# neka-nat/probreg

Measured on NVIDIA H100. Metric: cpd_em_iterations_per_sec, higher is better.
Workload: dtype f32

## Files before the change

probreg_b200/csrc/cpd_b200.cu:

```cuda
#include "cpd_b200.h"
#include "kernels.cuh"
#include "lowrank.cuh"
#include "gram_i8.cuh"
#include "bcpd.cuh"
#include "gmmtree.cuh"

#include <cub/device/device_radix_sort.cuh>
#ifdef CPD_HOST_EMU
#include "emu_nccl.h"
#include "emu_solver.h"
#endif

#include <dlfcn.h>
#include <math.h>
#include <stdarg.h>
#include <stdio.h>
#include <stdlib.h>
#include <string.h>

#include <algorithm>
#include <vector>

using namespace cpd;

static thread_local char g_err[512] = "";
static int fail(int code, const char* fmt, ...) {
    va_list ap;
    va_start(ap, fmt);
    vsnprintf(g_err, sizeof(g_err), fmt, ap);
    va_end(ap);
    return code;
}
#define CU(call)                                                                                   \
    do {                                                                                           \
        cudaError_t e_ = (call);                                                                   \
        if (e_ != cudaSuccess)                                                                     \
            return fail(CPD_ERR_CUDA, "%s failed at %s:%d: %s", #call, __FILE__, __LINE__, cudaGetErrorString(e_)); \
    } while (0)
#define KCHECK() CU(cudaGetLastError())

extern "C" const char* cpd_last_error(void) { return g_err; }
extern "C" int cpd_version(void) { return 100; }
extern "C" int cpd_device_count(void) {
    int n = 0;
    if (cudaGetDeviceCount(&n) != cudaSuccess) { cudaGetLastError(); return 0; }
    return n;
}

namespace {
typedef struct { char internal[128]; } nccl_uid;
typedef void* nccl_comm;
struct NcclApi {
    void* lib = nullptr;
    int (*GetUniqueId)(nccl_uid*) = nullptr;
    int (*CommInitRank)(nccl_comm*, int, nccl_uid, int) = nullptr;
    int (*AllReduce)(const void*, void*, size_t, int, int, nccl_comm, cudaStream_t) = nullptr;
    int (*CommDestroy)(nccl_comm) = nullptr;
    const char* (*GetErrorString)(int) = nullptr;
};
NcclApi g_nccl;
int load_nccl() {
    if (g_nccl.lib) return CPD_OK;
#ifdef CPD_HOST_EMU
    static_assert(sizeof(nccl_uid) == sizeof(emu::nccl_uid_t), "unique id layout");
    g_nccl.GetUniqueId = reinterpret_cast<int (*)(nccl_uid*)>(emu::ncclGetUniqueId);
    g_nccl.CommInitRank = reinterpret_cast<int (*)(nccl_comm*, int, nccl_uid, int)>(emu::ncclCommInitRank);
    g_nccl.AllReduce = emu::ncclAllReduce;
    g_nccl.CommDestroy = emu::ncclCommDestroy;
    g_nccl.GetErrorString = emu::ncclGetErrorString;
    g_nccl.lib = (void*)&g_nccl;
    return CPD_OK;
#endif
    const char* names[] = {"libnccl.so.2", "libnccl.so"};
    void* lib = nullptr;
    for (const char* nm : names) { lib = dlopen(nm, RTLD_NOW | RTLD_GLOBAL); if (lib) break; }
    if (!lib) return fail(CPD_ERR_NCCL, "cannot dlopen libnccl.so.2: %s", dlerror());
    g_nccl.GetUniqueId = (int (*)(nccl_uid*))dlsym(lib, "ncclGetUniqueId");
    g_nccl.CommInitRank = (int (*)(nccl_comm*, int, nccl_uid, int))dlsym(lib, "ncclCommInitRank");
    g_nccl.AllReduce = (int (*)(const void*, void*, size_t, int, int, nccl_comm, cudaStream_t))dlsym(lib, "ncclAllReduce");
    g_nccl.CommDestroy = (int (*)(nccl_comm))dlsym(lib, "ncclCommDestroy");
    g_nccl.GetErrorString = (const char* (*)(int))dlsym(lib, "ncclGetErrorString");
    if (!g_nccl.GetUniqueId || !g_nccl.CommInitRank || !g_nccl.AllReduce || !g_nccl.CommDestroy)
        return fail(CPD_ERR_NCCL, "libnccl lacks an expected symbol");
    g_nccl.lib = lib;
    return CPD_OK;
}
constexpr int NCCL_DOUBLE = 8, NCCL_SUM = 0;

struct SolverApi {
    void* lib = nullptr;
    int (*Create)(void**) = nullptr;
    int (*Destroy)(void*) = nullptr;
    int (*SetStream)(void*, cudaStream_t) = nullptr;
    int (*CreateParams)(void**) = nullptr;
    int (*DestroyParams)(void*) = nullptr;
    int (*XgetrfBuf)(void*, void*, int64_t, int64_t, int, const void*, int64_t, int, size_t*, size_t*) = nullptr;
    int (*Xgetrf)(void*, void*, int64_t, int64_t, int, void*, int64_t, int64_t*, int, void*, size_t, void*, size_t, int*) = nullptr;
    int (*Xgetrs)(void*, void*, int, int64_t, int64_t, int, const void*, int64_t, const int64_t*, int, void*, int64_t, int*) = nullptr;
};
SolverApi g_sol;
int load_cusolver() {
    if (g_sol.lib) return CPD_OK;
#ifdef CPD_HOST_EMU
    g_sol.Create = emu::solverCreate; g_sol.Destroy = emu::solverDestroy; g_sol.SetStream = emu::solverSetStream;
    g_sol.CreateParams = emu::solverCreateParams; g_sol.DestroyParams = emu::solverDestroyParams;
    g_sol.XgetrfBuf = emu::solverXgetrfBuf; g_sol.Xgetrf = emu::solverXgetrf; g_sol.Xgetrs = emu::solverXgetrs;
    g_sol.lib = (void*)&g_sol;
    return CPD_OK;
#endif
    const char* names[] = {"libcusolver.so.11", "/usr/local/cuda/lib64/libcusolver.so.11", "libcusolver.so"};
    void* lib = nullptr;
    for (const char* nm : names) { lib = dlopen(nm, RTLD_NOW | RTLD_GLOBAL); if (lib) break; }
    if (!lib) return fail(CPD_ERR_CUDA, "cannot dlopen libcusolver.so.11: %s", dlerror());
#define SOLSYM(field, name) g_sol.field = (decltype(g_sol.field))dlsym(lib, name)
    SOLSYM(Create, "cusolverDnCreate");
    SOLSYM(Destroy, "cusolverDnDestroy");
    SOLSYM(SetStream, "cusolverDnSetStream");
    SOLSYM(CreateParams, "cusolverDnCreateParams");
    SOLSYM(DestroyParams, "cusolverDnDestroyParams");
    SOLSYM(XgetrfBuf, "cusolverDnXgetrf_bufferSize");
    SOLSYM(Xgetrf, "cusolverDnXgetrf");
    SOLSYM(Xgetrs, "cusolverDnXgetrs");
#undef SOLSYM
    if (!g_sol.Create || !g_sol.SetStream || !g_sol.CreateParams || !g_sol.XgetrfBuf || !g_sol.Xgetrf || !g_sol.Xgetrs)
        return fail(CPD_ERR_CUDA, "libcusolver lacks an expected symbol");
    g_sol.lib = lib;
    return CPD_OK;
}
constexpr int CUDA_R_64F_ = 1, CUBLAS_OP_T_ = 1;
}
#define SOLV(call)                                                                          \
    do {                                                                                    \
        int r_ = (call);                                                                    \
        if (r_ != 0) return fail(CPD_ERR_CUDA, "%s failed with cusolverStatus %d", #call, r_); \
    } while (0)
#define NC(call)                                                                                                   \
    do {                                                                                                           \
        int r_ = (call);                                                                                           \
        if (r_ != 0)                                                                                               \
            return fail(CPD_ERR_NCCL, "%s failed: %s", #call, g_nccl.GetErrorString ? g_nccl.GetErrorString(r_) : "?"); \
    } while (0)

struct cpd_ctx {
    int device = 0, dim = 3, sm_count = 132, slots1 = 264, slots2 = 264;
    cudaStream_t stream = nullptr;
    bool own_stream = false;
    long long m = 0, mpad = 0, n = 0, npad = 0, n_global = 0;
    double *d_yc = nullptr, *d_ts = nullptr, *d_xc = nullptr, *d_raw = nullptr;
    size_t raw_cap = 0;
    float4 *d_srcP = nullptr, *d_srcJ = nullptr, *d_tgtP = nullptr, *d_tgtQ = nullptr;
    P1Part* d_part1 = nullptr;
    double* d_part2 = nullptr;
    size_t part1_cap = 0, part2_cap = 0;
    double *d_pt1 = nullptr, *d_p1 = nullptr, *d_pxc = nullptr, *d_px = nullptr;
    double *d_mom_src = nullptr, *d_mom_tgt = nullptr, *d_mom = nullptr, *d_sums = nullptr;
    size_t mom_src_cap = 0, mom_tgt_cap = 0, sums_cap = 0;
    DevState* d_state = nullptr;
    DevState h_state;
    double* h_pin = nullptr;
    double* d_frame = nullptr;
    double* h_stats = nullptr;
    cudaEvent_t stats_ev = nullptr, copy_ev = nullptr;
    int stats_pending = 0;
    long long stats_count[2] = {0, 0};
    bool origin_given = false;
    int it1 = 0, it2 = 0, j1 = 1, j2 = 1, g1 = 1, g2 = 1;
    float4 *d_sbox = nullptr, *d_tbox = nullptr, *d_ssub = nullptr, *d_tsub = nullptr;
    float *d_omax = nullptr, *d_omax_sub = nullptr;
    bool cull_on = true, cull_active = false;
    double extent = 0.0;
    int4 *d_work1 = nullptr, *d_work2 = nullptr;
    int *d_slots1 = nullptr, *d_slots2 = nullptr;
    bool have_source = false, have_target = false, have_state = false, prepared = false;
    nccl_comm comm = nullptr;
    int world = 1, rank = 0;
    int *d_perm_src = nullptr, *d_perm_tgt = nullptr, *d_idx_tmp = nullptr;
    unsigned *d_codes = nullptr, *d_codes_out = nullptr;
    size_t sort_cap = 0, sort_tmp_cap = 0;
    void* d_sort_tmp = nullptr;
    double *d_outN = nullptr, *d_outM = nullptr;
    float* d_G = nullptr;
    double *d_W = nullptr, *d_A = nullptr, *d_B = nullptr, *d_ts2 = nullptr, *d_nrpart = nullptr;
    int64_t* d_ipiv = nullptr;
    int* d_info = nullptr;
    void *d_work = nullptr, *h_work = nullptr, *sol = nullptr, *sol_params = nullptr;
    size_t work_dev = 0, work_host = 0;
    long long nr_m = 0;
    double nr_lmd = 0.0;
    bool nr_ready = false;
    bool nr_lost_to_bcpd = false;
    float* d_la = nullptr;
    double *d_la64 = nullptr, *d_la_part = nullptr, *d_bc_es = nullptr;
    size_t la_cap = 0;
    double* d_log2c = nullptr;
    bool wgt_on = false;
    BcpdState* d_bc = nullptr;
    float* d_bc_ginv = nullptr;
    double *d_bc_A = nullptr, *d_bc_S = nullptr, *d_bc_v = nullptr, *d_bc_r = nullptr, *d_bc_alpha = nullptr, *d_bc_sdiag = nullptr,
           *d_bc_part = nullptr, *d_bc_sums = nullptr;
    int64_t* d_bc_ipiv = nullptr;
    int* d_bc_info = nullptr;
    long long bc_m = 0;
    size_t bc_part_cap = 0;
    double bc_sigma2 = 0.0;
    bool bc_ready = false;
    bool bc_stopped = false;
    cudaEvent_t bc_ev[6] = {nullptr, nullptr, nullptr, nullptr, nullptr, nullptr};
    float bc_ms[5] = {0.f, 0.f, 0.f, 0.f, 0.f};
    long long bc_vec_m = 0, bc_dense_m = 0;
    bool bc_lowrank = false;
    double *d_bc_sys = nullptr, *d_bc_C = nullptr, *d_bc_CQ = nullptr, *d_bc_rt = nullptr, *d_bc_w = nullptr;
    int64_t* d_bc_lr_ipiv = nullptr;
    long long bc_lr_m = 0;
    int bc_lr_k = 0;
    int gt_levels = 0;
    long long gt_total = 0, gt_cap = 0, gt_m = 0;
    size_t gt_part_cap = 0, gt_sort_cap = 0;
    double *d_gt_nodes = nullptr, *d_gt_prep = nullptr, *d_gt_pts = nullptr, *d_gt_spts = nullptr, *d_gt_g = nullptr,
           *d_gt_part = nullptr, *d_gt_mom = nullptr, *d_gt_scr = nullptr;
    unsigned *d_gt_keys = nullptr, *d_gt_keys2 = nullptr;
    int *d_gt_idx = nullptr, *d_gt_idx2 = nullptr, *d_gt_cur = nullptr, *d_gt_start = nullptr, *d_gt_end = nullptr, *d_gt_asg = nullptr;
    long long* d_gt_seeds = nullptr;
    void* d_gt_sort = nullptr;
    cudaEvent_t gt_ev[7] = {nullptr, nullptr, nullptr, nullptr, nullptr, nullptr, nullptr};
    float gt_ms[6] = {0.f, 0.f, 0.f, 0.f, 0.f, 0.f};
    double *d_wgt = nullptr, *d_p1t = nullptr, *d_pxt = nullptr;
    long long prior_m = 0;
    double prior_alpha = 1.0;
    bool prior_on = false;
    int lr_rank = 0;
    int lr_owner = 0;
    double lr_gscale = 1.0;
    bool lr_w_stale = false;
    float lr_setup_ms[3] = {0.f, 0.f, 0.f};
    long long lr_m = 0;
    int lr_cap = 0;
    float4* d_lr_pts = nullptr;
    double *d_lr_Q = nullptr, *d_lr_X = nullptr, *d_lr_coef = nullptr, *d_lr_part = nullptr, *d_lr_Bc = nullptr, *d_lr_S = nullptr,
           *d_lr_R = nullptr, *d_lr_sys = nullptr, *d_lr_rhs = nullptr, *d_lr_c = nullptr, *d_lr_out = nullptr, *d_lr_panel = nullptr, *d_lr_Lt = nullptr;
    bool lr_spd = true;
    size_t lr_part_cap = 0;
    unsigned char* d_gi_planes = nullptr;
    double *d_gi_part = nullptr, *d_gi_colmax = nullptr;
    size_t gi_planes_cap = 0, gi_part_cap = 0, gi_colmax_cap = 0;
    size_t lr_out_cap = 0;
    P2PMailbox* d_box = nullptr;
    P2PInfo* d_p2p = nullptr;
    void* peer_ptr[P2P_MAX] = {nullptr};
    cudaEvent_t ev0 = nullptr, ev1 = nullptr, sev[7] = {nullptr, nullptr, nullptr, nullptr, nullptr, nullptr, nullptr};
    bool profiling = false;
    int64_t launches = 0;
    DevState* h_state_ring = nullptr;
    cudaEvent_t state_ev[8] = {nullptr, nullptr, nullptr, nullptr, nullptr, nullptr, nullptr, nullptr};
    int state_slot = 0;
    bool graph_on = true;
    cudaGraphExec_t em_graph = nullptr;
    int em_graph_key = -1, em_graph_launches = 0, prepare_gen = 0;
    void* d_flush = nullptr;
    size_t flush_cap = 0;
    std::vector<cudaEvent_t> pool;
};

namespace {
constexpr int STATE_RING = 8;
template <typename T>
int dev_alloc(T** p, size_t count) {
    if (*p) { cudaFree(*p); *p = nullptr; }
    cudaError_t e = cudaMalloc((void**)p, std::max<size_t>(count, 1) * sizeof(T));
    if (e != cudaSuccess) return fail(CPD_ERR_CUDA, "cudaMalloc(%zu bytes) failed: %s", count * sizeof(T), cudaGetErrorString(e));
    return CPD_OK;
}
#define TRY(x) do { int r__ = (x); if (r__ != CPD_OK) return r__; } while (0)
template <typename T>
struct DevBuf {
    T* p = nullptr;
    ~DevBuf() { if (p) cudaFree(p); }
    int alloc(size_t count) { return dev_alloc(&p, count); }
};

inline unsigned blocks_for(long long n) { return (unsigned)((n + THREADS - 1) / THREADS); }

struct WorkList {
    std::vector<int4> items;
    std::vector<int> tile_slots;
    int max_slots = 1;
};
WorkList build_work(int ntiles, int nunits, int slots, double last_cost, double overhead) {
    const double OVERHEAD = overhead;
    WorkList w;
    nunits = std::max(1, nunits);
    auto cost_of = [&](int t) { return t == ntiles - 1 ? last_cost : 1.0; };
    auto span_of = [&](int t, int j) { return cost_of(t) * (double)((nunits + j - 1) / j) + OVERHEAD; };
    int best_j = 1;
    double best = 1e300;
    for (int j = 1; j <= nunits; ++j) {
        const long long items = (long long)ntiles * j;
        const double waves = ceil((double)items / slots);
        const double span = waves * ((double)((nunits + j - 1) / j) + OVERHEAD);
        if (span < best - 1e-9) { best = span; best_j = j; }
        if (items > 8LL * slots) break;
    }
    w.tile_slots.assign(ntiles, best_j);
    if (ntiles <= slots) {
        std::vector<int> cuts(ntiles, 1);
        int used = ntiles;
        while (used < slots) {
            int worst = -1;
            double wv = -1.0;
            for (int t = 0; t < ntiles; ++t) {
                const double v = span_of(t, cuts[t]);
                if (cuts[t] < nunits && v > wv) { wv = v; worst = t; }
            }
            if (worst < 0) break;
            ++cuts[worst];
            ++used;
        }
        double span = 0.0;
        for (int t = 0; t < ntiles; ++t) span = std::max(span, span_of(t, cuts[t]));
        if (span <= best + 1e-9) w.tile_slots = cuts;
    }
    for (int t = 0; t < ntiles; ++t) {
        const int j = w.tile_slots[t];
        for (int s = 0; s < j; ++s) {
            const int a = (int)((long long)nunits * s / j), b = (int)((long long)nunits * (s + 1) / j);
            w.items.push_back(make_int4(t, a, b, s));
        }
        w.max_slots = std::max(w.max_slots, j);
    }
    std::stable_sort(w.items.begin(), w.items.end(), [&](const int4& a, const int4& b) {
        return cost_of(a.x) * (a.z - a.y) > cost_of(b.x) * (b.z - b.y);
    });
    return w;
}

int ensure_stats(cpd_ctx* h);
int upload_state(cpd_ctx* h) {
    TRY(ensure_stats(h));
    if (!h->h_state_ring) {
        CU(cudaMallocHost((void**)&h->h_state_ring, STATE_RING * sizeof(DevState)));
        for (int k = 0; k < STATE_RING; ++k) CU(cudaEventCreateWithFlags(&h->state_ev[k], cudaEventDisableTiming));
    }
    const int k = h->state_slot;
    h->state_slot = (k + 1) % STATE_RING;
    CU(cudaEventSynchronize(h->state_ev[k]));
    h->h_state_ring[k] = h->h_state;
    CU(cudaMemcpyAsync(h->d_state, &h->h_state_ring[k], sizeof(DevState), cudaMemcpyHostToDevice, h->stream));
    CU(cudaEventRecord(h->state_ev[k], h->stream));
    return CPD_OK;
}

int upload_cloud(cpd_ctx* h, const double* src, long long count, double* dst3) {
    if (h->dim == 3) {
        CU(cudaMemcpyAsync(dst3, src, (size_t)count * 3 * sizeof(double), cudaMemcpyHostToDevice, h->stream));
    } else {
        CU(cudaMemsetAsync(dst3, 0, (size_t)count * 3 * sizeof(double), h->stream));
        CU(cudaMemcpy2DAsync(dst3, 3 * sizeof(double), src, 2 * sizeof(double), 2 * sizeof(double), (size_t)count,
                             cudaMemcpyHostToDevice, h->stream));
    }
    return CPD_OK;
}
int download_cloud(cpd_ctx* h, const double* src3, long long count, double* dst) {
    if (h->dim == 3) {
        CU(cudaMemcpyAsync(dst, src3, (size_t)count * 3 * sizeof(double), cudaMemcpyDeviceToHost, h->stream));
    } else {
        CU(cudaMemcpy2DAsync(dst, 2 * sizeof(double), src3, 3 * sizeof(double), 2 * sizeof(double), (size_t)count,
                             cudaMemcpyDeviceToHost, h->stream));
    }
    return CPD_OK;
}

int cloud_sums_dev(cpd_ctx* h, const double* d_pts, long long count, double* part, double* d_out) {
    const unsigned nb = blocks_for(count);
    cloud_sums_kernel<<<nb, THREADS, 0, h->stream>>>(d_pts, count, part);
    reduce_cols_kernel<<<1, 4 * 32, 0, h->stream>>>(part, (int)nb, 4, d_out);
    KCHECK();
    h->launches += 2;
    return CPD_OK;
}

int ingest_cloud(cpd_ctx* h, const double* host_pts, long long count, int is_target, long long n_global, const double* origin,
                 int* d_perm, double* d_out) {
    if (h->raw_cap < (size_t)count * 3) { TRY(dev_alloc(&h->d_raw, (size_t)count * 3)); h->raw_cap = (size_t)count * 3; }
    const unsigned nb = blocks_for(count);
    if (h->sums_cap < (size_t)nb * 9 + 16) {
        TRY(dev_alloc(&h->d_sums, (size_t)nb * 9 + 16));
        h->sums_cap = (size_t)nb * 9 + 16;
    }
    if (h->sort_cap < (size_t)count) {
        TRY(dev_alloc(&h->d_codes, (size_t)count));
        TRY(dev_alloc(&h->d_codes_out, (size_t)count));
        TRY(dev_alloc(&h->d_idx_tmp, (size_t)count));
        h->sort_cap = (size_t)count;
    }
    size_t need = 0;
    CU(cub::DeviceRadixSort::SortPairs(nullptr, need, h->d_codes, h->d_codes_out, h->d_idx_tmp, d_perm, (int)count, 0, 30, h->stream));
    if (need > h->sort_tmp_cap) {
        if (h->d_sort_tmp) cudaFree(h->d_sort_tmp);
        h->d_sort_tmp = nullptr;
        CU(cudaMalloc(&h->d_sort_tmp, need));
        h->sort_tmp_cap = need;
    }
    TRY(upload_cloud(h, host_pts, count, h->d_raw));
    CU(cudaEventRecord(h->copy_ev, h->stream));
    double* frame = h->d_frame + 8 * is_target;
    stats_kernel<<<nb, THREADS, 0, h->stream>>>(h->d_raw, count, h->d_sums + 16);
    stats_fold_kernel<<<1, 288, 0, h->stream>>>(h->d_sums + 16, (int)nb, h->d_sums);
    cloud_frame_kernel<<<1, 32, 0, h->stream>>>(h->d_sums, count, is_target, n_global, origin != nullptr, origin ? origin[0] : 0.0,
                                                origin ? origin[1] : 0.0, origin ? origin[2] : 0.0, h->d_state, frame);
    CU(cudaMemcpyAsync(h->h_stats + 9 * is_target, h->d_sums, 9 * sizeof(double), cudaMemcpyDeviceToHost, h->stream));
    CU(cudaEventRecord(h->stats_ev, h->stream));
    h->stats_pending |= 1 << is_target;
    h->stats_count[is_target] = count;
    morton_frame_kernel<<<nb, THREADS, 0, h->stream>>>(h->d_raw, count, frame, h->d_codes, h->d_idx_tmp);
    CU(cub::DeviceRadixSort::SortPairs(h->d_sort_tmp, need, h->d_codes, h->d_codes_out, h->d_idx_tmp, d_perm, (int)count, 0, 30,
                                       h->stream));
    gather3_frame_kernel<<<nb, THREADS, 0, h->stream>>>(h->d_raw, d_perm, count, frame, d_out);
    KCHECK();
    h->launches += 6;
    CU(cudaEventSynchronize(h->copy_ev));
    return CPD_OK;
}

int ensure_stats(cpd_ctx* h) {
    if (!h->stats_pending) return CPD_OK;
    CU(cudaEventSynchronize(h->stats_ev));
    if (h->stats_pending & 1)
        for (int a = 0; a < 3; ++a) h->h_state.cy[a] = h->h_stats[a] / (double)h->stats_count[0];
    if (h->stats_pending & 2) {
        const double* t = h->h_stats + 9;
        if (!h->origin_given) for (int a = 0; a < 3; ++a) h->h_state.cx[a] = t[a] / (double)h->stats_count[1];
        h->extent = std::max(t[6] - t[3], std::max(t[7] - t[4], t[8] - t[5]));
    }
    h->stats_pending = 0;
    return CPD_OK;
}

int prepare(cpd_ctx* h) {
    TRY(ensure_stats(h));
    if (h->prepared) return CPD_OK;
    if (!h->have_source || !h->have_target) return fail(CPD_ERR_STATE, "source and target must both be set");
    h->it1 = (int)((h->n + ITILE1 - 1) / ITILE1);
    h->it2 = (int)((h->m + ITILE2 - 1) / ITILE2);
    const long long in_last = h->n - (long long)(h->it1 - 1) * ITILE1;
    const int live = (int)((in_last + 32 * RI1 - 1) / (32 * RI1));
    double last_cost = live < THREADS / 32 ? std::max(0.6, live / (double)(THREADS / 32)) : 1.0;
    if (const char* e = getenv("CPD_B200_PLAN_LAST_COST")) { const double v = atof(e); if (v > 0.0 && v <= 1.0) last_cost = v; }
    WorkList w1;
    if (const char* e = getenv("CPD_B200_PLAN_UNIT"); e && !strcmp(e, "stage")) {
        w1 = build_work(h->it1, (int)(h->mpad / P1_STAGE), h->slots1, last_cost, 0.5);
        for (int4& it : w1.items) { it.y *= P1_STAGE / SUB; it.z *= P1_STAGE / SUB; }
    } else {
        w1 = build_work(h->it1, (int)(h->mpad / SUB), h->slots1, last_cost, 0.5 * (P1_STAGE / SUB));
    }
    const WorkList w2 = build_work(h->it2, (int)(h->npad / P2_STAGE), h->slots2, 1.0, 0.5);
    h->j1 = w1.max_slots; h->g1 = (int)w1.items.size();
    h->j2 = w2.max_slots; h->g2 = (int)w2.items.size();
    TRY(dev_alloc(&h->d_work1, w1.items.size()));
    TRY(dev_alloc(&h->d_work2, w2.items.size()));
    TRY(dev_alloc(&h->d_slots1, w1.tile_slots.size()));
    TRY(dev_alloc(&h->d_slots2, w2.tile_slots.size()));
    CU(cudaMemcpyAsync(h->d_work1, w1.items.data(), w1.items.size() * sizeof(int4), cudaMemcpyHostToDevice, h->stream));
    CU(cudaMemcpyAsync(h->d_work2, w2.items.data(), w2.items.size() * sizeof(int4), cudaMemcpyHostToDevice, h->stream));
    CU(cudaMemcpyAsync(h->d_slots1, w1.tile_slots.data(), w1.tile_slots.size() * sizeof(int), cudaMemcpyHostToDevice, h->stream));
    CU(cudaMemcpyAsync(h->d_slots2, w2.tile_slots.data(), w2.tile_slots.size() * sizeof(int), cudaMemcpyHostToDevice, h->stream));
    CU(cudaStreamSynchronize(h->stream));
    TRY(dev_alloc(&h->d_sbox, (size_t)(h->mpad / P1_STAGE) * 2));
    TRY(dev_alloc(&h->d_tbox, (size_t)(h->npad / P2_STAGE) * 2));
    TRY(dev_alloc(&h->d_omax, (size_t)(h->npad / P2_STAGE)));
    TRY(dev_alloc(&h->d_ssub, (size_t)(h->mpad / SUB) * 2));
    TRY(dev_alloc(&h->d_tsub, (size_t)(h->npad / SUB) * 2));
    TRY(dev_alloc(&h->d_omax_sub, (size_t)(h->npad / SUB)));
    const size_t need1 = (size_t)h->j1 * h->n, need2 = (size_t)h->j2 * h->m * 4;
    if (need1 > h->part1_cap) { TRY(dev_alloc(&h->d_part1, need1)); h->part1_cap = need1; }
    if (need2 > h->part2_cap) { TRY(dev_alloc(&h->d_part2, need2)); h->part2_cap = need2; }
    const size_t ms = (size_t)blocks_for(h->m) * MOM_SRC, mt = (size_t)blocks_for(h->npad) * MOM_TGT;
    if (ms > h->mom_src_cap) { TRY(dev_alloc(&h->d_mom_src, ms)); h->mom_src_cap = ms; }
    if (mt > h->mom_tgt_cap) { TRY(dev_alloc(&h->d_mom_tgt, mt)); h->mom_tgt_cap = mt; }
    h->prepared = true;
    h->prepare_gen += 1;
    return CPD_OK;
}

int allreduce(cpd_ctx* h, double* buf, size_t count) {
    if (!h->comm) return CPD_OK;
    NC(g_nccl.AllReduce(buf, buf, count, NCCL_DOUBLE, NCCL_SUM, h->comm, h->stream));
    return CPD_OK;
}

inline void mark(cpd_ctx* h, int k) {
    if (h->profiling) cudaEventRecord(h->sev[k], h->stream);
}

int launch_estep(cpd_ctx* h, const double* d_sigma2, const double* d_w, const double* d_ts) {
    TRY(prepare(h));
    const long long cover = std::max(h->mpad, h->n);
    mark(h, 0);
    pack_kernel<<<blocks_for(cover), THREADS, 0, h->stream>>>(h->d_state, d_sigma2, h->d_yc, d_ts, h->d_xc, h->m, h->mpad,
                                                              h->n, h->d_srcP, h->d_srcJ, h->d_tgtP);
    mark(h, 1);
    const bool cull = h->cull_on && h->cull_active;
    const int nst1 = (int)(h->mpad / P1_STAGE);
    stage_bbox_kernel<<<(unsigned)nst1, THREADS, 0, h->stream>>>(h->d_srcP, (int)h->m, P1_STAGE, h->d_sbox);
    h->launches += 1;
    const int nsub1 = (int)(h->mpad / SUB), nsub2 = (int)(h->npad / SUB);
    if (cull) {
        stage_bbox_kernel<<<(unsigned)(h->npad / P2_STAGE), THREADS, 0, h->stream>>>(h->d_tgtP, (int)h->n, P2_STAGE, h->d_tbox);
        sub_bbox_kernel<<<(unsigned)((nsub1 + 7) / 8), THREADS, 0, h->stream>>>(h->d_srcP, (int)h->m, nsub1, h->d_ssub);
        sub_bbox_kernel<<<(unsigned)((nsub2 + 7) / 8), THREADS, 0, h->stream>>>(h->d_tgtP, (int)h->n, nsub2, h->d_tsub);
        h->launches += 3;
    }
    const bool wgt = h->wgt_on;
    if (wgt) {
        weight_patch_kernel<<<blocks_for(h->m), THREADS, 0, h->stream>>>(h->d_la, h->m, h->d_srcP, h->d_srcJ);
        h->launches += 1;
    }
#define CPD_PASS1(C, W) pass1_kernel<C, W><<<h->g1, THREADS, PASS1_SMEM, h->stream>>>(h->d_tgtP, (int)h->n, h->d_srcJ, h->d_work1, h->d_part1, h->d_sbox, nst1, (C) ? h->d_ssub : nullptr)
    if (cull) { if (wgt) CPD_PASS1(true, true); else CPD_PASS1(true, false); }
    else { if (wgt) CPD_PASS1(false, true); else CPD_PASS1(false, false); }
#undef CPD_PASS1
    mark(h, 2);
    finalize1_kernel<<<blocks_for(h->npad), THREADS, 0, h->stream>>>(h->d_state, d_sigma2, d_w, h->d_part1, h->d_slots1, (int)h->n,
                                                                     h->d_tgtP, h->d_tgtQ, h->npad, h->d_pt1, h->d_mom_tgt,
                                                                     wgt ? h->d_log2c : nullptr);
    mark(h, 3);
    if (cull) {
        stage_omax_kernel<<<(unsigned)(h->npad / P2_STAGE), THREADS, 0, h->stream>>>(h->d_tgtQ, h->d_omax);
        sub_omax_kernel<<<(unsigned)((nsub2 + 7) / 8), THREADS, 0, h->stream>>>(h->d_tgtQ, nsub2, h->d_omax_sub);
        h->launches += 2;
    }
#define CPD_PASS2(C, W) pass2_kernel<C, W><<<h->g2, THREADS, PASS2_SMEM, h->stream>>>(h->d_srcP, (int)h->m, h->d_tgtQ, h->d_work2, h->d_part2, (C) ? h->d_tbox : nullptr, (C) ? h->d_omax : nullptr, (C) ? h->d_tsub : nullptr, (C) ? h->d_omax_sub : nullptr)
    if (cull) { if (wgt) CPD_PASS2(true, true); else CPD_PASS2(true, false); }
    else { if (wgt) CPD_PASS2(false, true); else CPD_PASS2(false, false); }
#undef CPD_PASS2
    mark(h, 4);
    finalize2_kernel<<<blocks_for(h->m), THREADS, 0, h->stream>>>(h->d_state, d_sigma2, h->d_part2, h->d_slots2, (int)h->m, h->d_yc,
                                                                  d_ts, h->d_p1, h->d_pxc, h->d_mom_src);
    mark(h, 5);
    mark(h, 6);
    KCHECK();
    h->launches += 5;
    return CPD_OK;
}

int read_params(cpd_ctx* h, cpd_params* out) {
    static_assert(sizeof(DevState) <= 48 * sizeof(double), "DevState outgrew the pinned staging buffer");
    CU(cudaMemcpyAsync(h->h_pin, h->d_state, sizeof(DevState), cudaMemcpyDeviceToHost, h->stream));
    CU(cudaStreamSynchronize(h->stream));
    if (reinterpret_cast<const DevState*>(h->h_pin)->err)
        return fail(CPD_ERR_STATE, "a peer rank did not deliver its moments within the P2P exchange timeout");
    const int d = h->dim;
    for (int i = 0; i < 9; ++i) out->lin[i] = 0.0;
    for (int i = 0; i < d; ++i)
        for (int j = 0; j < d; ++j) out->lin[i * d + j] = h->h_pin[3 * i + j];
    for (int i = 0; i < 3; ++i) out->t[i] = (i < d) ? h->h_pin[9 + i] : 0.0;
    out->scale = h->h_pin[12];
    out->sigma2 = h->h_pin[13];
    TRY(ensure_stats(h));
    h->cull_active = h->extent > 0.0 && 13.3 * sqrt(out->sigma2) < 0.25 * h->extent;
    out->q = h->h_pin[14];
    out->n_p = h->h_pin[15];
    return CPD_OK;
}
}

extern "C" int cpd_plan_work(int ntiles, int nunits, int slots, double last_tile_cost, int* items ,
                             int capacity, int* n_items, int* max_slots) {
    if (ntiles < 1 || nunits < 1 || slots < 1 || !(last_tile_cost > 0.0 && last_tile_cost <= 1.0) || !n_items || !max_slots)
        return fail(CPD_ERR_ARG, "bad argument");
    const WorkList w = build_work(ntiles, nunits, slots, last_tile_cost, 0.5 * (P1_STAGE / SUB));
    *n_items = (int)w.items.size();
    *max_slots = w.max_slots;
    if (items) {
        if (capacity < (int)w.items.size()) return fail(CPD_ERR_ARG, "capacity %d < %d work items", capacity, (int)w.items.size());
        for (size_t i = 0; i < w.items.size(); ++i) {
            items[4 * i] = w.items[i].x; items[4 * i + 1] = w.items[i].y; items[4 * i + 2] = w.items[i].z; items[4 * i + 3] = w.items[i].w;
        }
    }
    return CPD_OK;
}

extern "C" int cpd_create(cpd_ctx** out, int device, int dim, void* stream) {
    if (!out) return fail(CPD_ERR_ARG, "out is NULL");
    if (dim != 2 && dim != 3) return fail(CPD_ERR_ARG, "dim must be 2 or 3, got %d", dim);
    int ndev = 0;
    if (cudaGetDeviceCount(&ndev) != cudaSuccess || ndev == 0) {
        cudaGetLastError();
        return fail(CPD_ERR_CUDA, "no CUDA device: this library has no CPU path");
    }
    if (device < 0 || device >= ndev) return fail(CPD_ERR_ARG, "device %d out of range (%d visible)", device, ndev);
    CU(cudaSetDevice(device));
    cudaDeviceProp prop;
    CU(cudaGetDeviceProperties(&prop, device));
    if (prop.major != 9 || prop.minor != 0)
        return fail(CPD_ERR_CUDA, "device %d is sm_%d%d; this library is built for sm_90a (Hopper) only", device, prop.major, prop.minor);
    cpd_ctx* h = new cpd_ctx();
    h->device = device;
    h->dim = dim;
    h->sm_count = prop.multiProcessorCount;
    if (stream) { h->stream = (cudaStream_t)stream; h->own_stream = false; }
    else { CU(cudaStreamCreateWithFlags(&h->stream, cudaStreamNonBlocking)); h->own_stream = true; }
    CU(cudaFuncSetAttribute(pass1_kernel<false, false>, cudaFuncAttributeMaxDynamicSharedMemorySize, PASS1_SMEM));
    CU(cudaFuncSetAttribute(pass2_kernel<false, false>, cudaFuncAttributeMaxDynamicSharedMemorySize, PASS2_SMEM));
    CU(cudaFuncSetAttribute(pass1_kernel<true, false>, cudaFuncAttributeMaxDynamicSharedMemorySize, PASS1_SMEM));
    CU(cudaFuncSetAttribute(pass2_kernel<true, false>, cudaFuncAttributeMaxDynamicSharedMemorySize, PASS2_SMEM));
    CU(cudaFuncSetAttribute(pass1_kernel<false, true>, cudaFuncAttributeMaxDynamicSharedMemorySize, PASS1_SMEM));
    CU(cudaFuncSetAttribute(pass2_kernel<false, true>, cudaFuncAttributeMaxDynamicSharedMemorySize, PASS2_SMEM));
    CU(cudaFuncSetAttribute(pass1_kernel<true, true>, cudaFuncAttributeMaxDynamicSharedMemorySize, PASS1_SMEM));
    CU(cudaFuncSetAttribute(pass2_kernel<true, true>, cudaFuncAttributeMaxDynamicSharedMemorySize, PASS2_SMEM));
    int occ1 = 0, occ2 = 0;
    CU(cudaOccupancyMaxActiveBlocksPerMultiprocessor(&occ1, pass1_kernel<false, false>, THREADS, PASS1_SMEM));
    CU(cudaOccupancyMaxActiveBlocksPerMultiprocessor(&occ2, pass2_kernel<false, false>, THREADS, PASS2_SMEM));
    h->slots1 = h->sm_count * std::max(1, occ1);
    h->slots2 = h->sm_count * std::max(1, occ2);
    TRY(dev_alloc(&h->d_state, 1));
    TRY(dev_alloc(&h->d_mom, (size_t)MOM_PAD));
    CU(cudaMallocHost((void**)&h->h_pin, 64 * sizeof(double)));
    TRY(dev_alloc(&h->d_frame, 16));
    CU(cudaMallocHost((void**)&h->h_stats, 18 * sizeof(double)));
    CU(cudaEventCreateWithFlags(&h->stats_ev, cudaEventDisableTiming));
    CU(cudaEventCreateWithFlags(&h->copy_ev, cudaEventDisableTiming));
    CU(cudaEventCreate(&h->ev0));
    CU(cudaEventCreate(&h->ev1));
    for (int k = 0; k < 7; ++k) CU(cudaEventCreate(&h->sev[k]));
    { const char* e = getenv("CPD_B200_NO_CULL"); h->cull_on = !(e && e[0] == '1'); }
    { const char* e = getenv("CPD_B200_NO_GRAPH"); h->graph_on = !(e && e[0] == '1'); }
    memset(&h->h_state, 0, sizeof(DevState));
    h->h_state.dim = dim;
    h->h_state.scale = 1.0;
    h->h_state.lin[0] = h->h_state.lin[4] = h->h_state.lin[8] = 1.0;
    h->h_state.update_scale = 1;
    *out = h;
    return upload_state(h);
}

extern "C" void cpd_destroy(cpd_ctx* h) {
    if (!h) return;
    cudaSetDevice(h->device);
    cudaStreamSynchronize(h->stream);
    void* wl[] = {h->d_work1, h->d_work2, h->d_slots1, h->d_slots2, h->d_sbox, h->d_tbox, h->d_omax, h->d_ssub, h->d_tsub, h->d_omax_sub};
    for (void* p : wl) if (p) cudaFree(p);
    void* srt[] = {h->d_perm_src, h->d_perm_tgt, h->d_idx_tmp, h->d_codes, h->d_codes_out, h->d_sort_tmp, h->d_outN, h->d_outM};
    for (void* p : srt) if (p) cudaFree(p);
    void* nrp[] = {h->d_G, h->d_W, h->d_A, h->d_B, h->d_ts2, h->d_nrpart, h->d_ipiv, h->d_info, h->d_work};
    for (void* p : nrp) if (p) cudaFree(p);
    void* lrp[] = {h->d_lr_pts, h->d_lr_Q, h->d_lr_X, h->d_lr_coef, h->d_lr_part, h->d_lr_Bc, h->d_lr_S, h->d_lr_R, h->d_lr_sys, h->d_lr_rhs,
                   h->d_lr_c, h->d_lr_out, h->d_lr_panel, h->d_lr_Lt, h->d_gi_planes, h->d_gi_part, h->d_gi_colmax, h->d_wgt, h->d_p1t, h->d_pxt, h->d_la, h->d_log2c,
                   h->d_la64, h->d_la_part, h->d_bc_es};
    for (void* p : lrp) if (p) cudaFree(p);
    void* bcp[] = {h->d_bc, h->d_bc_ginv, h->d_bc_A, h->d_bc_S, h->d_bc_v, h->d_bc_r, h->d_bc_alpha, h->d_bc_sdiag, h->d_bc_part, h->d_bc_sums,
                   h->d_bc_ipiv, h->d_bc_info, h->d_bc_sys, h->d_bc_C, h->d_bc_CQ, h->d_bc_rt, h->d_bc_w, h->d_bc_lr_ipiv};
    for (void* p : bcp) if (p) cudaFree(p);
    for (cudaEvent_t e : h->bc_ev) if (e) cudaEventDestroy(e);
    void* gtp[] = {h->d_gt_nodes, h->d_gt_prep, h->d_gt_pts, h->d_gt_spts, h->d_gt_g, h->d_gt_part, h->d_gt_mom, h->d_gt_scr, h->d_gt_keys,
                   h->d_gt_keys2, h->d_gt_idx, h->d_gt_idx2, h->d_gt_cur, h->d_gt_start, h->d_gt_end, h->d_gt_asg, h->d_gt_seeds, h->d_gt_sort};
    for (void* p : gtp) if (p) cudaFree(p);
    for (cudaEvent_t e : h->gt_ev) if (e) cudaEventDestroy(e);
    if (h->h_work) free(h->h_work);
    if (h->sol_params && g_sol.DestroyParams) g_sol.DestroyParams(h->sol_params);
    if (h->sol && g_sol.Destroy) g_sol.Destroy(h->sol);
    for (int r = 0; r < P2P_MAX; ++r) if (h->peer_ptr[r]) cudaIpcCloseMemHandle(h->peer_ptr[r]);
    if (h->d_box) cudaFree(h->d_box);
    if (h->d_p2p) cudaFree(h->d_p2p);
    void* ptrs[] = {h->d_yc, h->d_ts, h->d_xc, h->d_raw, h->d_srcP, h->d_srcJ, h->d_tgtP, h->d_tgtQ, h->d_part1, h->d_part2, h->d_pt1, h->d_p1,
                    h->d_pxc, h->d_px, h->d_mom_src, h->d_mom_tgt, h->d_mom, h->d_sums, h->d_state, h->d_flush};
    for (void* p : ptrs) if (p) cudaFree(p);
    if (h->h_pin) cudaFreeHost(h->h_pin);
    if (h->h_stats) cudaFreeHost(h->h_stats);
    if (h->d_frame) cudaFree(h->d_frame);
    if (h->stats_ev) cudaEventDestroy(h->stats_ev);
    if (h->copy_ev) cudaEventDestroy(h->copy_ev);
#ifndef CPD_HOST_EMU
    if (h->em_graph) cudaGraphExecDestroy(h->em_graph);
#endif
    if (h->h_state_ring) cudaFreeHost(h->h_state_ring);
    for (int k = 0; k < 8; ++k) if (h->state_ev[k]) cudaEventDestroy(h->state_ev[k]);
    if (h->ev0) cudaEventDestroy(h->ev0);
    if (h->ev1) cudaEventDestroy(h->ev1);
    for (int k = 0; k < 7; ++k) if (h->sev[k]) cudaEventDestroy(h->sev[k]);
    for (cudaEvent_t e : h->pool) if (e) cudaEventDestroy(e);
    if (h->own_stream) cudaStreamDestroy(h->stream);
    delete h;
}

extern "C" int cpd_set_source(cpd_ctx* h, const double* source, int64_t m) {
    if (!h || !source) return fail(CPD_ERR_ARG, "null argument");
    if (m < 1 || m > 0x7fffffffLL - 65536) return fail(CPD_ERR_ARG, "source count %lld out of range", (long long)m);
    CU(cudaSetDevice(h->device));
    if (m != h->m || !h->d_yc) {
        h->m = m;
        h->mpad = (m + P1_STAGE - 1) / P1_STAGE * P1_STAGE;
        TRY(dev_alloc(&h->d_yc, (size_t)m * 3));
        TRY(dev_alloc(&h->d_ts, (size_t)m * 3));
        TRY(dev_alloc(&h->d_srcP, (size_t)h->mpad));
        TRY(dev_alloc(&h->d_srcJ, (size_t)h->mpad * 2));
        TRY(dev_alloc(&h->d_p1, (size_t)m));
        TRY(dev_alloc(&h->d_pxc, (size_t)m * 3));
        TRY(dev_alloc(&h->d_px, (size_t)m * 3));
        TRY(dev_alloc(&h->d_perm_src, (size_t)m));
        TRY(dev_alloc(&h->d_outM, (size_t)m * 3));
        h->prepared = false;
        h->nr_ready = false;
    }
    TRY(ingest_cloud(h, source, m, 0, 0, nullptr, h->d_perm_src, h->d_yc));
    h->bc_ready = false;
    h->bc_stopped = false;
    h->h_state.m = m;
    h->have_source = true;
    return CPD_OK;
}

extern "C" int cpd_set_target(cpd_ctx* h, const double* target, int64_t n_local, int64_t n_global, const double* frame_origin) {
    if (!h || !target) return fail(CPD_ERR_ARG, "null argument");
    if (n_local < 1 || n_local > 0x7fffffffLL - 65536) return fail(CPD_ERR_ARG, "target count %lld out of range", (long long)n_local);
    if (n_global < n_local) return fail(CPD_ERR_ARG, "n_global (%lld) < n_local (%lld)", (long long)n_global, (long long)n_local);
    if (!frame_origin && n_global != n_local) return fail(CPD_ERR_ARG, "a sharded target needs an explicit frame_origin");
    CU(cudaSetDevice(h->device));
    if (n_local != h->n || !h->d_xc) {
        h->n = n_local;
        h->npad = (n_local + P2_STAGE - 1) / P2_STAGE * P2_STAGE;
        TRY(dev_alloc(&h->d_xc, (size_t)n_local * 3));
        TRY(dev_alloc(&h->d_tgtP, (size_t)n_local));
        TRY(dev_alloc(&h->d_tgtQ, (size_t)h->npad * 3));
        TRY(dev_alloc(&h->d_pt1, (size_t)n_local));
        TRY(dev_alloc(&h->d_perm_tgt, (size_t)n_local));
        TRY(dev_alloc(&h->d_outN, (size_t)n_local));
        h->prepared = false;
    }
    h->n_global = n_global;
    double origin[3] = {0.0, 0.0, 0.0};
    if (frame_origin) for (int a = 0; a < h->dim; ++a) origin[a] = frame_origin[a];
    h->origin_given = frame_origin != nullptr;
    if (h->origin_given) for (int a = 0; a < 3; ++a) h->h_state.cx[a] = origin[a];
    TRY(ingest_cloud(h, target, n_local, 1, n_global, frame_origin ? origin : nullptr, h->d_perm_tgt, h->d_xc));
    h->h_state.n_global = n_global;
    h->have_target = true;
    return CPD_OK;
}

extern "C" int cpd_sigma2_init(cpd_ctx* h, double* sigma2) {
    if (!h || !sigma2) return fail(CPD_ERR_ARG, "null argument");
    if (!h->have_source || !h->have_target) return fail(CPD_ERR_STATE, "source and target must both be set");
    CU(cudaSetDevice(h->device));
    double sx[4], sy[4];
    const size_t pn = (size_t)blocks_for(h->n) * 4, pm = (size_t)blocks_for(h->m) * 4;
    if (h->sums_cap < 16 + pn + pm) { TRY(dev_alloc(&h->d_sums, 16 + pn + pm)); h->sums_cap = 16 + pn + pm; }
    TRY(cloud_sums_dev(h, h->d_xc, h->n, h->d_sums + 16, h->d_sums));
    if (h->comm) TRY(allreduce(h, h->d_sums, 4));
    TRY(cloud_sums_dev(h, h->d_yc, h->m, h->d_sums + 16 + pn, h->d_sums + 4));
    CU(cudaMemcpyAsync(h->h_pin, h->d_sums, 8 * sizeof(double), cudaMemcpyDeviceToHost, h->stream));
    CU(cudaStreamSynchronize(h->stream));
    TRY(ensure_stats(h));
    for (int k = 0; k < 4; ++k) { sx[k] = h->h_pin[k]; sy[k] = h->h_pin[4 + k]; }
    double dlt[3], d2 = 0.0, dsy = 0.0;
    for (int a = 0; a < 3; ++a) { dlt[a] = h->h_state.cy[a] - h->h_state.cx[a]; d2 += dlt[a] * dlt[a]; dsy += dlt[a] * sy[1 + a]; }
    const double M = (double)h->m, N = (double)h->n_global;
    const double syy = sy[0] + 2.0 * dsy + M * d2;
    double cross = 0.0;
    for (int a = 0; a < 3; ++a) cross += sx[1 + a] * (sy[1 + a] + M * dlt[a]);
    *sigma2 = (M * sx[0] + N * syy - 2.0 * cross) / (M * N * h->dim);
    return CPD_OK;
}

extern "C" int cpd_set_state(cpd_ctx* h, int tf_kind, int update_scale, double w, const cpd_params* init) {
    if (!h || !init) return fail(CPD_ERR_ARG, "null argument");
    if (tf_kind != CPD_TF_RIGID && tf_kind != CPD_TF_AFFINE) return fail(CPD_ERR_ARG, "tf_kind %d not supported by the fused EM loop", tf_kind);
    if (!(w >= 0.0 && w < 1.0)) return fail(CPD_ERR_ARG, "w must be in [0, 1), got %g", w);
    if (!(init->sigma2 > 0.0)) return fail(CPD_ERR_ARG, "sigma2 must be positive, got %g", init->sigma2);
    CU(cudaSetDevice(h->device));
    DevState& s = h->h_state;
    const int d = h->dim;
    for (int i = 0; i < 3; ++i)
        for (int j = 0; j < 3; ++j) s.lin[3 * i + j] = (i < d && j < d) ? init->lin[i * d + j] : (i == j ? 1.0 : 0.0);
    for (int i = 0; i < 3; ++i) s.t[i] = (i < d) ? init->t[i] : 0.0;
    s.scale = (tf_kind == CPD_TF_RIGID) ? init->scale : 1.0;
    s.sigma2 = init->sigma2;
    s.q = init->q;
    s.n_p = 0.0;
    s.w = w;
    s.tf_kind = tf_kind;
    s.update_scale = update_scale ? 1 : 0;
    s.dim = d;
    TRY(ensure_stats(h));
    h->cull_active = h->extent > 0.0 && 13.3 * sqrt(init->sigma2) < 0.25 * h->extent;
    h->have_state = true;
    return upload_state(h);
}

namespace {
int em_step_launches(cpd_ctx* h) {
    TRY(launch_estep(h, &h->d_state->sigma2, &h->d_state->w, nullptr));
    const int nbs = (int)blocks_for(h->m), nbt = (int)blocks_for(h->npad);
    if (h->d_p2p) {
        moments_p2p_kernel<<<1, 256, 0, h->stream>>>(h->d_state, h->d_mom_src, nbs, RM_SRC, h->d_mom_tgt, nbt, RM_TGT, h->d_mom,
                                                     h->d_p2p);
        h->launches += 1;
    } else if (h->comm) {
        moments_kernel<0><<<1, 256, 0, h->stream>>>(h->d_state, h->d_mom_src, nbs, RM_SRC, h->d_mom_tgt, nbt, RM_TGT, h->d_mom);
        TRY(allreduce(h, h->d_mom, MOM_PAD));
        mstep_residual_kernel<<<1, 32, 0, h->stream>>>(h->d_state, h->d_mom);
        h->launches += 2;
    } else {
        moments_kernel<1><<<1, 256, 0, h->stream>>>(h->d_state, h->d_mom_src, nbs, RM_SRC, h->d_mom_tgt, nbt, RM_TGT, h->d_mom);
        h->launches += 1;
    }
    mark(h, 6);
    KCHECK();
    return CPD_OK;
}
}

extern "C" int cpd_em_step(cpd_ctx* h, cpd_params* out) {
    if (!h) return fail(CPD_ERR_ARG, "null handle");
    if (!h->have_state) return fail(CPD_ERR_STATE, "cpd_set_state has not been called");
    CU(cudaSetDevice(h->device));
#ifndef CPD_HOST_EMU
    const bool use_graph = h->graph_on && !h->profiling && !(h->comm && !h->d_p2p) && !h->wgt_on;
#else
    const bool use_graph = false;
#endif
    if (!use_graph) {
        TRY(em_step_launches(h));
    }
#ifndef CPD_HOST_EMU
    else {
        TRY(prepare(h));
        const int key = h->prepare_gen * 2 + ((h->cull_on && h->cull_active) ? 1 : 0);
        if (!h->em_graph || h->em_graph_key != key) {
            if (h->em_graph) { cudaGraphExecDestroy(h->em_graph); h->em_graph = nullptr; }
            const int64_t before = h->launches;
            cudaGraph_t g = nullptr;
            CU(cudaStreamBeginCapture(h->stream, cudaStreamCaptureModeThreadLocal));
            const int rc = em_step_launches(h);
            const cudaError_t ce = cudaStreamEndCapture(h->stream, &g);
            h->em_graph_launches = (int)(h->launches - before);
            h->launches = before;
            if (rc != CPD_OK) { if (g) cudaGraphDestroy(g); return rc; }
            if (ce != cudaSuccess) return fail(CPD_ERR_CUDA, "cudaStreamEndCapture failed: %s", cudaGetErrorString(ce));
            const cudaError_t ie = cudaGraphInstantiate(&h->em_graph, g, 0);
            cudaGraphDestroy(g);
            if (ie != cudaSuccess) { h->em_graph = nullptr; return fail(CPD_ERR_CUDA, "cudaGraphInstantiate failed: %s", cudaGetErrorString(ie)); }
            h->em_graph_key = key;
        }
        CU(cudaGraphLaunch(h->em_graph, h->stream));
        h->launches += h->em_graph_launches;
    }
#endif
    if (out) return read_params(h, out);
    return CPD_OK;
}

extern "C" int cpd_em_run(cpd_ctx* h, int maxiter, double tol, cpd_params* out, int* iters_run, double* trace) {
    if (!h || !out) return fail(CPD_ERR_ARG, "null argument");
    if (!h->have_state) return fail(CPD_ERR_STATE, "cpd_set_state has not been called");
    double q = h->h_state.q;
    int it = 0;
    cpd_params cur;
    memset(&cur, 0, sizeof(cur));
    for (it = 0; it < maxiter; ++it) {
        TRY(cpd_em_step(h, &cur));
        if (trace) { trace[2 * it] = cur.sigma2; trace[2 * it + 1] = cur.q; }
        if (fabs(cur.q - q) < tol) { ++it; break; }
        q = cur.q;
    }
    if (maxiter <= 0) TRY(read_params(h, &cur));
    *out = cur;
    if (iters_run) *iters_run = it;
    return CPD_OK;
}

extern "C" int cpd_estep(cpd_ctx* h, const double* t_source, double sigma2, double w, double* pt1, double* p1, double* px, double* n_p) {
    if (!h || !t_source) return fail(CPD_ERR_ARG, "null argument");
    if (!(sigma2 > 0.0)) return fail(CPD_ERR_ARG, "sigma2 must be positive, got %g", sigma2);
    if (!(w >= 0.0 && w < 1.0)) return fail(CPD_ERR_ARG, "w must be in [0, 1), got %g", w);
    if (!h->have_source || !h->have_target) return fail(CPD_ERR_STATE, "source and target must both be set");
    CU(cudaSetDevice(h->device));
    if (h->raw_cap < (size_t)h->m * 3) { TRY(dev_alloc(&h->d_raw, (size_t)h->m * 3)); h->raw_cap = (size_t)h->m * 3; }
    TRY(upload_cloud(h, t_source, h->m, h->d_raw));
    gather3_kernel<<<blocks_for(h->m), THREADS, 0, h->stream>>>(h->d_raw, h->d_perm_src, h->m, 0.0, 0.0, 0.0, h->d_ts);
    h->launches += 1;
    TRY(ensure_stats(h));
    h->cull_active = h->extent > 0.0 && 13.3 * sqrt(sigma2) < 0.25 * h->extent;
    h->h_pin[32] = sigma2;
    h->h_pin[33] = w;
    CU(cudaMemcpyAsync(&h->d_state->es_sigma2, h->h_pin + 32, 2 * sizeof(double), cudaMemcpyHostToDevice, h->stream));
    TRY(launch_estep(h, &h->d_state->es_sigma2, &h->d_state->es_w, h->d_ts));
    if (h->comm) {
        TRY(allreduce(h, h->d_p1, (size_t)h->m));
        TRY(allreduce(h, h->d_pxc, (size_t)h->m * 3));
    }
    return cpd_last_estep(h, pt1, p1, px, n_p);
}

namespace {
int bcpd_weights(cpd_ctx* h, const double* alpha, const double* sdiag, const int* perm, const double* ssw) {
    const long long m = h->m;
    const unsigned nb = blocks_for(m);
    bcpd_la_kernel<<<nb, THREADS, 0, h->stream>>>(alpha, sdiag, m, ssw, h->dim, h->d_la64, h->d_la_part);
    bcpd_la_finish_kernel<<<1, 32, 0, h->stream>>>(h->d_la_part, (int)nb, ssw, h->dim, h->n_global, h->d_log2c);
    bcpd_la_apply_kernel<<<nb, THREADS, 0, h->stream>>>(h->d_la64, perm, m, h->d_log2c, h->d_la);
    KCHECK();
    h->launches += 3;
    return CPD_OK;
}
int ensure_weight_buffers(cpd_ctx* h) {
    const long long m = h->m;
    if (h->la_cap < (size_t)m) {
        TRY(dev_alloc(&h->d_la, (size_t)m));
        TRY(dev_alloc(&h->d_la64, (size_t)m));
        TRY(dev_alloc(&h->d_la_part, (size_t)blocks_for(m)));
        h->la_cap = (size_t)m;
    }
    if (!h->d_log2c) TRY(dev_alloc(&h->d_log2c, 3));
    if (!h->d_bc_es) TRY(dev_alloc(&h->d_bc_es, 3));
    return CPD_OK;
}
}

extern "C" int cpd_bcpd_estep(cpd_ctx* h, const double* t_source, double scale, const double* alpha, const double* sigma_diag,
                              double sigma2, double w, double* nu_d, double* nu, double* px, double* n_p) {
    if (!h || !t_source || !alpha || !sigma_diag) return fail(CPD_ERR_ARG, "null argument");
    if (!(sigma2 > 0.0)) return fail(CPD_ERR_ARG, "sigma2 must be positive, got %g", sigma2);
    if (!(w >= 0.0 && w < 1.0)) return fail(CPD_ERR_ARG, "w must be in [0, 1), got %g", w);
    if (!h->have_source || !h->have_target) return fail(CPD_ERR_STATE, "source and target must both be set");
    CU(cudaSetDevice(h->device));
    const long long m = h->m;
    bool any_weight = false;
    for (long long i = 0; i < m; ++i) {
        if (!(alpha[i] >= 0.0) || !(sigma_diag[i] >= 0.0)) return fail(CPD_ERR_ARG, "alpha and diag(sigma_mat) must be non-negative");
        any_weight = any_weight || (alpha[i] > 0.0 && sigma_diag[i] < INFINITY);
    }
    if (!any_weight) return fail(CPD_ERR_ARG, "every source has zero weight");
    TRY(ensure_weight_buffers(h));
    h->h_pin[44] = scale;
    h->h_pin[45] = sigma2;
    h->h_pin[46] = w;
    CU(cudaMemcpyAsync(h->d_bc_es, h->h_pin + 44, 3 * sizeof(double), cudaMemcpyHostToDevice, h->stream));
    CU(cudaMemcpyAsync(h->d_outM, alpha, (size_t)m * sizeof(double), cudaMemcpyHostToDevice, h->stream));
    CU(cudaMemcpyAsync(h->d_outM + m, sigma_diag, (size_t)m * sizeof(double), cudaMemcpyHostToDevice, h->stream));
    TRY(bcpd_weights(h, h->d_outM, h->d_outM + m, h->d_perm_src, h->d_bc_es));
    if (h->raw_cap < (size_t)m * 3) { TRY(dev_alloc(&h->d_raw, (size_t)m * 3)); h->raw_cap = (size_t)m * 3; }
    TRY(upload_cloud(h, t_source, m, h->d_raw));
    gather3_kernel<<<blocks_for(m), THREADS, 0, h->stream>>>(h->d_raw, h->d_perm_src, m, 0.0, 0.0, 0.0, h->d_ts);
    h->launches += 1;
    TRY(ensure_stats(h));
    h->cull_active = h->extent > 0.0 && 13.3 * sqrt(sigma2) < 0.25 * h->extent;
    h->h_pin[32] = sigma2;
    h->h_pin[33] = w;
    CU(cudaMemcpyAsync(&h->d_state->es_sigma2, h->h_pin + 32, 2 * sizeof(double), cudaMemcpyHostToDevice, h->stream));
    h->wgt_on = true;
    const int r = launch_estep(h, &h->d_state->es_sigma2, &h->d_state->es_w, h->d_ts);
    h->wgt_on = false;
    TRY(r);
    if (h->comm) {
        TRY(allreduce(h, h->d_p1, (size_t)m));
        TRY(allreduce(h, h->d_pxc, (size_t)m * 3));
    }
    return cpd_last_estep(h, nu_d, nu, px, n_p);
}

extern "C" int cpd_last_estep(cpd_ctx* h, double* pt1, double* p1, double* px, double* n_p) {
    if (!h) return fail(CPD_ERR_ARG, "null handle");
    if (!h->prepared) return fail(CPD_ERR_STATE, "no E-step has run on this handle");
    CU(cudaSetDevice(h->device));
    if (pt1) {
        scatter_kernel<<<blocks_for(h->n), THREADS, 0, h->stream>>>(h->d_pt1, h->d_perm_tgt, h->n, 1, h->d_outN);
        CU(cudaMemcpyAsync(pt1, h->d_outN, (size_t)h->n * sizeof(double), cudaMemcpyDeviceToHost, h->stream));
        h->launches += 1;
    }
    if (p1) {
        scatter_kernel<<<blocks_for(h->m), THREADS, 0, h->stream>>>(h->d_p1, h->d_perm_src, h->m, 1, h->d_outM);
        CU(cudaMemcpyAsync(p1, h->d_outM, (size_t)h->m * sizeof(double), cudaMemcpyDeviceToHost, h->stream));
        CU(cudaStreamSynchronize(h->stream));
        h->launches += 1;
    }
    if (px) {
        uncentre_px_kernel<<<blocks_for(h->m), THREADS, 0, h->stream>>>(h->d_state, h->d_p1, h->d_pxc, (int)h->m, h->d_px);
        scatter_kernel<<<blocks_for(h->m), THREADS, 0, h->stream>>>(h->d_px, h->d_perm_src, h->m, 3, h->d_outM);
        KCHECK();
        h->launches += 2;
        TRY(download_cloud(h, h->d_outM, h->m, px));
    }
    if (n_p) {
        const unsigned nb = blocks_for(h->m);
        if (h->sums_cap < (size_t)nb * 4 + 4) { TRY(dev_alloc(&h->d_sums, (size_t)nb * 4 + 4)); h->sums_cap = (size_t)nb * 4 + 4; }
        src_moments_api_kernel<<<nb, THREADS, 0, h->stream>>>((int)h->m, h->d_yc, h->d_p1, h->d_pxc, h->d_mom_src);
        reduce_cols_kernel<<<1, MOM_SRC * 32, 0, h->stream>>>(h->d_mom_src, (int)nb, MOM_SRC, h->d_mom);
        KCHECK();
        h->launches += 2;
        CU(cudaMemcpyAsync(h->h_pin + 40, h->d_mom, sizeof(double), cudaMemcpyDeviceToHost, h->stream));
    }
    CU(cudaStreamSynchronize(h->stream));
    if (n_p) *n_p = h->h_pin[40];
    return CPD_OK;
}

extern "C" int cpd_mstep(cpd_ctx* h, int tf_kind, int update_scale, const double* pt1, const double* p1, const double* px, double n_p,
                         cpd_params* out) {
    (void)n_p;
    if (!h || !pt1 || !p1 || !px || !out) return fail(CPD_ERR_ARG, "null argument");
    if (tf_kind != CPD_TF_RIGID && tf_kind != CPD_TF_AFFINE) return fail(CPD_ERR_ARG, "tf_kind %d not supported", tf_kind);
    if (!h->have_source || !h->have_target) return fail(CPD_ERR_STATE, "source and target must both be set");
    CU(cudaSetDevice(h->device));
    TRY(prepare(h));
    h->h_state.tf_kind = tf_kind;
    h->h_state.update_scale = update_scale ? 1 : 0;
    CU(cudaMemcpyAsync(&h->d_state->tf_kind, &h->h_state.tf_kind, 2 * sizeof(int), cudaMemcpyHostToDevice, h->stream));
    CU(cudaMemcpyAsync(h->d_outN, pt1, (size_t)h->n * sizeof(double), cudaMemcpyHostToDevice, h->stream));
    gather1_kernel<<<blocks_for(h->n), THREADS, 0, h->stream>>>(h->d_outN, h->d_perm_tgt, h->n, h->d_pt1);
    CU(cudaMemcpyAsync(h->d_outM, p1, (size_t)h->m * sizeof(double), cudaMemcpyHostToDevice, h->stream));
    gather1_kernel<<<blocks_for(h->m), THREADS, 0, h->stream>>>(h->d_outM, h->d_perm_src, h->m, h->d_p1);
    if (h->raw_cap < (size_t)h->m * 3) { TRY(dev_alloc(&h->d_raw, (size_t)h->m * 3)); h->raw_cap = (size_t)h->m * 3; }
    TRY(upload_cloud(h, px, h->m, h->d_raw));
    gather3_kernel<<<blocks_for(h->m), THREADS, 0, h->stream>>>(h->d_raw, h->d_perm_src, h->m, 0.0, 0.0, 0.0, h->d_px);
    h->launches += 3;
    const int nbs = (int)blocks_for(h->m), nbt = (int)blocks_for(h->n);
    centre_px_kernel<<<nbs, THREADS, 0, h->stream>>>(h->d_state, h->d_p1, h->d_px, (int)h->m, h->d_pxc);
    src_moments_api_kernel<<<nbs, THREADS, 0, h->stream>>>((int)h->m, h->d_yc, h->d_p1, h->d_pxc, h->d_mom_src);
    tgt_moments_api_kernel<<<nbt, THREADS, 0, h->stream>>>(h->d_pt1, h->d_xc, (int)h->n, h->d_mom_tgt);
    moments_kernel<0><<<1, 256, 0, h->stream>>>(h->d_state, h->d_mom_src, nbs, MOM_SRC, h->d_mom_tgt, nbt, MOM_TGT, h->d_mom);
    KCHECK();
    if (h->comm) TRY(allreduce(h, h->d_mom + MOM_SRC, MOM_TGT));
    mstep_api_kernel<<<1, 32, 0, h->stream>>>(h->d_state, h->d_mom);
    KCHECK();
    h->launches += 5;
    return read_params(h, out);
}

#include "host_nonrigid.inl"
#include "host_bcpd.inl"
#include "host_gmmtree.inl"
#include "host_stateless.inl"
#include "host_multi.inl"
#include "host_measure.inl"
```

probreg_b200/csrc/kernels.cuh:

```cuda
#pragma once
#include <cuda_runtime.h>
#include <stdint.h>

namespace cpd {

#ifndef CPD_RI1
#define CPD_RI1 4
#endif
#ifndef CPD_RI2
#define CPD_RI2 4
#endif
#ifndef CPD_MINB1
#define CPD_MINB1 2
#endif
#ifndef CPD_MINB2
#define CPD_MINB2 2
#endif
#ifndef CPD_UNROLL1
#define CPD_UNROLL1 4
#endif
#ifndef CPD_UNROLL2
#define CPD_UNROLL2 4
#endif
#ifndef CPD_SUB
#define CPD_SUB 64
#endif
#ifndef CPD_GRP
#define CPD_GRP 8
#endif
constexpr int UNROLL1 = CPD_UNROLL1, UNROLL2 = CPD_UNROLL2;
constexpr int THREADS = 256;
constexpr int RI1 = CPD_RI1, RI2 = CPD_RI2;
constexpr int ITILE1 = THREADS * RI1, ITILE2 = THREADS * RI2;
constexpr int NPAIR1 = RI1 / 2, NPAIR2 = RI2 / 2;
#ifndef CPD_P1_STAGE
#define CPD_P1_STAGE 512
#endif
#ifndef CPD_P2_STAGE
#define CPD_P2_STAGE 512
#endif
constexpr int P1_STAGE = CPD_P1_STAGE;
constexpr int P2_STAGE = CPD_P2_STAGE;
static_assert(P1_STAGE % 256 == 0 && P2_STAGE % 256 == 0 && P1_STAGE >= 256 && P2_STAGE >= 256, "stage sizes are multiples of 256");
constexpr int P1_REC = 32, P2_REC = 48;
#ifndef CPD_NSTAGE
#define CPD_NSTAGE 3
#endif
constexpr int NSTAGE = CPD_NSTAGE;
constexpr int P1_STAGE_BYTES = P1_STAGE * P1_REC, P2_STAGE_BYTES = P2_STAGE * P2_REC;
constexpr int SUB = CPD_SUB;
constexpr int GRP = CPD_GRP;
constexpr int PASS1_SMEM = NSTAGE * P1_STAGE_BYTES + 64, PASS2_SMEM = NSTAGE * P2_STAGE_BYTES + 64;

#ifdef CPD_HOST_EMU
#define CPD_DYN_SMEM(name) unsigned char* const name = emu::g_dyn_smem
#else
#define CPD_DYN_SMEM(name) extern __shared__ __align__(128) unsigned char name[]
#endif

constexpr float O_INIT = 1048576.0f;
constexpr float TWO100 = 1.2676506002282294e30f;
constexpr float FAR_COORD = 1.0e18f;

constexpr double LOG2E = 1.4426950408889634074;
constexpr double DEAD_LOG2 = -1075.0;
constexpr double EPS32 = 1.1920928955078125e-07;

enum { RM_NP = 0, RM_SY = 1, RM_C = 4, RM_V1 = 10, RM_VY = 13, RM_SRC = 22, RM_SRR = 22, RM_NPT = 23, RM_TGT = 2,
       RM_COUNT = 24, MOM_PAD = 32 };
enum { MOM_NP = 0, MOM_SX = 1, MOM_SY = 4, MOM_B = 7, MOM_C = 16, MOM_NPT = 22, MOM_SXT = 23, MOM_TXX = 26,
       MOM_COUNT = 27, MOM_SRC = 22, MOM_TGT = 5 };

struct P1Part {
    double S;
    double SU;
    float o;
    float pad;
};

struct DevState {
    double lin[9];
    double t[3];
    double scale;
    double sigma2;
    double q;
    double n_p;
    double cx[3];
    double cy[3];
    double w;
    double es_sigma2;
    double es_w;
    long long m;
    long long n_global;
    int tf_kind;
    int update_scale;
    int dim;
    int err;
};

constexpr int P2P_MAX = 16;
struct P2PMailbox {
    double slots[2][P2P_MAX][MOM_PAD];
    unsigned long long flags[2][P2P_MAX];
};
struct P2PInfo {
    P2PMailbox* box[P2P_MAX];
    int world, rank;
    unsigned long long seq;
    unsigned long long timeout_ns;
};

#ifdef CPD_HOST_EMU
}
#include "emu_device.h"
namespace cpd {
#else
__device__ __forceinline__ float ex2(float x) {
    float y;
    asm("ex2.approx.ftz.f32 %0, %1;" : "=f"(y) : "f"(x));
    return y;
}
typedef unsigned long long u64;
__device__ __forceinline__ u64 pack2(float lo, float hi) { u64 r; asm("mov.b64 %0, {%1, %2};" : "=l"(r) : "f"(lo), "f"(hi)); return r; }
__device__ __forceinline__ float2 unpack2(u64 v) { float2 r; asm("mov.b64 {%0, %1}, %2;" : "=f"(r.x), "=f"(r.y) : "l"(v)); return r; }
__device__ __forceinline__ u64 fsub2(u64 a, u64 b) {
    const float2 x = unpack2(a), y = unpack2(b);
    return pack2(__fsub_rn(x.x, y.x), __fsub_rn(x.y, y.y));
}
__device__ __forceinline__ u64 fadd2(u64 a, u64 b) {
    const float2 x = unpack2(a), y = unpack2(b);
    return pack2(__fadd_rn(x.x, y.x), __fadd_rn(x.y, y.y));
}
__device__ __forceinline__ u64 fmul2(u64 a, u64 b) {
    const float2 x = unpack2(a), y = unpack2(b);
    return pack2(__fmul_rn(x.x, y.x), __fmul_rn(x.y, y.y));
}
__device__ __forceinline__ u64 ffma2(u64 a, u64 b, u64 c) {
    const float2 x = unpack2(a), y = unpack2(b), z = unpack2(c);
    return pack2(__fmaf_rn(x.x, y.x, z.x), __fmaf_rn(x.y, y.y, z.y));
}
__device__ __forceinline__ unsigned long long globaltimer_ns() {
    unsigned long long t;
    asm volatile("mov.u64 %0, %%globaltimer;" : "=l"(t));
    return t;
}
__device__ __forceinline__ uint32_t smem_u32(const void* p) { return (uint32_t)__cvta_generic_to_shared(p); }
__device__ __forceinline__ void mbar_init(uint64_t* bar, uint32_t count) {
    asm volatile("mbarrier.init.shared::cta.b64 [%0], %1;" ::"r"(smem_u32(bar)), "r"(count));
}
__device__ __forceinline__ void mbar_fence_init() { asm volatile("fence.mbarrier_init.release.cluster;" ::: "memory"); }
__device__ __forceinline__ void mbar_expect_tx(uint64_t* bar, uint32_t bytes) {
    asm volatile("mbarrier.arrive.expect_tx.shared::cta.b64 _, [%0], %1;" ::"r"(smem_u32(bar)), "r"(bytes) : "memory");
}
__device__ __forceinline__ void tma_load_1d(void* dst, const void* src, uint32_t bytes, uint64_t* bar) {
    asm volatile("cp.async.bulk.shared::cluster.global.mbarrier::complete_tx::bytes [%0], [%1], %2, [%3];" ::"r"(
                     smem_u32(dst)),
                 "l"(src), "r"(bytes), "r"(smem_u32(bar))
                 : "memory");
}
__device__ __forceinline__ void mbar_wait(uint64_t* bar, uint32_t parity) {
    asm volatile(
        "{\n"
        ".reg .pred P1;\n"
        "LAB_WAIT:\n"
        "mbarrier.try_wait.parity.shared::cta.b64 P1, [%0], %1;\n"
        "@P1 bra DONE;\n"
        "bra LAB_WAIT;\n"
        "DONE:\n"
        "}" ::"r"(smem_u32(bar)),
        "r"(parity)
        : "memory");
}
#endif
__device__ __forceinline__ double warp_sum(double v) {
#pragma unroll
    for (int o = 16; o > 0; o >>= 1) v += __shfl_xor_sync(0xffffffffu, v, o);
    return v;
}
template <int K>
__device__ __forceinline__ void block_reduce_store(double (&v)[K], double* out) {
    __shared__ double sh[K][THREADS / 32];
    const int lane = threadIdx.x & 31, wid = threadIdx.x >> 5;
#pragma unroll
    for (int k = 0; k < K; ++k) {
        double s = warp_sum(v[k]);
        if (lane == 0) sh[k][wid] = s;
    }
    __syncthreads();
    if (threadIdx.x < K) {
        double s = 0.0;
#pragma unroll
        for (int w = 0; w < THREADS / 32; ++w) s += sh[threadIdx.x][w];
        out[threadIdx.x] = s;
    }
}

__global__ void __launch_bounds__(THREADS)
pack_kernel(const DevState* __restrict__ st, const double* __restrict__ sigma2_ptr,
            const double* __restrict__ yc , const double* __restrict__ ts ,
            const double* __restrict__ xc , long long m, long long mpad, long long n,
            float4* __restrict__ srcP , float4* __restrict__ srcJ ,
            float4* __restrict__ tgtP ) {
    const long long i = (long long)blockIdx.x * THREADS + threadIdx.x;
    const double sk = sqrt(LOG2E / (2.0 * *sigma2_ptr));
    if (i < mpad) {
        float4 o;
        if (i < m) {
            double px, py, pz;
            if (ts != nullptr) {
                px = ts[3 * i + 0] - st->cx[0];
                py = ts[3 * i + 1] - st->cx[1];
                pz = ts[3 * i + 2] - st->cx[2];
            } else {
                const double s = (st->tf_kind == 0) ? st->scale : 1.0;
                double l[9], tp[3];
#pragma unroll
                for (int k = 0; k < 9; ++k) l[k] = s * st->lin[k];
#pragma unroll
                for (int a = 0; a < 3; ++a)
                    tp[a] = l[3 * a] * st->cy[0] + l[3 * a + 1] * st->cy[1] + l[3 * a + 2] * st->cy[2] + st->t[a] - st->cx[a];
                const double y0 = yc[3 * i], y1 = yc[3 * i + 1], y2 = yc[3 * i + 2];
                px = l[0] * y0 + l[1] * y1 + l[2] * y2 + tp[0];
                py = l[3] * y0 + l[4] * y1 + l[5] * y2 + tp[1];
                pz = l[6] * y0 + l[7] * y1 + l[8] * y2 + tp[2];
            }
            o = make_float4((float)(sk * px), (float)(sk * py), (float)(sk * pz), 0.0f);
        } else {
            o = make_float4(FAR_COORD, FAR_COORD, FAR_COORD, 0.0f);
        }
        srcP[i] = o;
        srcJ[2 * i] = make_float4(o.x, o.x, o.y, o.y);
        srcJ[2 * i + 1] = make_float4(o.z, o.z, 0.0f, 0.0f);
    }
    if (i < n) {
        tgtP[i] = make_float4((float)(sk * xc[3 * i]), (float)(sk * xc[3 * i + 1]), (float)(sk * xc[3 * i + 2]), 0.0f);
    }
}

__global__ void __launch_bounds__(THREADS)
weight_patch_kernel(const float* __restrict__ la, long long m, float4* __restrict__ srcP, float4* __restrict__ srcJ) {
    const long long i = (long long)blockIdx.x * THREADS + threadIdx.x;
    if (i < m) {
        const float v = la[i];
        srcP[i].w = v;
        float4 r = srcJ[2 * i + 1];
        r.z = v; r.w = v;
        srcJ[2 * i + 1] = r;
    }
}

constexpr float CULL_GAP = 130.0f;
__global__ void __launch_bounds__(THREADS)
stage_bbox_kernel(const float4* __restrict__ pts, int n, int blk, float4* __restrict__ box) {
    __shared__ float sh[6][THREADS / 32];
    const int b = blockIdx.x;
    float lo[3] = {3.0e38f, 3.0e38f, 3.0e38f}, hi[3] = {-3.0e38f, -3.0e38f, -3.0e38f};
    for (int i = b * blk + threadIdx.x; i < min(n, (b + 1) * blk); i += THREADS) {
        const float4 p = pts[i];
        lo[0] = fminf(lo[0], p.x); lo[1] = fminf(lo[1], p.y); lo[2] = fminf(lo[2], p.z);
        hi[0] = fmaxf(hi[0], p.x); hi[1] = fmaxf(hi[1], p.y); hi[2] = fmaxf(hi[2], p.z);
    }
    const int lane = threadIdx.x & 31, wid = threadIdx.x >> 5;
#pragma unroll
    for (int a = 0; a < 3; ++a) {
#pragma unroll
        for (int o = 16; o > 0; o >>= 1) {
            lo[a] = fminf(lo[a], __shfl_xor_sync(0xffffffffu, lo[a], o));
            hi[a] = fmaxf(hi[a], __shfl_xor_sync(0xffffffffu, hi[a], o));
        }
        if (lane == 0) { sh[a][wid] = lo[a]; sh[3 + a][wid] = hi[a]; }
    }
    __syncthreads();
    if (threadIdx.x == 0) {
        float l[3], h[3];
        for (int a = 0; a < 3; ++a) {
            l[a] = sh[a][0]; h[a] = sh[3 + a][0];
            for (int w = 1; w < THREADS / 32; ++w) { l[a] = fminf(l[a], sh[a][w]); h[a] = fmaxf(h[a], sh[3 + a][w]); }
        }
        box[2 * b] = make_float4(l[0], l[1], l[2], 0.f);
        box[2 * b + 1] = make_float4(h[0], h[1], h[2], 0.f);
    }
}
__global__ void __launch_bounds__(THREADS)
stage_omax_kernel(const float4* __restrict__ tgtQ, float* __restrict__ omax) {
    __shared__ float sh[THREADS / 32];
    const int b = blockIdx.x;
    float m = 3.0e38f;
    for (int i = threadIdx.x; i < P2_STAGE; i += THREADS) m = fminf(m, tgtQ[3 * ((size_t)b * P2_STAGE + i) + 1].z);
#pragma unroll
    for (int o = 16; o > 0; o >>= 1) m = fminf(m, __shfl_xor_sync(0xffffffffu, m, o));
    if ((threadIdx.x & 31) == 0) sh[threadIdx.x >> 5] = m;
    __syncthreads();
    if (threadIdx.x == 0) {
        for (int w = 1; w < THREADS / 32; ++w) m = fminf(m, sh[w]);
        omax[b] = -m;
    }
}
__global__ void __launch_bounds__(THREADS)
sub_bbox_kernel(const float4* __restrict__ pts, int n, int nsub, float4* __restrict__ box) {
    const int b = blockIdx.x * (THREADS / 32) + (threadIdx.x >> 5), lane = threadIdx.x & 31;
    if (b >= nsub) return;
    float lo[3] = {3.0e38f, 3.0e38f, 3.0e38f}, hi[3] = {-3.0e38f, -3.0e38f, -3.0e38f};
    for (int i = b * SUB + lane; i < min(n, (b + 1) * SUB); i += 32) {
        const float4 p = pts[i];
        lo[0] = fminf(lo[0], p.x); lo[1] = fminf(lo[1], p.y); lo[2] = fminf(lo[2], p.z);
        hi[0] = fmaxf(hi[0], p.x); hi[1] = fmaxf(hi[1], p.y); hi[2] = fmaxf(hi[2], p.z);
    }
#pragma unroll
    for (int a = 0; a < 3; ++a) {
#pragma unroll
        for (int o = 16; o > 0; o >>= 1) {
            lo[a] = fminf(lo[a], __shfl_xor_sync(0xffffffffu, lo[a], o));
            hi[a] = fmaxf(hi[a], __shfl_xor_sync(0xffffffffu, hi[a], o));
        }
    }
    if (lane == 0) {
        box[2 * b] = make_float4(lo[0], lo[1], lo[2], 0.f);
        box[2 * b + 1] = make_float4(hi[0], hi[1], hi[2], 0.f);
    }
}
__global__ void __launch_bounds__(THREADS)
sub_omax_kernel(const float4* __restrict__ tgtQ, int nsub, float* __restrict__ omax) {
    const int b = blockIdx.x * (THREADS / 32) + (threadIdx.x >> 5), lane = threadIdx.x & 31;
    if (b >= nsub) return;
    float m = 3.0e38f;
    for (int i = lane; i < SUB; i += 32) m = fminf(m, tgtQ[3 * ((size_t)b * SUB + i) + 1].z);
#pragma unroll
    for (int o = 16; o > 0; o >>= 1) m = fminf(m, __shfl_xor_sync(0xffffffffu, m, o));
    if (lane == 0) omax[b] = -m;
}
template <int NP>
__device__ __forceinline__ void warp_bbox(const u64 (&ax)[NP], const u64 (&ay)[NP], const u64 (&az)[NP], float* __restrict__ wbox) {
    float lo[3] = {3.0e38f, 3.0e38f, 3.0e38f}, hi[3] = {-3.0e38f, -3.0e38f, -3.0e38f};
#pragma unroll
    for (int p = 0; p < NP; ++p) {
        const float2 x = unpack2(ax[p]), y = unpack2(ay[p]), z = unpack2(az[p]);
        lo[0] = fminf(lo[0], fminf(x.x, x.y)); hi[0] = fmaxf(hi[0], fmaxf(x.x, x.y));
        lo[1] = fminf(lo[1], fminf(y.x, y.y)); hi[1] = fmaxf(hi[1], fmaxf(y.x, y.y));
        lo[2] = fminf(lo[2], fminf(z.x, z.y)); hi[2] = fmaxf(hi[2], fmaxf(z.x, z.y));
    }
#pragma unroll
    for (int a = 0; a < 3; ++a) {
#pragma unroll
        for (int o = 16; o > 0; o >>= 1) {
            lo[a] = fminf(lo[a], __shfl_xor_sync(0xffffffffu, lo[a], o));
            hi[a] = fmaxf(hi[a], __shfl_xor_sync(0xffffffffu, hi[a], o));
        }
    }
    if ((threadIdx.x & 31) == 0) {
#pragma unroll
        for (int a = 0; a < 3; ++a) { wbox[a] = lo[a]; wbox[3 + a] = hi[a]; }
    }
    __syncwarp();
}
__device__ __forceinline__ float box_gap2(const float* __restrict__ wbox, const float4 blo, const float4 bhi) {
    const float gx = fmaxf(0.f, fmaxf(blo.x - wbox[3], wbox[0] - bhi.x));
    const float gy = fmaxf(0.f, fmaxf(blo.y - wbox[4], wbox[1] - bhi.y));
    const float gz = fmaxf(0.f, fmaxf(blo.z - wbox[5], wbox[2] - bhi.z));
    return fmaf(gz, gz, fmaf(gy, gy, gx * gx)) * 0.9999f;
}

template <bool WGT>
__device__ __forceinline__ void pass1_sum(const ulonglong2* __restrict__ q, const u64 (&ax)[NPAIR1], const u64 (&ay)[NPAIR1],
                                          const u64 (&az)[NPAIR1], const u64 (&no)[NPAIR1], u64 (&Sc)[NPAIR1], u64 (&Uc)[NPAIR1]) {
    if (GRP > 0) {
#pragma unroll 1
        for (int g0 = 0; g0 < SUB; g0 += (GRP > 0 ? GRP : SUB)) {
            u64 gs[NPAIR1], gu[NPAIR1];
#pragma unroll
            for (int jj = 0; jj < (GRP > 0 ? GRP : 1); ++jj) {
                const ulonglong2 bxy = q[2 * (g0 + jj)];
                const u64 bz = q[2 * (g0 + jj) + 1].x;
                u64 la = 0ull;
                if (WGT) la = q[2 * (g0 + jj) + 1].y;
#pragma unroll
                for (int p = 0; p < NPAIR1; ++p) {
                    const u64 dx = fsub2(ax[p], bxy.x), dy = fsub2(ay[p], bxy.y), dz = fsub2(az[p], bz);
                    u64 t = ffma2(dx, dx, no[p]);
                    t = ffma2(dy, dy, t);
                    t = ffma2(dz, dz, t);
                    if (WGT) t = fadd2(t, la);
                    const float2 tt = unpack2(t);
                    const u64 e = pack2(ex2(-tt.x), ex2(-tt.y));
                    gs[p] = jj == 0 ? e : fadd2(gs[p], e);
                    gu[p] = jj == 0 ? fmul2(e, t) : ffma2(e, t, gu[p]);
                }
            }
#pragma unroll
            for (int p = 0; p < NPAIR1; ++p) { Sc[p] = fadd2(Sc[p], gs[p]); Uc[p] = fadd2(Uc[p], gu[p]); }
        }
    } else {
#pragma unroll UNROLL1
        for (int jj = 0; jj < SUB; ++jj) {
            const ulonglong2 bxy = q[2 * jj];
            const u64 bz = q[2 * jj + 1].x;
            u64 la = 0ull;
            if (WGT) la = q[2 * jj + 1].y;
#pragma unroll
            for (int p = 0; p < NPAIR1; ++p) {
                const u64 dx = fsub2(ax[p], bxy.x), dy = fsub2(ay[p], bxy.y), dz = fsub2(az[p], bz);
                u64 t = ffma2(dx, dx, no[p]);
                t = ffma2(dy, dy, t);
                t = ffma2(dz, dz, t);
                if (WGT) t = fadd2(t, la);
                const float2 tt = unpack2(t);
                const u64 e = pack2(ex2(-tt.x), ex2(-tt.y));
                Sc[p] = fadd2(Sc[p], e);
                Uc[p] = ffma2(e, t, Uc[p]);
            }
        }
    }
}

template <bool CULL, bool WGT>
__global__ void __launch_bounds__(THREADS, CPD_MINB1)
pass1_kernel(const float4* __restrict__ ipts, int ni, const float4* __restrict__ jrec, const int4* __restrict__ work,
             P1Part* __restrict__ part, const float4* __restrict__ sbox ,
             int nstages_total, const float4* __restrict__ ssub ) {
    __shared__ float wbox[THREADS / 32][8];
    CPD_DYN_SMEM(smraw);
    uint64_t* full = reinterpret_cast<uint64_t*>(smraw + NSTAGE * P1_STAGE_BYTES);
    const int tid = threadIdx.x;
    const int4 wk = work[blockIdx.x];
    constexpr int SPS = P1_STAGE / SUB;
    const int itile = wk.x, split = wk.w;
    const int st0 = wk.y / SPS, nst = (wk.z + SPS - 1) / SPS - st0;
    const int sc_first = wk.y - st0 * SPS, sc_last = wk.z - (st0 + nst - 1) * SPS;
    const unsigned char* jbytes = reinterpret_cast<const unsigned char*>(jrec);
    if (tid == 0) {
        for (int s = 0; s < NSTAGE; ++s) mbar_init(&full[s], 1);
        mbar_fence_init();
    }
    __syncthreads();
    if (tid == 0) {
        for (int s = 0; s < NSTAGE && s < nst; ++s) {
            mbar_expect_tx(&full[s], P1_STAGE_BYTES);
            tma_load_1d(smraw + s * P1_STAGE_BYTES, jbytes + (size_t)(st0 + s) * P1_STAGE_BYTES, P1_STAGE_BYTES, &full[s]);
        }
    }
    if (itile * ITILE1 + (tid >> 5) * (32 * RI1) >= ni) return;
    u64 ax[NPAIR1], ay[NPAIR1], az[NPAIR1], no[NPAIR1];
    double S[RI1], SU[RI1];
#pragma unroll
    for (int p = 0; p < NPAIR1; ++p) {
        int n0 = itile * ITILE1 + (tid >> 5) * (32 * RI1) + (2 * p) * 32 + (tid & 31), n1 = n0 + 32;
        n0 = n0 < ni ? n0 : ni - 1;
        n1 = n1 < ni ? n1 : ni - 1;
        const float4 p0 = ipts[n0], p1 = ipts[n1];
        ax[p] = pack2(p0.x, p1.x); ay[p] = pack2(p0.y, p1.y); az[p] = pack2(p0.z, p1.z);
        no[p] = pack2(-O_INIT, -O_INIT);
    }
    float* const mybox = wbox[tid >> 5];
    warp_bbox<NPAIR1>(ax, ay, az, mybox);
    {
        const int lane = tid & 31;
        float best = 3.0e38f;
        int bi = 0;
        for (int sidx = lane; sidx < nstages_total; sidx += 32) {
            const float g2 = box_gap2(mybox, sbox[2 * sidx], sbox[2 * sidx + 1]);
            if (g2 < best) { best = g2; bi = sidx; }
        }
#pragma unroll
        for (int o = 16; o > 0; o >>= 1) {
            const float ob = __shfl_xor_sync(0xffffffffu, best, o);
            const int oi = __shfl_xor_sync(0xffffffffu, bi, o);
            if (ob < best || (ob == best && oi < bi)) { best = ob; bi = oi; }
        }
        const ulonglong2* near = reinterpret_cast<const ulonglong2*>(jbytes + (size_t)bi * P1_STAGE_BYTES);
        float cm[RI1];
#pragma unroll
        for (int r = 0; r < RI1; ++r) cm[r] = 3.0e38f;
#pragma unroll 4
        for (int jj = 0; jj < 128; ++jj) {
            const ulonglong2 bxy = near[2 * jj];
            const u64 bz = near[2 * jj + 1].x;
            u64 la = 0ull;
            if (WGT) la = near[2 * jj + 1].y;
#pragma unroll
            for (int p = 0; p < NPAIR1; ++p) {
                const u64 dx = fsub2(ax[p], bxy.x), dy = fsub2(ay[p], bxy.y), dz = fsub2(az[p], bz);
                u64 uu = ffma2(dz, dz, ffma2(dy, dy, fmul2(dx, dx)));
                if (WGT) uu = fadd2(uu, la);
                const float2 u = unpack2(uu);
                cm[2 * p] = fminf(cm[2 * p], u.x);
                cm[2 * p + 1] = fminf(cm[2 * p + 1], u.y);
            }
        }
#pragma unroll
        for (int p = 0; p < NPAIR1; ++p)
            no[p] = pack2(-fminf(O_INIT, floorf(cm[2 * p])), -fminf(O_INIT, floorf(cm[2 * p + 1])));
    }
    float omax_w = O_INIT;
    if (CULL) {
        float om = -3.0e38f;
#pragma unroll
        for (int p = 0; p < NPAIR1; ++p) { const float2 nv = unpack2(no[p]); om = fmaxf(om, fmaxf(-nv.x, -nv.y)); }
#pragma unroll
        for (int o = 16; o > 0; o >>= 1) om = fmaxf(om, __shfl_xor_sync(0xffffffffu, om, o));
        omax_w = om;
    }
#pragma unroll
    for (int r = 0; r < RI1; ++r) { S[r] = 0.0; SU[r] = 0.0; }
    for (int it = 0; it < nst; ++it) {
        const int s = it % NSTAGE;
        mbar_wait(&full[s], (uint32_t)((it / NSTAGE) & 1));
        const ulonglong2* sp = reinterpret_cast<const ulonglong2*>(smraw + s * P1_STAGE_BYTES);
        bool skip = false;
        if (CULL) {
            const float4 blo = sbox[2 * (st0 + it)], bhi = sbox[2 * (st0 + it) + 1];
            skip = box_gap2(mybox, blo, bhi) - omax_w >= CULL_GAP;
        }
#pragma unroll 1
        for (int sc = (it == 0 ? sc_first : 0); sc < (skip ? 0 : (it == nst - 1 ? sc_last : SPS)); ++sc) {
            if (CULL) {
                const int sb = (st0 + it) * (P1_STAGE / SUB) + sc;
                if (box_gap2(mybox, ssub[2 * sb], ssub[2 * sb + 1]) - omax_w >= CULL_GAP) continue;
            }
            const ulonglong2* q = sp + sc * (2 * SUB);
            u64 Sc[NPAIR1], Uc[NPAIR1];
#pragma unroll
            for (int p = 0; p < NPAIR1; ++p) { Sc[p] = 0ull; Uc[p] = 0ull; }
            pass1_sum<WGT>(q, ax, ay, az, no, Sc, Uc);
            bool bad = false;
#pragma unroll
            for (int p = 0; p < NPAIR1; ++p) {
                const float2 v = unpack2(Sc[p]);
                bad |= !(v.x < TWO100) | !(v.y < TWO100);
            }
            if (__any_sync(0xffffffffu, bad)) {
                float cm[RI1];
#pragma unroll
                for (int r = 0; r < RI1; ++r) cm[r] = 3.0e38f;
#pragma unroll UNROLL1
                for (int jj = 0; jj < SUB; ++jj) {
                    const ulonglong2 bxy = q[2 * jj];
                    const u64 bz = q[2 * jj + 1].x;
                    u64 la = 0ull;
                    if (WGT) la = q[2 * jj + 1].y;
#pragma unroll
                    for (int p = 0; p < NPAIR1; ++p) {
                        const u64 dx = fsub2(ax[p], bxy.x), dy = fsub2(ay[p], bxy.y), dz = fsub2(az[p], bz);
                        u64 uu = ffma2(dz, dz, ffma2(dy, dy, fmul2(dx, dx)));
                        if (WGT) uu = fadd2(uu, la);
                        const float2 u = unpack2(uu);
                        cm[2 * p] = fminf(cm[2 * p], u.x);
                        cm[2 * p + 1] = fminf(cm[2 * p + 1], u.y);
                    }
                }
#pragma unroll
                for (int p = 0; p < NPAIR1; ++p) {
                    const float2 nv = unpack2(no[p]);
                    const float o0 = -nv.x, o1 = -nv.y;
                    const float on0 = fminf(o0, floorf(cm[2 * p])), on1 = fminf(o1, floorf(cm[2 * p + 1]));
                    const int sh0 = (int)fmaxf(on0 - o0, -4000.0f), sh1 = (int)fmaxf(on1 - o1, -4000.0f);
                    S[2 * p] = ldexp(S[2 * p], sh0); SU[2 * p] = ldexp(SU[2 * p], sh0);
                    S[2 * p + 1] = ldexp(S[2 * p + 1], sh1); SU[2 * p + 1] = ldexp(SU[2 * p + 1], sh1);
                    no[p] = pack2(-on0, -on1);
                    Sc[p] = 0ull; Uc[p] = 0ull;
                }
                if (CULL) {
                    float om = -3.0e38f;
#pragma unroll
                    for (int p = 0; p < NPAIR1; ++p) { const float2 nv = unpack2(no[p]); om = fmaxf(om, fmaxf(-nv.x, -nv.y)); }
#pragma unroll
                    for (int o = 16; o > 0; o >>= 1) om = fmaxf(om, __shfl_xor_sync(0xffffffffu, om, o));
                    omax_w = om;
                }
                pass1_sum<WGT>(q, ax, ay, az, no, Sc, Uc);
            }
#pragma unroll
            for (int p = 0; p < NPAIR1; ++p) {
                const float2 sv = unpack2(Sc[p]), uv = unpack2(Uc[p]), nv = unpack2(no[p]);
                S[2 * p] += (double)sv.x;
                S[2 * p + 1] += (double)sv.y;
                SU[2 * p] += (double)uv.x - (double)nv.x * (double)sv.x;
                SU[2 * p + 1] += (double)uv.y - (double)nv.y * (double)sv.y;
            }
        }
        __syncthreads();
        if (tid == 0 && it + NSTAGE < nst) {
            mbar_expect_tx(&full[s], P1_STAGE_BYTES);
            tma_load_1d(smraw + s * P1_STAGE_BYTES, jbytes + (size_t)(st0 + it + NSTAGE) * P1_STAGE_BYTES, P1_STAGE_BYTES, &full[s]);
        }
    }
#pragma unroll
    for (int p = 0; p < NPAIR1; ++p) {
        const float2 nv = unpack2(no[p]);
#pragma unroll
        for (int h = 0; h < 2; ++h) {
            const int n = itile * ITILE1 + (tid >> 5) * (32 * RI1) + (2 * p + h) * 32 + (tid & 31);
            if (n < ni) {
                P1Part out;
                out.S = S[2 * p + h]; out.SU = SU[2 * p + h]; out.o = h ? -nv.y : -nv.x; out.pad = 0.0f;
                part[(size_t)split * ni + n] = out;
            }
        }
    }
}

__global__ void __launch_bounds__(THREADS)
finalize1_kernel(const DevState* __restrict__ st, const double* __restrict__ sigma2_ptr, const double* __restrict__ w_ptr,
                 const P1Part* __restrict__ part, const int* __restrict__ tile_slots, int n, const float4* __restrict__ tgtP,
                 float4* __restrict__ tgtQ, long long npad, double* __restrict__ pt1, double* __restrict__ mom_part,
                 const double* __restrict__ log2c_ptr ) {
    const int i = blockIdx.x * THREADS + threadIdx.x;
    double v[RM_TGT] = {0.0, 0.0};
    if (i < n) {
        const int nsplit = tile_slots[i / ITILE1];
        float omin = 3.0e38f;
        for (int s = 0; s < nsplit; ++s) {
            const P1Part p = part[(size_t)s * n + i];
            if (p.S > 0.0) omin = fminf(omin, p.o);
        }
        double log2S = -INFINITY, SU = 0.0;
        if (omin < 3.0e38f) {
            double S = 0.0;
            for (int s = 0; s < nsplit; ++s) {
                const P1Part p = part[(size_t)s * n + i];
                if (p.S > 0.0) {
                    const int sh = (int)fmaxf(omin - p.o, -4000.0f);
                    S += ldexp(p.S, sh);
                    SU += ldexp(p.SU, sh);
                }
            }
            log2S = log2(S) - (double)omin;
        }
        const double sigma2 = *sigma2_ptr, w = *w_ptr;
        double c = 0.0;
        if (w > 0.0) {
            const double tps = 2.0 * 3.14159265358979323846 * sigma2;
            c = (st->dim == 3 ? tps * sqrt(tps) : tps) * (w / (1.0 - w) * (double)st->m / (double)st->n_global);
        }
        double lc = c > 0.0 ? log2(c) : -INFINITY, dead_shift = 0.0;
        if (log2c_ptr != nullptr) { lc = log2c_ptr[0]; dead_shift = log2c_ptr[1]; c = (lc > -INFINITY) ? 1.0 : 0.0; }
        const bool dead = !(log2S + dead_shift >= DEAD_LOG2);
        double L = 0.0, p1n = 0.0;
        if (!dead) {
            if (c > 0.0) {
                const double hi = fmax(log2S, lc), lo = fmin(log2S, lc);
                L = hi + log2(1.0 + exp2(lo - hi));
                p1n = exp2(log2S - L);
            } else {
                L = log2S; p1n = 1.0;
            }
        }
        pt1[i] = p1n;
        const float4 b = tgtP[i];
        float no = INFINITY, rnf = 0.0f;
        if (!dead) {
            const double rn = exp2(-(L + (double)omin));
            no = -omin;
            rnf = (float)rn;
            v[0] = SU * (double)rnf;
        }
        v[1] = p1n;
        tgtQ[3 * (size_t)i] = make_float4(b.x, b.x, b.y, b.y);
        tgtQ[3 * (size_t)i + 1] = make_float4(b.z, b.z, no, no);
        tgtQ[3 * (size_t)i + 2] = make_float4(rnf, rnf, 0.f, 0.f);
    } else if (i < npad) {
        tgtQ[3 * (size_t)i] = make_float4(0.f, 0.f, 0.f, 0.f);
        tgtQ[3 * (size_t)i + 1] = make_float4(0.f, 0.f, INFINITY, INFINITY);
        tgtQ[3 * (size_t)i + 2] = make_float4(0.f, 0.f, 0.f, 0.f);
    }
    block_reduce_store<RM_TGT>(v, mom_part + (size_t)blockIdx.x * RM_TGT);
}

template <bool CULL, bool WGT>
__global__ void __launch_bounds__(THREADS, CPD_MINB2)
pass2_kernel(const float4* __restrict__ ipts, int ni, const float4* __restrict__ jrec, const int4* __restrict__ work,
             double* __restrict__ part , const float4* __restrict__ tbox ,
             const float* __restrict__ omax_stage, const float4* __restrict__ tsub, const float* __restrict__ omax_sub) {
    __shared__ float wbox[THREADS / 32][8];
    CPD_DYN_SMEM(smraw);
    uint64_t* full = reinterpret_cast<uint64_t*>(smraw + NSTAGE * P2_STAGE_BYTES);
    const int tid = threadIdx.x;
    const int4 wk = work[blockIdx.x];
    const int itile = wk.x, st0 = wk.y, split = wk.w;
    const int nst = wk.z - wk.y;
    const unsigned char* jbytes = reinterpret_cast<const unsigned char*>(jrec);
    if (tid == 0) {
        for (int s = 0; s < NSTAGE; ++s) mbar_init(&full[s], 1);
        mbar_fence_init();
    }
    __syncthreads();
    if (tid == 0) {
        for (int s = 0; s < NSTAGE && s < nst; ++s) {
            mbar_expect_tx(&full[s], P2_STAGE_BYTES);
            tma_load_1d(smraw + s * P2_STAGE_BYTES, jbytes + (size_t)(st0 + s) * P2_STAGE_BYTES, P2_STAGE_BYTES, &full[s]);
        }
    }
    u64 ax[NPAIR2], ay[NPAIR2], az[NPAIR2], al[NPAIR2];
    double A1[RI2], AX[RI2], AY[RI2], AZ[RI2];
#pragma unroll
    for (int p = 0; p < NPAIR2; ++p) {
        int m0 = itile * ITILE2 + (tid >> 5) * (32 * RI2) + (2 * p) * 32 + (tid & 31), m1 = m0 + 32;
        m0 = m0 < ni ? m0 : ni - 1;
        m1 = m1 < ni ? m1 : ni - 1;
        const float4 p0 = ipts[m0], p1 = ipts[m1];
        ax[p] = pack2(p0.x, p1.x); ay[p] = pack2(p0.y, p1.y); az[p] = pack2(p0.z, p1.z);
        if (WGT) al[p] = pack2(p0.w, p1.w);
    }
    float* const mybox = wbox[tid >> 5];
    if (CULL) warp_bbox<NPAIR2>(ax, ay, az, mybox);
#pragma unroll
    for (int r = 0; r < RI2; ++r) { A1[r] = 0.0; AX[r] = 0.0; AY[r] = 0.0; AZ[r] = 0.0; }
    for (int it = 0; it < nst; ++it) {
        const int s = it % NSTAGE;
        mbar_wait(&full[s], (uint32_t)((it / NSTAGE) & 1));
        const ulonglong2* sp = reinterpret_cast<const ulonglong2*>(smraw + s * P2_STAGE_BYTES);
        bool skip = false;
        if (CULL) {
            const float4 blo = tbox[2 * (st0 + it)], bhi = tbox[2 * (st0 + it) + 1];
            skip = box_gap2(mybox, blo, bhi) - omax_stage[st0 + it] >= CULL_GAP;
        }
#pragma unroll 1
        for (int sc = 0; sc < (skip ? 0 : P2_STAGE / SUB); ++sc) {
            if (CULL) {
                const int sb = (st0 + it) * (P2_STAGE / SUB) + sc;
                if (box_gap2(mybox, tsub[2 * sb], tsub[2 * sb + 1]) - omax_sub[sb] >= CULL_GAP) continue;
            }
            const ulonglong2* q = sp + sc * (3 * SUB);
            u64 s1[NPAIR2], sx[NPAIR2], sy[NPAIR2], sz[NPAIR2];
#pragma unroll
            for (int p = 0; p < NPAIR2; ++p) { s1[p] = 0ull; sx[p] = 0ull; sy[p] = 0ull; sz[p] = 0ull; }
            if (GRP > 0) {
#pragma unroll 1
                for (int g0 = 0; g0 < SUB; g0 += (GRP > 0 ? GRP : SUB)) {
                    u64 g1[NPAIR2], gx[NPAIR2], gy[NPAIR2], gz[NPAIR2];
#pragma unroll
                    for (int jj = 0; jj < (GRP > 0 ? GRP : 1); ++jj) {
                        const ulonglong2 bxy = q[3 * (g0 + jj)];
                        const ulonglong2 bzo = q[3 * (g0 + jj) + 1];
                        const u64 rn = q[3 * (g0 + jj) + 2].x;
#pragma unroll
                        for (int p = 0; p < NPAIR2; ++p) {
                            const u64 dx = fsub2(ax[p], bxy.x), dy = fsub2(ay[p], bxy.y), dz = fsub2(az[p], bzo.x);
                            u64 t = ffma2(dx, dx, bzo.y);
                            t = ffma2(dy, dy, t);
                            t = ffma2(dz, dz, t);
                            if (WGT) t = fadd2(t, al[p]);
                            const float2 tt = unpack2(t);
                            const u64 pr = fmul2(pack2(ex2(-tt.x), ex2(-tt.y)), rn);
                            g1[p] = jj == 0 ? pr : fadd2(g1[p], pr);
                            gx[p] = jj == 0 ? fmul2(pr, dx) : ffma2(pr, dx, gx[p]);
                            gy[p] = jj == 0 ? fmul2(pr, dy) : ffma2(pr, dy, gy[p]);
                            gz[p] = jj == 0 ? fmul2(pr, dz) : ffma2(pr, dz, gz[p]);
                        }
                    }
#pragma unroll
                    for (int p = 0; p < NPAIR2; ++p) {
                        s1[p] = fadd2(s1[p], g1[p]); sx[p] = fadd2(sx[p], gx[p]);
                        sy[p] = fadd2(sy[p], gy[p]); sz[p] = fadd2(sz[p], gz[p]);
                    }
                }
            } else {
#pragma unroll UNROLL2
                for (int jj = 0; jj < SUB; ++jj) {
                    const ulonglong2 bxy = q[3 * jj];
                    const ulonglong2 bzo = q[3 * jj + 1];
                    const u64 rn = q[3 * jj + 2].x;
#pragma unroll
                    for (int p = 0; p < NPAIR2; ++p) {
                        const u64 dx = fsub2(ax[p], bxy.x), dy = fsub2(ay[p], bxy.y), dz = fsub2(az[p], bzo.x);
                        u64 t = ffma2(dx, dx, bzo.y);
                        t = ffma2(dy, dy, t);
                        t = ffma2(dz, dz, t);
                        if (WGT) t = fadd2(t, al[p]);
                        const float2 tt = unpack2(t);
                        const u64 pr = fmul2(pack2(ex2(-tt.x), ex2(-tt.y)), rn);
                        s1[p] = fadd2(s1[p], pr);
                        sx[p] = ffma2(pr, dx, sx[p]);
                        sy[p] = ffma2(pr, dy, sy[p]);
                        sz[p] = ffma2(pr, dz, sz[p]);
                    }
                }
            }
#pragma unroll
            for (int p = 0; p < NPAIR2; ++p) {
                const float2 v1 = unpack2(s1[p]), vx = unpack2(sx[p]), vy = unpack2(sy[p]), vz = unpack2(sz[p]);
                A1[2 * p] += (double)v1.x; AX[2 * p] += (double)vx.x; AY[2 * p] += (double)vy.x; AZ[2 * p] += (double)vz.x;
                A1[2 * p + 1] += (double)v1.y; AX[2 * p + 1] += (double)vx.y; AY[2 * p + 1] += (double)vy.y; AZ[2 * p + 1] += (double)vz.y;
            }
        }
        __syncthreads();
        if (tid == 0 && it + NSTAGE < nst) {
            mbar_expect_tx(&full[s], P2_STAGE_BYTES);
            tma_load_1d(smraw + s * P2_STAGE_BYTES, jbytes + (size_t)(st0 + it + NSTAGE) * P2_STAGE_BYTES, P2_STAGE_BYTES, &full[s]);
        }
    }
#pragma unroll
    for (int r = 0; r < RI2; ++r) {
        const int m = itile * ITILE2 + (tid >> 5) * (32 * RI2) + r * 32 + (tid & 31);
        if (m < ni) {
            double2* dst = reinterpret_cast<double2*>(part + ((size_t)split * ni + m) * 4);
            dst[0] = make_double2(A1[r], AX[r]);
            dst[1] = make_double2(AY[r], AZ[r]);
        }
    }
}

__global__ void __launch_bounds__(THREADS)
finalize2_kernel(const DevState* __restrict__ st, const double* __restrict__ sigma2_ptr, const double* __restrict__ part,
                 const int* __restrict__ tile_slots, int m, const double* __restrict__ yc, const double* __restrict__ ts, double* __restrict__ p1,
                 double* __restrict__ pxc, double* __restrict__ mom_part) {
    const int i = blockIdx.x * THREADS + threadIdx.x;
    double v[RM_SRC];
#pragma unroll
    for (int k = 0; k < RM_SRC; ++k) v[k] = 0.0;
    if (i < m) {
        double a1 = 0.0, a[3] = {0.0, 0.0, 0.0};
        const int nsplit = tile_slots[i / ITILE2];
        for (int s = 0; s < nsplit; ++s) {
            const double2* src = reinterpret_cast<const double2*>(part + ((size_t)s * m + i) * 4);
            const double2 u0 = src[0], u1 = src[1];
            a1 += u0.x; a[0] += u0.y; a[1] += u1.x; a[2] += u1.y;
        }
        const double inv_sk = 1.0 / sqrt(LOG2E / (2.0 * *sigma2_ptr));
        const double vv[3] = {-a[0] * inv_sk, -a[1] * inv_sk, -a[2] * inv_sk};
        const double y[3] = {yc[3 * (size_t)i], yc[3 * (size_t)i + 1], yc[3 * (size_t)i + 2]};
        double z[3];
        if (ts != nullptr) {
#pragma unroll
            for (int d = 0; d < 3; ++d) z[d] = ts[3 * (size_t)i + d] - st->cx[d];
        } else {
            const double sc = (st->tf_kind == 0) ? st->scale : 1.0;
#pragma unroll
            for (int d = 0; d < 3; ++d) {
                const double l0 = sc * st->lin[3 * d], l1 = sc * st->lin[3 * d + 1], l2 = sc * st->lin[3 * d + 2];
                const double tp = l0 * st->cy[0] + l1 * st->cy[1] + l2 * st->cy[2] + st->t[d] - st->cx[d];
                z[d] = l0 * y[0] + l1 * y[1] + l2 * y[2] + tp;
            }
        }
        p1[i] = a1;
#pragma unroll
        for (int d = 0; d < 3; ++d) pxc[3 * (size_t)i + d] = a1 * z[d] + vv[d];
        v[RM_NP] = a1;
#pragma unroll
        for (int d = 0; d < 3; ++d) {
            v[RM_SY + d] = a1 * y[d];
            v[RM_V1 + d] = vv[d];
#pragma unroll
            for (int e = 0; e < 3; ++e) v[RM_VY + 3 * d + e] = vv[d] * y[e];
        }
        v[RM_C + 0] = a1 * y[0] * y[0]; v[RM_C + 1] = a1 * y[0] * y[1]; v[RM_C + 2] = a1 * y[0] * y[2];
        v[RM_C + 3] = a1 * y[1] * y[1]; v[RM_C + 4] = a1 * y[1] * y[2]; v[RM_C + 5] = a1 * y[2] * y[2];
    }
    block_reduce_store<RM_SRC>(v, mom_part + (size_t)blockIdx.x * RM_SRC);
}

__global__ void __launch_bounds__(THREADS)
src_moments_api_kernel(int m, const double* __restrict__ yc, const double* __restrict__ p1, const double* __restrict__ pxc,
                       double* __restrict__ mom_part) {
    const int i = blockIdx.x * THREADS + threadIdx.x;
    double v[MOM_SRC];
#pragma unroll
    for (int k = 0; k < MOM_SRC; ++k) v[k] = 0.0;
    if (i < m) {
        const double a1 = p1[i];
        const double a[3] = {pxc[3 * (size_t)i], pxc[3 * (size_t)i + 1], pxc[3 * (size_t)i + 2]};
        const double y[3] = {yc[3 * (size_t)i], yc[3 * (size_t)i + 1], yc[3 * (size_t)i + 2]};
        v[MOM_NP] = a1;
#pragma unroll
        for (int d = 0; d < 3; ++d) {
            v[MOM_SX + d] = a[d];
            v[MOM_SY + d] = a1 * y[d];
#pragma unroll
            for (int e = 0; e < 3; ++e) v[MOM_B + 3 * d + e] = a[d] * y[e];
        }
        v[MOM_C + 0] = a1 * y[0] * y[0]; v[MOM_C + 1] = a1 * y[0] * y[1]; v[MOM_C + 2] = a1 * y[0] * y[2];
        v[MOM_C + 3] = a1 * y[1] * y[1]; v[MOM_C + 4] = a1 * y[1] * y[2]; v[MOM_C + 5] = a1 * y[2] * y[2];
    }
    block_reduce_store<MOM_SRC>(v, mom_part + (size_t)blockIdx.x * MOM_SRC);
}

__global__ void __launch_bounds__(THREADS)
tgt_moments_api_kernel(const double* __restrict__ pt1, const double* __restrict__ xc, int n, double* __restrict__ mom_part) {
    const int i = blockIdx.x * THREADS + threadIdx.x;
    double v[MOM_TGT] = {0.0, 0.0, 0.0, 0.0, 0.0};
    if (i < n) {
        const double p = pt1[i], x0 = xc[3 * (size_t)i], x1 = xc[3 * (size_t)i + 1], x2 = xc[3 * (size_t)i + 2];
        v[0] = p; v[1] = p * x0; v[2] = p * x1; v[3] = p * x2; v[4] = p * (x0 * x0 + x1 * x1 + x2 * x2);
    }
    block_reduce_store<MOM_TGT>(v, mom_part + (size_t)blockIdx.x * MOM_TGT);
}

__device__ inline void jacobi_svd(int n, const double a[3][3], double U[3][3], double s[3], double V[3][3]) {
    double W[3][3];
    for (int i = 0; i < 3; ++i)
        for (int j = 0; j < 3; ++j) { W[i][j] = (i < n && j < n) ? a[i][j] : 0.0; V[i][j] = (i == j) ? 1.0 : 0.0; }
    for (int sweep = 0; sweep < 60; ++sweep) {
        double off = 0.0;
        for (int p = 0; p < n - 1; ++p)
            for (int q = p + 1; q < n; ++q) {
                double al = 0, be = 0, ga = 0;
                for (int i = 0; i < n; ++i) { al += W[i][p] * W[i][p]; be += W[i][q] * W[i][q]; ga += W[i][p] * W[i][q]; }
                if (ga == 0.0) continue;
                const double lim = 1e-32 * al * be;
                if (ga * ga <= lim) continue;
                off = fmax(off, ga * ga / (al * be));
                const double zeta = (be - al) / (2.0 * ga);
                const double t = (zeta >= 0 ? 1.0 : -1.0) / (fabs(zeta) + sqrt(1.0 + zeta * zeta));
                const double c = 1.0 / sqrt(1.0 + t * t), sn = c * t;
                for (int i = 0; i < n; ++i) {
                    const double wp = W[i][p], wq = W[i][q];
                    W[i][p] = c * wp - sn * wq; W[i][q] = sn * wp + c * wq;
                    const double vp = V[i][p], vq = V[i][q];
                    V[i][p] = c * vp - sn * vq; V[i][q] = sn * vp + c * vq;
                }
            }
        if (off == 0.0) break;
    }
    int ord[3] = {0, 1, 2};
    double nrm[3] = {0, 0, 0};
    for (int j = 0; j < n; ++j) { double t = 0; for (int i = 0; i < n; ++i) t += W[i][j] * W[i][j]; nrm[j] = sqrt(t); }
    for (int i = 0; i < n - 1; ++i)
        for (int j = 0; j < n - 1 - i; ++j)
            if (nrm[ord[j]] < nrm[ord[j + 1]]) { int t = ord[j]; ord[j] = ord[j + 1]; ord[j + 1] = t; }
    double Vs[3][3];
    for (int j = 0; j < 3; ++j)
        for (int i = 0; i < 3; ++i) { U[i][j] = (i == j) ? 1.0 : 0.0; Vs[i][j] = (i == j) ? 1.0 : 0.0; }
    const double tiny = nrm[ord[0]] * 1e-300;
    for (int j = 0; j < n; ++j) {
        const int c = ord[j];
        s[j] = nrm[c];
        for (int i = 0; i < n; ++i) { Vs[i][j] = V[i][c]; U[i][j] = (nrm[c] > tiny) ? W[i][c] / nrm[c] : 0.0; }
    }
    for (int j = n; j < 3; ++j) s[j] = 0.0;
    if (n == 3) {
        if (!(s[2] > tiny) && s[1] > tiny) {
            U[0][2] = U[1][0] * U[2][1] - U[2][0] * U[1][1];
            U[1][2] = U[2][0] * U[0][1] - U[0][0] * U[2][1];
            U[2][2] = U[0][0] * U[1][1] - U[1][0] * U[0][1];
        }
    } else if (n == 2) {
        if (!(s[1] > tiny) && s[0] > tiny) { U[0][1] = -U[1][0]; U[1][1] = U[0][0]; }
    }
    for (int i = 0; i < 3; ++i) for (int j = 0; j < 3; ++j) V[i][j] = Vs[i][j];
}

__device__ inline double det_n(int n, const double a[3][3]) {
    if (n == 2) return a[0][0] * a[1][1] - a[0][1] * a[1][0];
    return a[0][0] * (a[1][1] * a[2][2] - a[1][2] * a[2][1]) - a[0][1] * (a[1][0] * a[2][2] - a[1][2] * a[2][0]) +
           a[0][2] * (a[1][0] * a[2][1] - a[1][1] * a[2][0]);
}

__device__ inline void solve_affine(int n, const double Y[3][3], const double A[3][3], double B[3][3]) {
    double Mx[3][6];
    for (int i = 0; i < n; ++i)
        for (int j = 0; j < n; ++j) { Mx[i][j] = Y[j][i]; Mx[i][n + j] = A[j][i]; }
    for (int k = 0; k < n; ++k) {
        int piv = k;
        for (int i = k + 1; i < n; ++i) if (fabs(Mx[i][k]) > fabs(Mx[piv][k])) piv = i;
        if (piv != k) for (int j = 0; j < 2 * n; ++j) { const double t = Mx[k][j]; Mx[k][j] = Mx[piv][j]; Mx[piv][j] = t; }
        for (int i = k + 1; i < n; ++i) {
            const double f = Mx[i][k] / Mx[k][k];
            for (int j = k; j < 2 * n; ++j) Mx[i][j] -= f * Mx[k][j];
        }
    }
    double Z[3][3];
    for (int c = 0; c < n; ++c)
        for (int i = n - 1; i >= 0; --i) {
            double t = Mx[i][n + c];
            for (int j = i + 1; j < n; ++j) t -= Mx[i][j] * Z[j][c];
            Z[i][c] = t / Mx[i][i];
        }
    for (int i = 0; i < 3; ++i) for (int j = 0; j < 3; ++j) B[i][j] = (i < n && j < n) ? Z[j][i] : (i == j ? 1.0 : 0.0);
}

__device__ inline void mstep_solve_api(DevState* st, const double* __restrict__ mom) {
    const int n = st->dim;
    const double Np = mom[MOM_NP];
    double mux[3], muy[3], A[3][3], Y[3][3];
    for (int a = 0; a < 3; ++a) { mux[a] = mom[MOM_SX + a] / Np; muy[a] = mom[MOM_SY + a] / Np; }
    const double Cs[3][3] = {{mom[MOM_C + 0], mom[MOM_C + 1], mom[MOM_C + 2]},
                             {mom[MOM_C + 1], mom[MOM_C + 3], mom[MOM_C + 4]},
                             {mom[MOM_C + 2], mom[MOM_C + 4], mom[MOM_C + 5]}};
    for (int a = 0; a < 3; ++a)
        for (int b = 0; b < 3; ++b) {
            A[a][b] = mom[MOM_B + 3 * a + b] - mom[MOM_SX + a] * mom[MOM_SY + b] / Np;
            Y[a][b] = Cs[a][b] - mom[MOM_SY + a] * mom[MOM_SY + b] / Np;
        }
    double tr_yp1y = 0.0;
    for (int a = 0; a < n; ++a) tr_yp1y += Y[a][a];
    double tr_xp1x = mom[MOM_TXX] + mom[MOM_NPT] * (mux[0] * mux[0] + mux[1] * mux[1] + mux[2] * mux[2]) -
                     2.0 * (mux[0] * mom[MOM_SXT] + mux[1] * mom[MOM_SXT + 1] + mux[2] * mom[MOM_SXT + 2]);
    double lin[3][3], scale = 1.0, sigma2, q;
    if (st->tf_kind == 0) {
        double U[3][3], s[3], V[3][3], UVt[3][3];
        jacobi_svd(n, A, U, s, V);
        for (int i = 0; i < 3; ++i)
            for (int j = 0; j < 3; ++j) { double t = 0; for (int k = 0; k < n; ++k) t += U[i][k] * V[j][k]; UVt[i][j] = t; }
        const double dt = det_n(n, UVt);
        for (int i = 0; i < 3; ++i)
            for (int j = 0; j < 3; ++j) {
                double t = 0;
                for (int k = 0; k < n; ++k) t += U[i][k] * (k == n - 1 ? dt : 1.0) * V[j][k];
                lin[i][j] = (i < n && j < n) ? t : (i == j ? 1.0 : 0.0);
            }
        double tr_atr = 0.0;
        for (int i = 0; i < n; ++i) for (int j = 0; j < n; ++j) tr_atr += A[i][j] * lin[i][j];
        scale = st->update_scale ? tr_atr / tr_yp1y : 1.0;
        if (st->update_scale) sigma2 = (tr_xp1x - scale * tr_atr) / (Np * n);
        else sigma2 = (tr_xp1x + tr_yp1y - scale * tr_atr) / (Np * n);
        sigma2 = fmax(sigma2, EPS32);
        q = (tr_xp1x - 2.0 * scale * tr_atr + scale * scale * tr_yp1y) / (2.0 * sigma2) + n * Np * 0.5 * log(sigma2);
    } else {
        solve_affine(n, Y, A, lin);
        double tr_abt = 0.0;
        for (int i = 0; i < n; ++i) for (int j = 0; j < n; ++j) tr_abt += A[i][j] * lin[i][j];
        sigma2 = fmax((tr_xp1x - tr_abt) / (Np * n), EPS32);
        q = (tr_xp1x - 2.0 * tr_abt + tr_abt) / (2.0 * sigma2) + n * Np * 0.5 * log(sigma2);
    }
    for (int a = 0; a < 3; ++a) {
        double r = 0.0;
        for (int b = 0; b < 3; ++b) r += lin[a][b] * (st->cy[b] + muy[b]);
        st->t[a] = (a < n) ? (st->cx[a] + mux[a]) - scale * r : 0.0;
        for (int b = 0; b < 3; ++b) st->lin[3 * a + b] = lin[a][b];
    }
    st->scale = scale; st->sigma2 = sigma2; st->q = q; st->n_p = Np;
}

__device__ inline void mstep_solve_residual(DevState* st, const double* __restrict__ mom) {
    const int n = st->dim;
    const double Np = mom[RM_NP];
    const double sk2 = LOG2E / (2.0 * st->sigma2);
    const double Srr = mom[RM_SRR] / sk2;
    double muy[3], V1[3], Aold[3][3], Y[3][3], Vc[3][3], Am[3][3], told[3];
    const double sc = (st->tf_kind == 0) ? st->scale : 1.0;
    for (int a = 0; a < 3; ++a) {
        muy[a] = mom[RM_SY + a] / Np;
        V1[a] = mom[RM_V1 + a];
        for (int b = 0; b < 3; ++b) Aold[a][b] = sc * st->lin[3 * a + b];
    }
    for (int a = 0; a < 3; ++a)
        told[a] = Aold[a][0] * st->cy[0] + Aold[a][1] * st->cy[1] + Aold[a][2] * st->cy[2] + st->t[a] - st->cx[a];
    const double Cs[3][3] = {{mom[RM_C + 0], mom[RM_C + 1], mom[RM_C + 2]},
                             {mom[RM_C + 1], mom[RM_C + 3], mom[RM_C + 4]},
                             {mom[RM_C + 2], mom[RM_C + 4], mom[RM_C + 5]}};
    for (int a = 0; a < 3; ++a)
        for (int b = 0; b < 3; ++b) {
            Y[a][b] = Cs[a][b] - mom[RM_SY + a] * mom[RM_SY + b] / Np;
            Vc[a][b] = mom[RM_VY + 3 * a + b] - V1[a] * mom[RM_SY + b] / Np;
        }
    for (int a = 0; a < 3; ++a)
        for (int b = 0; b < 3; ++b) {
            double t = Vc[a][b];
            for (int k = 0; k < 3; ++k) t += Aold[a][k] * Y[k][b];
            Am[a][b] = (a < n && b < n) ? t : 0.0;
        }
    double tr_yp1y = 0.0;
    for (int a = 0; a < n; ++a) tr_yp1y += Y[a][a];
    double lin[3][3], Anew[3][3], scale = 1.0, tr_atr = 0.0;
    if (st->tf_kind == 0) {
        double U[3][3], s[3], V[3][3], UVt[3][3];
        jacobi_svd(n, Am, U, s, V);
        for (int i = 0; i < 3; ++i)
            for (int j = 0; j < 3; ++j) { double t = 0; for (int k = 0; k < n; ++k) t += U[i][k] * V[j][k]; UVt[i][j] = t; }
        const double dt = det_n(n, UVt);
        for (int i = 0; i < 3; ++i)
            for (int j = 0; j < 3; ++j) {
                double t = 0;
                for (int k = 0; k < n; ++k) t += U[i][k] * (k == n - 1 ? dt : 1.0) * V[j][k];
                lin[i][j] = (i < n && j < n) ? t : (i == j ? 1.0 : 0.0);
            }
        for (int i = 0; i < n; ++i) for (int j = 0; j < n; ++j) tr_atr += Am[i][j] * lin[i][j];
        scale = st->update_scale ? tr_atr / tr_yp1y : 1.0;
    } else {
        solve_affine(n, Y, Am, lin);
    }
    for (int i = 0; i < 3; ++i) for (int j = 0; j < 3; ++j) Anew[i][j] = scale * lin[i][j];
    double Q = Srr - (V1[0] * V1[0] + V1[1] * V1[1] + V1[2] * V1[2]) / Np;
    for (int a = 0; a < n; ++a)
        for (int b = 0; b < n; ++b) {
            const double dab = Aold[a][b] - Anew[a][b];
            Q += 2.0 * dab * Vc[a][b];
            double t = 0.0;
            for (int k = 0; k < n; ++k) t += (Aold[a][k] - Anew[a][k]) * Y[k][b];
            Q += t * dab;
        }
    double sigma2;
    if (st->tf_kind == 0 && !st->update_scale) sigma2 = (Q + tr_atr) / (Np * n);
    else sigma2 = Q / (Np * n);
    sigma2 = fmax(sigma2, EPS32);
    const double q = Q / (2.0 * sigma2) + n * Np * 0.5 * log(sigma2);
    for (int a = 0; a < 3; ++a) {
        double mux = st->cx[a] + told[a] + V1[a] / Np, r = 0.0;
        for (int b = 0; b < 3; ++b) { mux += Aold[a][b] * muy[b]; r += Anew[a][b] * (st->cy[b] + muy[b]); }
        st->t[a] = (a < n) ? mux - r : 0.0;
    }
    for (int a = 0; a < 3; ++a) for (int b = 0; b < 3; ++b) st->lin[3 * a + b] = lin[a][b];
    st->scale = scale; st->sigma2 = sigma2; st->q = q; st->n_p = Np;
}

__device__ __forceinline__ void mstep_staged(DevState* st, const double* mom) {
    __shared__ DevState sst;
    __shared__ double smom[MOM_PAD];
    static_assert(sizeof(DevState) % 8 == 0, "DevState is copied as 8-byte words");
    const int nw = (int)(sizeof(DevState) / 8);
    for (int e = threadIdx.x; e < nw; e += blockDim.x) reinterpret_cast<double*>(&sst)[e] = reinterpret_cast<const double*>(st)[e];
    for (int e = threadIdx.x; e < MOM_PAD; e += blockDim.x) smom[e] = mom[e];
    __syncthreads();
    if (threadIdx.x == 0) mstep_solve_residual(&sst, smom);
    __syncthreads();
    if (threadIdx.x < 16) reinterpret_cast<double*>(st)[threadIdx.x] = reinterpret_cast<const double*>(&sst)[threadIdx.x];
}

template <int SOLVE>
__global__ void __launch_bounds__(256)
moments_kernel(DevState* st, const double* __restrict__ part_a, int nb_a, int ka, const double* __restrict__ part_b, int nb_b,
               int kb, double* __restrict__ mom) {
    __shared__ double sh[8][32];
    const int k = threadIdx.x & 31, w = threadIdx.x >> 5;
    double s = 0.0;
    if (k < ka) {
#pragma unroll 8
        for (int b = w; b < nb_a; b += 8) s += part_a[(size_t)b * ka + k];
    } else if (k < ka + kb) {
#pragma unroll 8
        for (int b = w; b < nb_b; b += 8) s += part_b[(size_t)b * kb + (k - ka)];
    }
    sh[w][k] = s;
    __syncthreads();
    if (w == 0) {
        double t = 0.0;
#pragma unroll
        for (int i = 0; i < 8; ++i) t += sh[i][k];
        mom[k] = t;
    }
    if (SOLVE) {
        __syncthreads();
        mstep_staged(st, mom);
    }
}
__global__ void mstep_residual_kernel(DevState* st, const double* __restrict__ mom) {
    mstep_staged(st, mom);
}
__global__ void mstep_api_kernel(DevState* st, const double* __restrict__ mom) {
    if (threadIdx.x == 0) mstep_solve_api(st, mom);
}

#ifndef CPD_HOST_EMU
__device__ __forceinline__ void st_release_sys(unsigned long long* p, unsigned long long v) {
    asm volatile("st.release.sys.global.u64 [%0], %1;" ::"l"(p), "l"(v) : "memory");
}
__device__ __forceinline__ unsigned long long ld_acquire_sys(const unsigned long long* p) {
    unsigned long long v;
    asm volatile("ld.acquire.sys.global.u64 %0, [%1];" : "=l"(v) : "l"(p) : "memory");
    return v;
}
__device__ __forceinline__ double ld_relaxed_sys(const double* p) {
    double v;
    asm volatile("ld.relaxed.sys.global.f64 %0, [%1];" : "=d"(v) : "l"(p) : "memory");
    return v;
}
#endif
__global__ void __launch_bounds__(256)
moments_p2p_kernel(DevState* st, const double* __restrict__ part_a, int nb_a, int ka, const double* __restrict__ part_b,
                   int nb_b, int kb, double* __restrict__ mom, P2PInfo* info) {
    __shared__ double sh[8][32];
    __shared__ double loc[32];
    __shared__ int timeout;
    const int k = threadIdx.x & 31, w = threadIdx.x >> 5;
    double s = 0.0;
    if (k < ka) {
#pragma unroll 8
        for (int b = w; b < nb_a; b += 8) s += part_a[(size_t)b * ka + k];
    } else if (k < ka + kb) {
#pragma unroll 8
        for (int b = w; b < nb_b; b += 8) s += part_b[(size_t)b * kb + (k - ka)];
    }
    sh[w][k] = s;
    if (threadIdx.x == 0) timeout = 0;
    __syncthreads();
    if (w == 0) {
        double t = 0.0;
#pragma unroll
        for (int i = 0; i < 8; ++i) t += sh[i][k];
        loc[k] = t;
    }
    __syncthreads();
    const int world = info->world, rank = info->rank;
    const unsigned long long seq = info->seq + 1;
    const int par = (int)(seq & 1ull);
    for (int r = w; r < world; r += 8) info->box[r]->slots[par][rank][k] = loc[k];
    __threadfence_system();
    __syncthreads();
    if ((int)threadIdx.x < world) {
        st_release_sys(&info->box[threadIdx.x]->flags[par][rank], seq);
        const unsigned long long* f = &info->box[rank]->flags[par][threadIdx.x];
        const unsigned long long t0 = globaltimer_ns(), limit = info->timeout_ns;
        while (ld_acquire_sys(f) < seq) {
            __nanosleep(64);
            if (globaltimer_ns() - t0 > limit) { timeout = 1; break; }
        }
    }
    __syncthreads();
    if (w == 0) {
        double t = 0.0;
        for (int r = 0; r < world; ++r) t += ld_relaxed_sys(&info->box[rank]->slots[par][r][k]);
        mom[k] = t;
        if (k == 0) {
            info->seq = seq;
            if (timeout) st->err = 1;
        }
    }
    __syncthreads();
    if (!timeout && st->err == 0) mstep_staged(st, mom);
}

__device__ __forceinline__ unsigned spread3(unsigned v) {
    v &= 0x3ffu;
    v = (v | (v << 16)) & 0x030000ffu;
    v = (v | (v << 8)) & 0x0300f00fu;
    v = (v | (v << 4)) & 0x030c30c3u;
    v = (v | (v << 2)) & 0x09249249u;
    return v;
}
__global__ void __launch_bounds__(THREADS)
morton_kernel(const double* __restrict__ pts, long long n, double lo0, double lo1, double lo2, double inv_range,
              unsigned* __restrict__ codes, int* __restrict__ idx) {
    const long long i = (long long)blockIdx.x * THREADS + threadIdx.x;
    if (i < n) {
        const double q0 = (pts[3 * i] - lo0) * inv_range, q1 = (pts[3 * i + 1] - lo1) * inv_range, q2 = (pts[3 * i + 2] - lo2) * inv_range;
        const unsigned a = (unsigned)fmin(fmax(q0 * 1023.0, 0.0), 1023.0), b = (unsigned)fmin(fmax(q1 * 1023.0, 0.0), 1023.0),
                       c = (unsigned)fmin(fmax(q2 * 1023.0, 0.0), 1023.0);
        codes[i] = spread3(a) | (spread3(b) << 1) | (spread3(c) << 2);
        idx[i] = (int)i;
    }
}
__global__ void __launch_bounds__(THREADS)
morton_frame_kernel(const double* __restrict__ pts, long long n, const double* __restrict__ frame, unsigned* __restrict__ codes,
                    int* __restrict__ idx) {
    const long long i = (long long)blockIdx.x * THREADS + threadIdx.x;
    if (i < n) {
        const double inv_range = frame[3];
        const double q0 = (pts[3 * i] - frame[0]) * inv_range, q1 = (pts[3 * i + 1] - frame[1]) * inv_range,
                     q2 = (pts[3 * i + 2] - frame[2]) * inv_range;
        const unsigned a = (unsigned)fmin(fmax(q0 * 1023.0, 0.0), 1023.0), b = (unsigned)fmin(fmax(q1 * 1023.0, 0.0), 1023.0),
                       c = (unsigned)fmin(fmax(q2 * 1023.0, 0.0), 1023.0);
        codes[i] = spread3(a) | (spread3(b) << 1) | (spread3(c) << 2);
        idx[i] = (int)i;
    }
}
__global__ void __launch_bounds__(THREADS)
gather3_frame_kernel(const double* __restrict__ in, const int* __restrict__ perm, long long n, const double* __restrict__ frame,
                     double* __restrict__ out) {
    const long long k = (long long)blockIdx.x * THREADS + threadIdx.x;
    if (k < n) {
        const long long j = perm[k];
        out[3 * k] = in[3 * j] - frame[4]; out[3 * k + 1] = in[3 * j + 1] - frame[5]; out[3 * k + 2] = in[3 * j + 2] - frame[6];
    }
}
__global__ void __launch_bounds__(THREADS)
gather3_kernel(const double* __restrict__ in, const int* __restrict__ perm, long long n, double o0, double o1, double o2,
               double* __restrict__ out) {
    const long long k = (long long)blockIdx.x * THREADS + threadIdx.x;
    if (k < n) {
        const long long j = perm[k];
        out[3 * k] = in[3 * j] - o0; out[3 * k + 1] = in[3 * j + 1] - o1; out[3 * k + 2] = in[3 * j + 2] - o2;
    }
}
__global__ void __launch_bounds__(THREADS)
gather1_kernel(const double* __restrict__ in, const int* __restrict__ perm, long long n, double* __restrict__ out) {
    const long long k = (long long)blockIdx.x * THREADS + threadIdx.x;
    if (k < n) out[k] = in[perm[k]];
}
__global__ void __launch_bounds__(THREADS)
gather_f32_kernel(const double* __restrict__ in, const int* __restrict__ perm, long long n, float* __restrict__ out) {
    const long long k = (long long)blockIdx.x * THREADS + threadIdx.x;
    if (k < n) out[k] = (float)in[perm[k]];
}
__global__ void __launch_bounds__(THREADS)
scatter_kernel(const double* __restrict__ in, const int* __restrict__ perm, long long n, int ncomp, double* __restrict__ out) {
    const long long k = (long long)blockIdx.x * THREADS + threadIdx.x;
    if (k < n) {
        const long long j = perm[k];
        for (int c = 0; c < ncomp; ++c) out[ncomp * j + c] = in[ncomp * k + c];
    }
}

__global__ void __launch_bounds__(THREADS)
stats_kernel(const double* __restrict__ pts, long long n, double* __restrict__ part) {
    __shared__ double sh[9][THREADS / 32];
    const long long i = (long long)blockIdx.x * THREADS + threadIdx.x;
    double v[9];
    if (i < n) {
        for (int a = 0; a < 3; ++a) { v[a] = pts[3 * i + a]; v[3 + a] = v[a]; v[6 + a] = v[a]; }
    } else {
        for (int a = 0; a < 3; ++a) { v[a] = 0.0; v[3 + a] = 1.0e300; v[6 + a] = -1.0e300; }
    }
    const int lane = threadIdx.x & 31, wid = threadIdx.x >> 5;
#pragma unroll
    for (int k = 0; k < 9; ++k) {
        double x = v[k];
#pragma unroll
        for (int o = 16; o > 0; o >>= 1) {
            const double y = __shfl_xor_sync(0xffffffffu, x, o);
            x = k < 3 ? x + y : (k < 6 ? fmin(x, y) : fmax(x, y));
        }
        if (lane == 0) sh[k][wid] = x;
    }
    __syncthreads();
    if (threadIdx.x < 9) {
        const int k = threadIdx.x;
        double x = sh[k][0];
        for (int w = 1; w < THREADS / 32; ++w) x = k < 3 ? x + sh[k][w] : (k < 6 ? fmin(x, sh[k][w]) : fmax(x, sh[k][w]));
        part[(size_t)blockIdx.x * 9 + k] = x;
    }
}
__global__ void __launch_bounds__(288)
stats_fold_kernel(const double* __restrict__ part, int nb, double* __restrict__ out) {
    const int k = threadIdx.x >> 5, lane = threadIdx.x & 31;
    double x = k < 3 ? 0.0 : (k < 6 ? 1.0e300 : -1.0e300);
    for (int b = lane; b < nb; b += 32) {
        const double y = part[(size_t)b * 9 + k];
        x = k < 3 ? x + y : (k < 6 ? fmin(x, y) : fmax(x, y));
    }
#pragma unroll
    for (int o = 16; o > 0; o >>= 1) {
        const double y = __shfl_xor_sync(0xffffffffu, x, o);
        x = k < 3 ? x + y : (k < 6 ? fmin(x, y) : fmax(x, y));
    }
    if (lane == 0) out[k] = x;
}

__global__ void cloud_frame_kernel(const double* __restrict__ sums9, long long count, int is_target, long long n_global, int origin_given,
                                   double o0, double o1, double o2, DevState* __restrict__ st, double* __restrict__ frame) {
    if (threadIdx.x != 0 || blockIdx.x != 0) return;
    double range = 0.0;
    for (int a = 0; a < 3; ++a) { frame[a] = sums9[3 + a]; range = fmax(range, sums9[6 + a] - sums9[3 + a]); }
    frame[3] = range > 0.0 ? 1.0 / range : 0.0;
    const double og[3] = {o0, o1, o2};
    for (int a = 0; a < 3; ++a) {
        const double o = origin_given ? og[a] : sums9[a] / (double)count;
        frame[4 + a] = o;
        if (is_target) st->cx[a] = o; else st->cy[a] = o;
    }
    if (is_target) st->n_global = n_global; else st->m = count;
}

__global__ void __launch_bounds__(THREADS)
cloud_sums_kernel(const double* __restrict__ pts, long long n, double* __restrict__ out) {
    const long long i = (long long)blockIdx.x * THREADS + threadIdx.x;
    double v[4] = {0.0, 0.0, 0.0, 0.0};
    if (i < n) {
        const double a = pts[3 * i], b = pts[3 * i + 1], c = pts[3 * i + 2];
        v[0] = a * a + b * b + c * c; v[1] = a; v[2] = b; v[3] = c;
    }
    block_reduce_store<4>(v, out + (size_t)blockIdx.x * 4);
}
__global__ void __launch_bounds__(1024)
reduce_cols_kernel(const double* __restrict__ part, int nb, int k, double* __restrict__ out) {
    const int c = threadIdx.x >> 5, lane = threadIdx.x & 31;
    if (c >= k) return;
    double s = 0.0;
    for (int b = lane; b < nb; b += 32) s += part[(size_t)b * k + c];
#pragma unroll
    for (int o = 16; o > 0; o >>= 1) s += __shfl_xor_sync(0xffffffffu, s, o);
    if (lane == 0) out[c] = s;
}

__global__ void __launch_bounds__(THREADS)
uncentre_px_kernel(const DevState* __restrict__ st, const double* __restrict__ p1, const double* __restrict__ pxc, int m,
                   double* __restrict__ px) {
    const int i = blockIdx.x * THREADS + threadIdx.x;
    if (i < m) {
#pragma unroll
        for (int d = 0; d < 3; ++d) px[3 * (size_t)i + d] = pxc[3 * (size_t)i + d] + st->cx[d] * p1[i];
    }
}
__global__ void __launch_bounds__(THREADS)
centre_px_kernel(const DevState* __restrict__ st, const double* __restrict__ p1, const double* __restrict__ px, int m,
                 double* __restrict__ pxc) {
    const int i = blockIdx.x * THREADS + threadIdx.x;
    if (i < m) {
#pragma unroll
        for (int d = 0; d < 3; ++d) pxc[3 * (size_t)i + d] = px[3 * (size_t)i + d] - st->cx[d] * p1[i];
    }
}
__global__ void __launch_bounds__(THREADS)
rbf_kernel_kernel(const float* __restrict__ x, long long nx, const float* __restrict__ y, long long ny, int dim, float two_beta,
                  float* __restrict__ out) {
    const long long j = (long long)blockIdx.y * THREADS + threadIdx.x;
    const long long i = blockIdx.x;
    if (j < ny) {
        float d2 = 0.f;
        for (int a = 0; a < dim; ++a) { const float d = x[i * dim + a] - y[j * dim + a]; d2 += d * d; }
        out[i * ny + j] = expf(-d2 / two_beta);
    }
}

__global__ void __launch_bounds__(THREADS)
imq_kernel_kernel(const float* __restrict__ x, long long nx, const float* __restrict__ y, long long ny, int dim, float c,
                  float* __restrict__ out) {
    const long long j = (long long)blockIdx.y * THREADS + threadIdx.x;
    const long long i = blockIdx.x;
    if (j < ny) {
        float d2 = 0.f;
        for (int a = 0; a < dim; ++a) { const float d = __fsub_rn(x[i * dim + a], y[j * dim + a]); d2 = __fadd_rn(d2, __fmul_rn(d, d)); }
        out[i * ny + j] = __fdiv_rn(1.0f, __fsqrt_rn(__fadd_rn(d2, c)));
    }
}

__global__ void __launch_bounds__(THREADS)
nr_gram_kernel(const double* __restrict__ yc, double c0, double c1, double c2, long long m, int dim, float two_beta,
               float* __restrict__ G) {
    const long long j = (long long)blockIdx.y * THREADS + threadIdx.x;
    const long long i = blockIdx.x;
    if (j < m) {
        const double cc[3] = {c0, c1, c2};
        float d2 = 0.f;
        for (int a = 0; a < dim; ++a) {
            const float d = (float)(yc[3 * i + a] + cc[a]) - (float)(yc[3 * j + a] + cc[a]);
            d2 += d * d;
        }
        G[i * m + j] = expf(-d2 / two_beta);
    }
}
__global__ void __launch_bounds__(THREADS)
nr_apply_kernel(const float* __restrict__ G, const double* __restrict__ W, const double* __restrict__ yc, double c0, double c1,
                double c2, long long m, double* __restrict__ ts) {
    const long long i = (long long)blockIdx.x * (THREADS / 32) + (threadIdx.x >> 5);
    const int lane = threadIdx.x & 31;
    if (i >= m) return;
    const float* row = G + i * m;
    double a0 = 0.0, a1 = 0.0, a2 = 0.0;
    for (long long j = lane; j < m; j += 32) {
        const double g = (double)row[j];
        a0 += g * W[3 * j]; a1 += g * W[3 * j + 1]; a2 += g * W[3 * j + 2];
    }
    a0 = warp_sum(a0); a1 = warp_sum(a1); a2 = warp_sum(a2);
    if (lane == 0) {
        ts[3 * i] = yc[3 * i] + c0 + a0;
        ts[3 * i + 1] = yc[3 * i + 1] + c1 + a1;
        ts[3 * i + 2] = yc[3 * i + 2] + c2 + a2;
    }
}
__global__ void __launch_bounds__(THREADS)
nr_system_kernel(const float* __restrict__ G, const double* __restrict__ wgt ,
                 const double* __restrict__ sigma2_ptr, double lmd, long long m, double* __restrict__ A) {
    const long long j = (long long)blockIdx.y * THREADS + threadIdx.x;
    const long long i = blockIdx.x;
    if (j < m) A[i * m + j] = wgt[i] * (double)G[i * m + j] + (i == j ? lmd * *sigma2_ptr : 0.0);
}
__global__ void __launch_bounds__(THREADS)
nr_rhs_kernel(const DevState* __restrict__ st, const double* __restrict__ p1, const double* __restrict__ pxc,
              const double* __restrict__ yc, const double* __restrict__ p1t, const double* __restrict__ pxt, double alpha, long long m,
              double* __restrict__ B) {
    const long long i = (long long)blockIdx.x * THREADS + threadIdx.x;
    if (i < m) {
        const double k = p1t ? st->sigma2 / alpha : 0.0;
#pragma unroll
        for (int c = 0; c < 3; ++c) {
            const double y = yc[3 * i + c] + st->cy[c];
            double r = pxc[3 * i + c] + p1[i] * (st->cx[c] - y);
            if (p1t) r += k * (pxt[3 * i + c] - p1t[i] * y);
            B[c * m + i] = r;
        }
    }
}
__global__ void __launch_bounds__(THREADS)
nr_weight_kernel(const double* __restrict__ p1, const double* __restrict__ p1t, const double* __restrict__ sigma2_ptr, double alpha,
                 long long m, double* __restrict__ wgt) {
    const long long i = (long long)blockIdx.x * THREADS + threadIdx.x;
    if (i < m) wgt[i] = p1[i] + (*sigma2_ptr / alpha) * p1t[i];
}
__global__ void __launch_bounds__(THREADS)
nr_identity_kernel(const double* __restrict__ yc, double c0, double c1, double c2, long long m, double* __restrict__ ts) {
    const long long i = (long long)blockIdx.x * THREADS + threadIdx.x;
    if (i < m) { ts[3 * i] = yc[3 * i] + c0; ts[3 * i + 1] = yc[3 * i + 1] + c1; ts[3 * i + 2] = yc[3 * i + 2] + c2; }
}
__global__ void __launch_bounds__(THREADS)
nr_unpack_kernel(const double* __restrict__ B, long long m, double* __restrict__ W) {
    const long long i = (long long)blockIdx.x * THREADS + threadIdx.x;
    if (i < m) { W[3 * i] = B[i]; W[3 * i + 1] = B[m + i]; W[3 * i + 2] = B[2 * m + i]; }
}
__global__ void __launch_bounds__(THREADS)
nr_resid_kernel(const DevState* __restrict__ st, const double* __restrict__ p1, const double* __restrict__ pxc,
                const double* __restrict__ ts_old, const double* __restrict__ ts_new, long long m, double* __restrict__ part) {
    const long long i = (long long)blockIdx.x * THREADS + threadIdx.x;
    double v[2] = {0.0, 0.0};
    if (i < m) {
        double acc = 0.0;
#pragma unroll
        for (int c = 0; c < 3; ++c) {
            const double e = ts_old[3 * i + c] - ts_new[3 * i + c];
            const double vv = pxc[3 * i + c] - p1[i] * (ts_old[3 * i + c] - st->cx[c]);
            acc += 2.0 * e * vv + p1[i] * e * e;
        }
        v[0] = acc; v[1] = p1[i];
    }
    block_reduce_store<2>(v, part + (size_t)blockIdx.x * 2);
}
__global__ void __launch_bounds__(THREADS)
nr_traces_kernel(const DevState* __restrict__ st, const double* __restrict__ pt1, const double* __restrict__ xc, long long n,
                 const double* __restrict__ p1, const double* __restrict__ pxc, const double* __restrict__ ts, long long m,
                 double* __restrict__ part) {
    const long long i = (long long)blockIdx.x * THREADS + threadIdx.x;
    double v[4] = {0.0, 0.0, 0.0, 0.0};
    if (i < n) {
        double x2 = 0.0;
#pragma unroll
        for (int c = 0; c < 3; ++c) { const double x = xc[3 * i + c] + st->cx[c]; x2 += x * x; }
        v[0] = pt1[i] * x2;
    }
    if (i < m) {
        double pt = 0.0, t2 = 0.0;
#pragma unroll
        for (int c = 0; c < 3; ++c) {
            const double t = ts[3 * i + c];
            pt += (pxc[3 * i + c] + st->cx[c] * p1[i]) * t;
            t2 += t * t;
        }
        v[1] = pt; v[2] = p1[i] * t2; v[3] = p1[i];
    }
    block_reduce_store<4>(v, part + (size_t)blockIdx.x * 4);
}
__global__ void __launch_bounds__(32)
nr_sigma_api_kernel(DevState* st, const double* __restrict__ tr) {
    if (threadIdx.x == 0) {
        st->sigma2 = (tr[0] - 2.0 * tr[1] + tr[2]) / (tr[3] * st->dim);
        st->q = st->sigma2;
        st->n_p = tr[3];
    }
}
__global__ void __launch_bounds__(32)
nr_sigma_kernel(DevState* st, const double* __restrict__ part, int nb, const double* __restrict__ mom) {
    if (threadIdx.x == 0) {
        double a = 0.0, np_ = 0.0;
        for (int b = 0; b < nb; ++b) { a += part[2 * (size_t)b]; np_ += part[2 * (size_t)b + 1]; }
        const double sk2 = LOG2E / (2.0 * st->sigma2);
        const double q = mom[RM_SRR] / sk2 + a;
        st->sigma2 = q / (np_ * st->dim);
        st->q = st->sigma2;
        st->n_p = np_;
    }
}

constexpr int GT_K = 4, GT_TILE = 256;
__global__ void __launch_bounds__(THREADS)
gauss_transform_kernel(const float4* __restrict__ tg, int n, const float4* __restrict__ sc, const float* __restrict__ wts, int mpad,
                       int k0, int kn, double* __restrict__ out) {
    __shared__ float4 sp[GT_TILE];
    __shared__ float sw[GT_K][GT_TILE];
    const int i = blockIdx.x * THREADS + threadIdx.x;
    const float4 t = tg[i < n ? i : n - 1];
    double acc[GT_K];
#pragma unroll
    for (int c = 0; c < GT_K; ++c) acc[c] = 0.0;
    for (int j0 = 0; j0 < mpad; j0 += GT_TILE) {
        __syncthreads();
        sp[threadIdx.x] = sc[j0 + threadIdx.x];
#pragma unroll
        for (int c = 0; c < GT_K; ++c) sw[c][threadIdx.x] = c < kn ? wts[(size_t)(k0 + c) * mpad + j0 + threadIdx.x] : 0.0f;
        __syncthreads();
#pragma unroll 1
        for (int g = 0; g < GT_TILE; g += 32) {
            float a[GT_K];
#pragma unroll
            for (int c = 0; c < GT_K; ++c) a[c] = 0.0f;
#pragma unroll 8
            for (int jj = 0; jj < 32; ++jj) {
                const float4 b = sp[g + jj];
                const float dx = t.x - b.x, dy = t.y - b.y, dz = t.z - b.z;
                const float e = ex2(-fmaf(dz, dz, fmaf(dy, dy, dx * dx)));
#pragma unroll
                for (int c = 0; c < GT_K; ++c) a[c] = fmaf(e, sw[c][g + jj], a[c]);
            }
#pragma unroll
            for (int c = 0; c < GT_K; ++c) acc[c] += (double)a[c];
        }
    }
    if (i < n)
        for (int c = 0; c < kn; ++c) out[(size_t)(k0 + c) * n + i] = acc[c];
}

__global__ void __launch_bounds__(256)
probe_ffma_kernel(float* out, int iters, float seed) {
    float a[16];
#pragma unroll
    for (int k = 0; k < 16; ++k) a[k] = seed + k;
    const float m = 0.9999f + seed * 1e-9f, c = 1e-7f;
    for (int i = 0; i < iters; ++i) {
#pragma unroll
        for (int k = 0; k < 16; ++k) a[k] = fmaf(a[k], m, c);
    }
    float s = 0.f;
#pragma unroll
    for (int k = 0; k < 16; ++k) s += a[k];
    if (s == 123.456f) out[0] = s;
}
__global__ void __launch_bounds__(256)
probe_mufu_kernel(float* out, int iters, float seed) {
    float a[8];
#pragma unroll
    for (int k = 0; k < 8; ++k) a[k] = seed * 0.01f - k;
    for (int i = 0; i < iters; ++i) {
#pragma unroll
        for (int k = 0; k < 8; ++k) a[k] = ex2(a[k]) - 1.5f;
    }
    float s = 0.f;
#pragma unroll
    for (int k = 0; k < 8; ++k) s += a[k];
    if (s == 123.456f) out[0] = s;
}
__global__ void __launch_bounds__(256)
probe_ffma2_kernel(float* out, int iters, float seed) {
    u64 a[8];
#pragma unroll
    for (int k = 0; k < 8; ++k) a[k] = pack2(seed + k, seed - k);
    const u64 m = pack2(0.9999f + seed * 1e-9f, 0.9998f), c = pack2(1e-7f, 2e-7f);
    for (int i = 0; i < iters; ++i) {
#pragma unroll
        for (int k = 0; k < 8; ++k) a[k] = ffma2(a[k], m, c);
    }
    float s = 0.f;
#pragma unroll
    for (int k = 0; k < 8; ++k) { const float2 v = unpack2(a[k]); s += v.x + v.y; }
    if (s == 123.456f) out[0] = s;
}
__global__ void __launch_bounds__(256)
probe_ffma_mixed_kernel(float* out, int iters, float seed) {
    u64 a[6];
    float b[6];
#pragma unroll
    for (int k = 0; k < 6; ++k) { a[k] = pack2(seed + k, seed - k); b[k] = seed + 0.5f * k; }
    const u64 m2 = pack2(0.9999f + seed * 1e-9f, 0.9998f), c2 = pack2(1e-7f, 2e-7f);
    const float m = 0.9999f + seed * 1e-9f, c = 1e-7f;
    for (int i = 0; i < iters; ++i) {
#pragma unroll
        for (int k = 0; k < 6; ++k) { a[k] = ffma2(a[k], m2, c2); b[k] = fmaf(b[k], m, c); }
    }
    float s = 0.f;
#pragma unroll
    for (int k = 0; k < 6; ++k) { const float2 v = unpack2(a[k]); s += v.x + v.y + b[k]; }
    if (s == 123.456f) out[0] = s;
}
template <int NF, bool PACKED>
__global__ void __launch_bounds__(256)
probe_mix_kernel(float* out, int iters, float seed) {
    float x[8], acc[8];
    unsigned long long pa[4];
#pragma unroll
    for (int k = 0; k < 8; ++k) { x[k] = seed * 0.01f - 0.1f * k; acc[k] = 0.f; }
#pragma unroll
    for (int k = 0; k < 4; ++k) pa[k] = pack2(seed, seed + k);
    const float m = 0.999f + seed * 1e-9f;
    const unsigned long long pm = pack2(m, m);
    for (int i = 0; i < iters; ++i) {
        if (PACKED) {
#pragma unroll
            for (int k = 0; k < 4; ++k) {
#pragma unroll
                for (int f = 0; f < NF; ++f) pa[k] = ffma2(pa[k], pm, pm);
                const float2 v = unpack2(pa[k]);
                pa[k] = pack2(ex2(-v.x * v.x), ex2(-v.y * v.y));
            }
        } else {
#pragma unroll
            for (int k = 0; k < 8; ++k) {
                float t = x[k];
#pragma unroll
                for (int f = 0; f < NF - 1; ++f) t = fmaf(t, m, acc[k]);
                const float e = ex2(-t * t);
                acc[k] = e;
            }
        }
    }
    float s = 0.f;
#pragma unroll
    for (int k = 0; k < 8; ++k) s += acc[k];
#pragma unroll
    for (int k = 0; k < 4; ++k) { const float2 v = unpack2(pa[k]); s += v.x + v.y; }
    if (s == 123.456f) out[0] = s;
}
__global__ void probe_clock_kernel(long long* out) {
    const long long c0 = clock64();
    const unsigned long long t0 = globaltimer_ns();
    unsigned long long t1;
    do { t1 = globaltimer_ns(); } while (t1 - t0 < 2000000ull);
    out[0] = clock64() - c0;
    out[1] = (long long)(t1 - t0);
}

}
```

Measured before the change: 105.3.

## Drop paired-float duplicated records and use scalar float4 layouts in E-step passes

Removes the duplicated srcJ record buffer and the emulated packed float2 arithmetic. Pass1 and pass2 now read compact float4 records (16 and 32 bytes instead of 32 and 48), which halves the target Q footprint. Pass1 uses scalar per-point math, and the pipeline depth drops from 3 to 2 stages. Pass2 moves its double accumulators from registers into shared memory, trading register pressure for extra shared-memory traffic and a larger dynamic smem footprint.

New measurement: 108.3 (median of 6 runs). 1.03x the previous value.

```diff
diff --git a/probreg_b200/csrc/cpd_b200.cu b/probreg_b200/csrc/cpd_b200.cu
--- a/probreg_b200/csrc/cpd_b200.cu
+++ b/probreg_b200/csrc/cpd_b200.cu
@@ -148,7 +148,7 @@
     long long m = 0, mpad = 0, n = 0, npad = 0, n_global = 0;
     double *d_yc = nullptr, *d_ts = nullptr, *d_xc = nullptr, *d_raw = nullptr;
     size_t raw_cap = 0;
-    float4 *d_srcP = nullptr, *d_srcJ = nullptr, *d_tgtP = nullptr, *d_tgtQ = nullptr;
+    float4 *d_srcP = nullptr, *d_tgtP = nullptr, *d_tgtQ = nullptr;
     P1Part* d_part1 = nullptr;
     double* d_part2 = nullptr;
     size_t part1_cap = 0, part2_cap = 0;
@@ -496,7 +496,7 @@
     const long long cover = std::max(h->mpad, h->n);
     mark(h, 0);
     pack_kernel<<<blocks_for(cover), THREADS, 0, h->stream>>>(h->d_state, d_sigma2, h->d_yc, d_ts, h->d_xc, h->m, h->mpad,
-                                                              h->n, h->d_srcP, h->d_srcJ, h->d_tgtP);
+                                                              h->n, h->d_srcP, h->d_tgtP);
     mark(h, 1);
     const bool cull = h->cull_on && h->cull_active;
     const int nst1 = (int)(h->mpad / P1_STAGE);
@@ -511,10 +511,10 @@
     }
     const bool wgt = h->wgt_on;
     if (wgt) {
-        weight_patch_kernel<<<blocks_for(h->m), THREADS, 0, h->stream>>>(h->d_la, h->m, h->d_srcP, h->d_srcJ);
+        weight_patch_kernel<<<blocks_for(h->m), THREADS, 0, h->stream>>>(h->d_la, h->m, h->d_srcP);
         h->launches += 1;
     }
-#define CPD_PASS1(C, W) pass1_kernel<C, W><<<h->g1, THREADS, PASS1_SMEM, h->stream>>>(h->d_tgtP, (int)h->n, h->d_srcJ, h->d_work1, h->d_part1, h->d_sbox, nst1, (C) ? h->d_ssub : nullptr)
+#define CPD_PASS1(C, W) pass1_kernel<C, W><<<h->g1, THREADS, PASS1_SMEM, h->stream>>>(h->d_tgtP, (int)h->n, h->d_srcP, h->d_work1, h->d_part1, h->d_sbox, nst1, (C) ? h->d_ssub : nullptr)
     if (cull) { if (wgt) CPD_PASS1(true, true); else CPD_PASS1(true, false); }
     else { if (wgt) CPD_PASS1(false, true); else CPD_PASS1(false, false); }
 #undef CPD_PASS1
@@ -661,7 +661,7 @@
     for (int r = 0; r < P2P_MAX; ++r) if (h->peer_ptr[r]) cudaIpcCloseMemHandle(h->peer_ptr[r]);
     if (h->d_box) cudaFree(h->d_box);
     if (h->d_p2p) cudaFree(h->d_p2p);
-    void* ptrs[] = {h->d_yc, h->d_ts, h->d_xc, h->d_raw, h->d_srcP, h->d_srcJ, h->d_tgtP, h->d_tgtQ, h->d_part1, h->d_part2, h->d_pt1, h->d_p1,
+    void* ptrs[] = {h->d_yc, h->d_ts, h->d_xc, h->d_raw, h->d_srcP, h->d_tgtP, h->d_tgtQ, h->d_part1, h->d_part2, h->d_pt1, h->d_p1,
                     h->d_pxc, h->d_px, h->d_mom_src, h->d_mom_tgt, h->d_mom, h->d_sums, h->d_state, h->d_flush};
     for (void* p : ptrs) if (p) cudaFree(p);
     if (h->h_pin) cudaFreeHost(h->h_pin);
@@ -692,7 +692,6 @@
         TRY(dev_alloc(&h->d_yc, (size_t)m * 3));
         TRY(dev_alloc(&h->d_ts, (size_t)m * 3));
         TRY(dev_alloc(&h->d_srcP, (size_t)h->mpad));
-        TRY(dev_alloc(&h->d_srcJ, (size_t)h->mpad * 2));
         TRY(dev_alloc(&h->d_p1, (size_t)m));
         TRY(dev_alloc(&h->d_pxc, (size_t)m * 3));
         TRY(dev_alloc(&h->d_px, (size_t)m * 3));
@@ -720,7 +719,7 @@
         h->npad = (n_local + P2_STAGE - 1) / P2_STAGE * P2_STAGE;
         TRY(dev_alloc(&h->d_xc, (size_t)n_local * 3));
         TRY(dev_alloc(&h->d_tgtP, (size_t)n_local));
-        TRY(dev_alloc(&h->d_tgtQ, (size_t)h->npad * 3));
+        TRY(dev_alloc(&h->d_tgtQ, (size_t)h->npad * 2));
         TRY(dev_alloc(&h->d_pt1, (size_t)n_local));
         TRY(dev_alloc(&h->d_perm_tgt, (size_t)n_local));
         TRY(dev_alloc(&h->d_outN, (size_t)n_local));
diff --git a/probreg_b200/csrc/kernels.cuh b/probreg_b200/csrc/kernels.cuh
--- a/probreg_b200/csrc/kernels.cuh
+++ b/probreg_b200/csrc/kernels.cuh
@@ -4,35 +4,12 @@
 
 namespace cpd {
 
-#ifndef CPD_RI1
-#define CPD_RI1 4
-#endif
-#ifndef CPD_RI2
-#define CPD_RI2 4
-#endif
-#ifndef CPD_MINB1
-#define CPD_MINB1 2
-#endif
-#ifndef CPD_MINB2
-#define CPD_MINB2 2
-#endif
-#ifndef CPD_UNROLL1
-#define CPD_UNROLL1 4
-#endif
-#ifndef CPD_UNROLL2
-#define CPD_UNROLL2 4
-#endif
 #ifndef CPD_SUB
 #define CPD_SUB 64
 #endif
-#ifndef CPD_GRP
-#define CPD_GRP 8
-#endif
-constexpr int UNROLL1 = CPD_UNROLL1, UNROLL2 = CPD_UNROLL2;
 constexpr int THREADS = 256;
-constexpr int RI1 = CPD_RI1, RI2 = CPD_RI2;
+constexpr int RI1 = 4, RI2 = 4;
 constexpr int ITILE1 = THREADS * RI1, ITILE2 = THREADS * RI2;
-constexpr int NPAIR1 = RI1 / 2, NPAIR2 = RI2 / 2;
 #ifndef CPD_P1_STAGE
 #define CPD_P1_STAGE 512
 #endif
@@ -42,15 +19,14 @@
 constexpr int P1_STAGE = CPD_P1_STAGE;
 constexpr int P2_STAGE = CPD_P2_STAGE;
 static_assert(P1_STAGE % 256 == 0 && P2_STAGE % 256 == 0 && P1_STAGE >= 256 && P2_STAGE >= 256, "stage sizes are multiples of 256");
-constexpr int P1_REC = 32, P2_REC = 48;
-#ifndef CPD_NSTAGE
-#define CPD_NSTAGE 3
-#endif
-constexpr int NSTAGE = CPD_NSTAGE;
+constexpr int P1_REC = 16, P2_REC = 32;
+constexpr int NSTAGE = 2;
 constexpr int P1_STAGE_BYTES = P1_STAGE * P1_REC, P2_STAGE_BYTES = P2_STAGE * P2_REC;
 constexpr int SUB = CPD_SUB;
-constexpr int GRP = CPD_GRP;
-constexpr int PASS1_SMEM = NSTAGE * P1_STAGE_BYTES + 64, PASS2_SMEM = NSTAGE * P2_STAGE_BYTES + 64;
+constexpr int GRP = 8;
+static_assert(SUB % GRP == 0, "a sub-chunk is a whole number of groups");
+constexpr int P2_ACC_BYTES = 4 * RI2 * THREADS * 8;
+constexpr int PASS1_SMEM = NSTAGE * P1_STAGE_BYTES + 64, PASS2_SMEM = NSTAGE * P2_STAGE_BYTES + 64 + P2_ACC_BYTES;
 
 #ifdef CPD_HOST_EMU
 #define CPD_DYN_SMEM(name) unsigned char* const name = emu::g_dyn_smem
@@ -120,25 +96,6 @@
     asm("ex2.approx.ftz.f32 %0, %1;" : "=f"(y) : "f"(x));
     return y;
 }
-typedef unsigned long long u64;
-__device__ __forceinline__ u64 pack2(float lo, float hi) { u64 r; asm("mov.b64 %0, {%1, %2};" : "=l"(r) : "f"(lo), "f"(hi)); return r; }
-__device__ __forceinline__ float2 unpack2(u64 v) { float2 r; asm("mov.b64 {%0, %1}, %2;" : "=f"(r.x), "=f"(r.y) : "l"(v)); return r; }
-__device__ __forceinline__ u64 fsub2(u64 a, u64 b) {
-    const float2 x = unpack2(a), y = unpack2(b);
-    return pack2(__fsub_rn(x.x, y.x), __fsub_rn(x.y, y.y));
-}
-__device__ __forceinline__ u64 fadd2(u64 a, u64 b) {
-    const float2 x = unpack2(a), y = unpack2(b);
-    return pack2(__fadd_rn(x.x, y.x), __fadd_rn(x.y, y.y));
-}
-__device__ __forceinline__ u64 fmul2(u64 a, u64 b) {
-    const float2 x = unpack2(a), y = unpack2(b);
-    return pack2(__fmul_rn(x.x, y.x), __fmul_rn(x.y, y.y));
-}
-__device__ __forceinline__ u64 ffma2(u64 a, u64 b, u64 c) {
-    const float2 x = unpack2(a), y = unpack2(b), z = unpack2(c);
-    return pack2(__fmaf_rn(x.x, y.x, z.x), __fmaf_rn(x.y, y.y, z.y));
-}
 __device__ __forceinline__ unsigned long long globaltimer_ns() {
     unsigned long long t;
     asm volatile("mov.u64 %0, %%globaltimer;" : "=l"(t));
@@ -199,7 +156,7 @@
 pack_kernel(const DevState* __restrict__ st, const double* __restrict__ sigma2_ptr,
             const double* __restrict__ yc , const double* __restrict__ ts ,
             const double* __restrict__ xc , long long m, long long mpad, long long n,
-            float4* __restrict__ srcP , float4* __restrict__ srcJ ,
+            float4* __restrict__ srcP ,
             float4* __restrict__ tgtP ) {
     const long long i = (long long)blockIdx.x * THREADS + threadIdx.x;
     const double sk = sqrt(LOG2E / (2.0 * *sigma2_ptr));
@@ -229,8 +186,6 @@
             o = make_float4(FAR_COORD, FAR_COORD, FAR_COORD, 0.0f);
         }
         srcP[i] = o;
-        srcJ[2 * i] = make_float4(o.x, o.x, o.y, o.y);
-        srcJ[2 * i + 1] = make_float4(o.z, o.z, 0.0f, 0.0f);
     }
     if (i < n) {
         tgtP[i] = make_float4((float)(sk * xc[3 * i]), (float)(sk * xc[3 * i + 1]), (float)(sk * xc[3 * i + 2]), 0.0f);
@@ -238,15 +193,9 @@
 }
 
 __global__ void __launch_bounds__(THREADS)
-weight_patch_kernel(const float* __restrict__ la, long long m, float4* __restrict__ srcP, float4* __restrict__ srcJ) {
+weight_patch_kernel(const float* __restrict__ la, long long m, float4* __restrict__ srcP) {
     const long long i = (long long)blockIdx.x * THREADS + threadIdx.x;
-    if (i < m) {
-        const float v = la[i];
-        srcP[i].w = v;
-        float4 r = srcJ[2 * i + 1];
-        r.z = v; r.w = v;
-        srcJ[2 * i + 1] = r;
-    }
+    if (i < m) srcP[i].w = la[i];
 }
 
 constexpr float CULL_GAP = 130.0f;
@@ -286,7 +235,7 @@
     __shared__ float sh[THREADS / 32];
     const int b = blockIdx.x;
     float m = 3.0e38f;
-    for (int i = threadIdx.x; i < P2_STAGE; i += THREADS) m = fminf(m, tgtQ[3 * ((size_t)b * P2_STAGE + i) + 1].z);
+    for (int i = threadIdx.x; i < P2_STAGE; i += THREADS) m = fminf(m, tgtQ[2 * ((size_t)b * P2_STAGE + i)].w);
 #pragma unroll
     for (int o = 16; o > 0; o >>= 1) m = fminf(m, __shfl_xor_sync(0xffffffffu, m, o));
     if ((threadIdx.x & 31) == 0) sh[threadIdx.x >> 5] = m;
@@ -324,20 +273,19 @@
     const int b = blockIdx.x * (THREADS / 32) + (threadIdx.x >> 5), lane = threadIdx.x & 31;
     if (b >= nsub) return;
     float m = 3.0e38f;
-    for (int i = lane; i < SUB; i += 32) m = fminf(m, tgtQ[3 * ((size_t)b * SUB + i) + 1].z);
+    for (int i = lane; i < SUB; i += 32) m = fminf(m, tgtQ[2 * ((size_t)b * SUB + i)].w);
 #pragma unroll
     for (int o = 16; o > 0; o >>= 1) m = fminf(m, __shfl_xor_sync(0xffffffffu, m, o));
     if (lane == 0) omax[b] = -m;
 }
-template <int NP>
-__device__ __forceinline__ void warp_bbox(const u64 (&ax)[NP], const u64 (&ay)[NP], const u64 (&az)[NP], float* __restrict__ wbox) {
+template <int R>
+__device__ __forceinline__ void warp_bbox(const float (&ax)[R], const float (&ay)[R], const float (&az)[R], float* __restrict__ wbox) {
     float lo[3] = {3.0e38f, 3.0e38f, 3.0e38f}, hi[3] = {-3.0e38f, -3.0e38f, -3.0e38f};
 #pragma unroll
-    for (int p = 0; p < NP; ++p) {
-        const float2 x = unpack2(ax[p]), y = unpack2(ay[p]), z = unpack2(az[p]);
-        lo[0] = fminf(lo[0], fminf(x.x, x.y)); hi[0] = fmaxf(hi[0], fmaxf(x.x, x.y));
-        lo[1] = fminf(lo[1], fminf(y.x, y.y)); hi[1] = fmaxf(hi[1], fmaxf(y.x, y.y));
-        lo[2] = fminf(lo[2], fminf(z.x, z.y)); hi[2] = fmaxf(hi[2], fmaxf(z.x, z.y));
+    for (int r = 0; r < R; ++r) {
+        lo[0] = fminf(lo[0], ax[r]); hi[0] = fmaxf(hi[0], ax[r]);
+        lo[1] = fminf(lo[1], ay[r]); hi[1] = fmaxf(hi[1], ay[r]);
+        lo[2] = fminf(lo[2], az[r]); hi[2] = fmaxf(hi[2], az[r]);
     }
 #pragma unroll
     for (int a = 0; a < 3; ++a) {
@@ -361,59 +309,51 @@
 }
 
 template <bool WGT>
-__device__ __forceinline__ void pass1_sum(const ulonglong2* __restrict__ q, const u64 (&ax)[NPAIR1], const u64 (&ay)[NPAIR1],
-                                          const u64 (&az)[NPAIR1], const u64 (&no)[NPAIR1], u64 (&Sc)[NPAIR1], u64 (&Uc)[NPAIR1]) {
-    if (GRP > 0) {
+__device__ __forceinline__ void pass1_sum(const float4* __restrict__ q, const float (&ax)[RI1], const float (&ay)[RI1],
+                                          const float (&az)[RI1], const float (&no)[RI1], float (&Sc)[RI1], float (&Uc)[RI1]) {
 #pragma unroll 1
-        for (int g0 = 0; g0 < SUB; g0 += (GRP > 0 ? GRP : SUB)) {
-            u64 gs[NPAIR1], gu[NPAIR1];
-#pragma unroll
-            for (int jj = 0; jj < (GRP > 0 ? GRP : 1); ++jj) {
-                const ulonglong2 bxy = q[2 * (g0 + jj)];
-                const u64 bz = q[2 * (g0 + jj) + 1].x;
-                u64 la = 0ull;
-                if (WGT) la = q[2 * (g0 + jj) + 1].y;
-#pragma unroll
-                for (int p = 0; p < NPAIR1; ++p) {
-                    const u64 dx = fsub2(ax[p], bxy.x), dy = fsub2(ay[p], bxy.y), dz = fsub2(az[p], bz);
-                    u64 t = ffma2(dx, dx, no[p]);
-                    t = ffma2(dy, dy, t);
-                    t = ffma2(dz, dz, t);
-                    if (WGT) t = fadd2(t, la);
-                    const float2 tt = unpack2(t);
-                    const u64 e = pack2(ex2(-tt.x), ex2(-tt.y));
-                    gs[p] = jj == 0 ? e : fadd2(gs[p], e);
-                    gu[p] = jj == 0 ? fmul2(e, t) : ffma2(e, t, gu[p]);
-                }
-            }
-#pragma unroll
-            for (int p = 0; p < NPAIR1; ++p) { Sc[p] = fadd2(Sc[p], gs[p]); Uc[p] = fadd2(Uc[p], gu[p]); }
-        }
-    } else {
-#pragma unroll UNROLL1
-        for (int jj = 0; jj < SUB; ++jj) {
-            const ulonglong2 bxy = q[2 * jj];
-            const u64 bz = q[2 * jj + 1].x;
-            u64 la = 0ull;
-            if (WGT) la = q[2 * jj + 1].y;
-#pragma unroll
-            for (int p = 0; p < NPAIR1; ++p) {
-                const u64 dx = fsub2(ax[p], bxy.x), dy = fsub2(ay[p], bxy.y), dz = fsub2(az[p], bz);
-                u64 t = ffma2(dx, dx, no[p]);
-                t = ffma2(dy, dy, t);
-                t = ffma2(dz, dz, t);
-                if (WGT) t = fadd2(t, la);
-                const float2 tt = unpack2(t);
-                const u64 e = pack2(ex2(-tt.x), ex2(-tt.y));
-                Sc[p] = fadd2(Sc[p], e);
-                Uc[p] = ffma2(e, t, Uc[p]);
-            }
+    for (int g0 = 0; g0 < SUB; g0 += GRP) {
+        float gs[RI1], gu[RI1];
+#pragma unroll
+        for (int jj = 0; jj < GRP; ++jj) {
+            const float4 b = q[g0 + jj];
+#pragma unroll
+            for (int r = 0; r < RI1; ++r) {
+                const float dx = __fsub_rn(ax[r], b.x), dy = __fsub_rn(ay[r], b.y), dz = __fsub_rn(az[r], b.z);
+                float t = __fmaf_rn(dx, dx, no[r]);
+                t = __fmaf_rn(dy, dy, t);
+                t = __fmaf_rn(dz, dz, t);
+                if (WGT) t = __fadd_rn(t, b.w);
+                const float e = ex2(-t);
+                gs[r] = jj == 0 ? e : __fadd_rn(gs[r], e);
+                gu[r] = jj == 0 ? __fmul_rn(e, t) : __fmaf_rn(e, t, gu[r]);
+            }
+        }
+#pragma unroll
+        for (int r = 0; r < RI1; ++r) { Sc[r] = __fadd_rn(Sc[r], gs[r]); Uc[r] = __fadd_rn(Uc[r], gu[r]); }
+    }
+}
+
+template <bool WGT>
+__device__ __forceinline__ void pass1_umin(const float4* __restrict__ q, int n, const float (&ax)[RI1], const float (&ay)[RI1],
+                                           const float (&az)[RI1], float (&cm)[RI1]) {
+#pragma unroll
+    for (int r = 0; r < RI1; ++r) cm[r] = 3.0e38f;
+#pragma unroll 4
+    for (int jj = 0; jj < n; ++jj) {
+        const float4 b = q[jj];
+#pragma unroll
+        for (int r = 0; r < RI1; ++r) {
+            const float dx = __fsub_rn(ax[r], b.x), dy = __fsub_rn(ay[r], b.y), dz = __fsub_rn(az[r], b.z);
+            float u = __fmaf_rn(dz, dz, __fmaf_rn(dy, dy, __fmul_rn(dx, dx)));
+            if (WGT) u = __fadd_rn(u, b.w);
+            cm[r] = fminf(cm[r], u);
         }
     }
 }
 
 template <bool CULL, bool WGT>
-__global__ void __launch_bounds__(THREADS, CPD_MINB1)
+__global__ void __launch_bounds__(THREADS, 2)
 pass1_kernel(const float4* __restrict__ ipts, int ni, const float4* __restrict__ jrec, const int4* __restrict__ work,
              P1Part* __restrict__ part, const float4* __restrict__ sbox ,
              int nstages_total, const float4* __restrict__ ssub ) {
@@ -439,19 +379,17 @@
         }
     }
     if (itile * ITILE1 + (tid >> 5) * (32 * RI1) >= ni) return;
-    u64 ax[NPAIR1], ay[NPAIR1], az[NPAIR1], no[NPAIR1];
+    float ax[RI1], ay[RI1], az[RI1], no[RI1];
     double S[RI1], SU[RI1];
 #pragma unroll
-    for (int p = 0; p < NPAIR1; ++p) {
-        int n0 = itile * ITILE1 + (tid >> 5) * (32 * RI1) + (2 * p) * 32 + (tid & 31), n1 = n0 + 32;
+    for (int r = 0; r < RI1; ++r) {
+        int n0 = itile * ITILE1 + (tid >> 5) * (32 * RI1) + r * 32 + (tid & 31);
         n0 = n0 < ni ? n0 : ni - 1;
-        n1 = n1 < ni ? n1 : ni - 1;
-        const float4 p0 = ipts[n0], p1 = ipts[n1];
-        ax[p] = pack2(p0.x, p1.x); ay[p] = pack2(p0.y, p1.y); az[p] = pack2(p0.z, p1.z);
-        no[p] = pack2(-O_INIT, -O_INIT);
+        const float4 p = ipts[n0];
+        ax[r] = p.x; ay[r] = p.y; az[r] = p.z;
     }
     float* const mybox = wbox[tid >> 5];
-    warp_bbox<NPAIR1>(ax, ay, az, mybox);
+    warp_bbox<RI1>(ax, ay, az, mybox);
     {
         const int lane = tid & 31;
         float best = 3.0e38f;
@@ -466,35 +404,16 @@
             const int oi = __shfl_xor_sync(0xffffffffu, bi, o);
             if (ob < best || (ob == best && oi < bi)) { best = ob; bi = oi; }
         }
-        const ulonglong2* near = reinterpret_cast<const ulonglong2*>(jbytes + (size_t)bi * P1_STAGE_BYTES);
         float cm[RI1];
-#pragma unroll
-        for (int r = 0; r < RI1; ++r) cm[r] = 3.0e38f;
-#pragma unroll 4
-        for (int jj = 0; jj < 128; ++jj) {
-            const ulonglong2 bxy = near[2 * jj];
-            const u64 bz = near[2 * jj + 1].x;
-            u64 la = 0ull;
-            if (WGT) la = near[2 * jj + 1].y;
-#pragma unroll
-            for (int p = 0; p < NPAIR1; ++p) {
-                const u64 dx = fsub2(ax[p], bxy.x), dy = fsub2(ay[p], bxy.y), dz = fsub2(az[p], bz);
-                u64 uu = ffma2(dz, dz, ffma2(dy, dy, fmul2(dx, dx)));
-                if (WGT) uu = fadd2(uu, la);
-                const float2 u = unpack2(uu);
-                cm[2 * p] = fminf(cm[2 * p], u.x);
-                cm[2 * p + 1] = fminf(cm[2 * p + 1], u.y);
-            }
-        }
-#pragma unroll
-        for (int p = 0; p < NPAIR1; ++p)
-            no[p] = pack2(-fminf(O_INIT, floorf(cm[2 * p])), -fminf(O_INIT, floorf(cm[2 * p + 1])));
+        pass1_umin<WGT>(reinterpret_cast<const float4*>(jbytes + (size_t)bi * P1_STAGE_BYTES), 128, ax, ay, az, cm);
+#pragma unroll
+        for (int r = 0; r < RI1; ++r) no[r] = -fminf(O_INIT, floorf(cm[r]));
     }
     float omax_w = O_INIT;
     if (CULL) {
         float om = -3.0e38f;
 #pragma unroll
-        for (int p = 0; p < NPAIR1; ++p) { const float2 nv = unpack2(no[p]); om = fmaxf(om, fmaxf(-nv.x, -nv.y)); }
+        for (int r = 0; r < RI1; ++r) om = fmaxf(om, -no[r]);
 #pragma unroll
         for (int o = 16; o > 0; o >>= 1) om = fmaxf(om, __shfl_xor_sync(0xffffffffu, om, o));
         omax_w = om;
@@ -504,7 +423,7 @@
     for (int it = 0; it < nst; ++it) {
         const int s = it % NSTAGE;
         mbar_wait(&full[s], (uint32_t)((it / NSTAGE) & 1));
-        const ulonglong2* sp = reinterpret_cast<const ulonglong2*>(smraw + s * P1_STAGE_BYTES);
+        const float4* sp = reinterpret_cast<const float4*>(smraw + s * P1_STAGE_BYTES);
         bool skip = false;
         if (CULL) {
             const float4 blo = sbox[2 * (st0 + it)], bhi = sbox[2 * (st0 + it) + 1];
@@ -516,52 +435,29 @@
                 const int sb = (st0 + it) * (P1_STAGE / SUB) + sc;
                 if (box_gap2(mybox, ssub[2 * sb], ssub[2 * sb + 1]) - omax_w >= CULL_GAP) continue;
             }
-            const ulonglong2* q = sp + sc * (2 * SUB);
-            u64 Sc[NPAIR1], Uc[NPAIR1];
-#pragma unroll
-            for (int p = 0; p < NPAIR1; ++p) { Sc[p] = 0ull; Uc[p] = 0ull; }
+            const float4* q = sp + sc * SUB;
+            float Sc[RI1], Uc[RI1];
+#pragma unroll
+            for (int r = 0; r < RI1; ++r) { Sc[r] = 0.0f; Uc[r] = 0.0f; }
             pass1_sum<WGT>(q, ax, ay, az, no, Sc, Uc);
             bool bad = false;
 #pragma unroll
-            for (int p = 0; p < NPAIR1; ++p) {
-                const float2 v = unpack2(Sc[p]);
-                bad |= !(v.x < TWO100) | !(v.y < TWO100);
-            }
+            for (int r = 0; r < RI1; ++r) bad |= !(Sc[r] < TWO100);
             if (__any_sync(0xffffffffu, bad)) {
                 float cm[RI1];
-#pragma unroll
-                for (int r = 0; r < RI1; ++r) cm[r] = 3.0e38f;
-#pragma unroll UNROLL1
-                for (int jj = 0; jj < SUB; ++jj) {
-                    const ulonglong2 bxy = q[2 * jj];
-                    const u64 bz = q[2 * jj + 1].x;
-                    u64 la = 0ull;
-                    if (WGT) la = q[2 * jj + 1].y;
-#pragma unroll
-                    for (int p = 0; p < NPAIR1; ++p) {
-                        const u64 dx = fsub2(ax[p], bxy.x), dy = fsub2(ay[p], bxy.y), dz = fsub2(az[p], bz);
-                        u64 uu = ffma2(dz, dz, ffma2(dy, dy, fmul2(dx, dx)));
-                        if (WGT) uu = fadd2(uu, la);
-                        const float2 u = unpack2(uu);
-                        cm[2 * p] = fminf(cm[2 * p], u.x);
-                        cm[2 * p + 1] = fminf(cm[2 * p + 1], u.y);
-                    }
-                }
-#pragma unroll
-                for (int p = 0; p < NPAIR1; ++p) {
-                    const float2 nv = unpack2(no[p]);
-                    const float o0 = -nv.x, o1 = -nv.y;
-                    const float on0 = fminf(o0, floorf(cm[2 * p])), on1 = fminf(o1, floorf(cm[2 * p + 1]));
-                    const int sh0 = (int)fmaxf(on0 - o0, -4000.0f), sh1 = (int)fmaxf(on1 - o1, -4000.0f);
-                    S[2 * p] = ldexp(S[2 * p], sh0); SU[2 * p] = ldexp(SU[2 * p], sh0);
-                    S[2 * p + 1] = ldexp(S[2 * p + 1], sh1); SU[2 * p + 1] = ldexp(SU[2 * p + 1], sh1);
-                    no[p] = pack2(-on0, -on1);
-                    Sc[p] = 0ull; Uc[p] = 0ull;
+                pass1_umin<WGT>(q, SUB, ax, ay, az, cm);
+#pragma unroll
+                for (int r = 0; r < RI1; ++r) {
+                    const float o = -no[r], on = fminf(o, floorf(cm[r]));
+                    const int sh = (int)fmaxf(on - o, -4000.0f);
+                    S[r] = ldexp(S[r], sh); SU[r] = ldexp(SU[r], sh);
+                    no[r] = -on;
+                    Sc[r] = 0.0f; Uc[r] = 0.0f;
                 }
                 if (CULL) {
                     float om = -3.0e38f;
 #pragma unroll
-                    for (int p = 0; p < NPAIR1; ++p) { const float2 nv = unpack2(no[p]); om = fmaxf(om, fmaxf(-nv.x, -nv.y)); }
+                    for (int r = 0; r < RI1; ++r) om = fmaxf(om, -no[r]);
 #pragma unroll
                     for (int o = 16; o > 0; o >>= 1) om = fmaxf(om, __shfl_xor_sync(0xffffffffu, om, o));
                     omax_w = om;
@@ -569,12 +465,9 @@
                 pass1_sum<WGT>(q, ax, ay, az, no, Sc, Uc);
             }
 #pragma unroll
-            for (int p = 0; p < NPAIR1; ++p) {
-                const float2 sv = unpack2(Sc[p]), uv = unpack2(Uc[p]), nv = unpack2(no[p]);
-                S[2 * p] += (double)sv.x;
-                S[2 * p + 1] += (double)sv.y;
-                SU[2 * p] += (double)uv.x - (double)nv.x * (double)sv.x;
-                SU[2 * p + 1] += (double)uv.y - (double)nv.y * (double)sv.y;
+            for (int r = 0; r < RI1; ++r) {
+                S[r] += (double)Sc[r];
+                SU[r] += (double)Uc[r] - (double)no[r] * (double)Sc[r];
             }
         }
         __syncthreads();
@@ -584,16 +477,12 @@
         }
     }
 #pragma unroll
-    for (int p = 0; p < NPAIR1; ++p) {
-        const float2 nv = unpack2(no[p]);
-#pragma unroll
-        for (int h = 0; h < 2; ++h) {
-            const int n = itile * ITILE1 + (tid >> 5) * (32 * RI1) + (2 * p + h) * 32 + (tid & 31);
-            if (n < ni) {
-                P1Part out;
-                out.S = S[2 * p + h]; out.SU = SU[2 * p + h]; out.o = h ? -nv.y : -nv.x; out.pad = 0.0f;
-                part[(size_t)split * ni + n] = out;
-            }
+    for (int r = 0; r < RI1; ++r) {
+        const int n = itile * ITILE1 + (tid >> 5) * (32 * RI1) + r * 32 + (tid & 31);
+        if (n < ni) {
+            P1Part out;
+            out.S = S[r]; out.SU = SU[r]; out.o = -no[r]; out.pad = 0.0f;
+            part[(size_t)split * ni + n] = out;
         }
     }
 }
@@ -654,19 +543,17 @@
             v[0] = SU * (double)rnf;
         }
         v[1] = p1n;
-        tgtQ[3 * (size_t)i] = make_float4(b.x, b.x, b.y, b.y);
-        tgtQ[3 * (size_t)i + 1] = make_float4(b.z, b.z, no, no);
-        tgtQ[3 * (size_t)i + 2] = make_float4(rnf, rnf, 0.f, 0.f);
+        tgtQ[2 * (size_t)i] = make_float4(b.x, b.y, b.z, no);
+        tgtQ[2 * (size_t)i + 1] = make_float4(rnf, 0.f, 0.f, 0.f);
     } else if (i < npad) {
-        tgtQ[3 * (size_t)i] = make_float4(0.f, 0.f, 0.f, 0.f);
-        tgtQ[3 * (size_t)i + 1] = make_float4(0.f, 0.f, INFINITY, INFINITY);
-        tgtQ[3 * (size_t)i + 2] = make_float4(0.f, 0.f, 0.f, 0.f);
+        tgtQ[2 * (size_t)i] = make_float4(0.f, 0.f, 0.f, INFINITY);
+        tgtQ[2 * (size_t)i + 1] = make_float4(0.f, 0.f, 0.f, 0.f);
     }
     block_reduce_store<RM_TGT>(v, mom_part + (size_t)blockIdx.x * RM_TGT);
 }
 
 template <bool CULL, bool WGT>
-__global__ void __launch_bounds__(THREADS, CPD_MINB2)
+__global__ void __launch_bounds__(THREADS, 2)
 pass2_kernel(const float4* __restrict__ ipts, int ni, const float4* __restrict__ jrec, const int4* __restrict__ work,
              double* __restrict__ part , const float4* __restrict__ tbox ,
              const float* __restrict__ omax_stage, const float4* __restrict__ tsub, const float* __restrict__ omax_sub) {
@@ -689,25 +576,23 @@
             tma_load_1d(smraw + s * P2_STAGE_BYTES, jbytes + (size_t)(st0 + s) * P2_STAGE_BYTES, P2_STAGE_BYTES, &full[s]);
         }
     }
-    u64 ax[NPAIR2], ay[NPAIR2], az[NPAIR2], al[NPAIR2];
-    double A1[RI2], AX[RI2], AY[RI2], AZ[RI2];
-#pragma unroll
-    for (int p = 0; p < NPAIR2; ++p) {
-        int m0 = itile * ITILE2 + (tid >> 5) * (32 * RI2) + (2 * p) * 32 + (tid & 31), m1 = m0 + 32;
+    double* const acc = reinterpret_cast<double*>(smraw + NSTAGE * P2_STAGE_BYTES + 64) + tid;
+    float ax[RI2], ay[RI2], az[RI2], al[RI2];
+#pragma unroll
+    for (int r = 0; r < RI2; ++r) {
+        int m0 = itile * ITILE2 + (tid >> 5) * (32 * RI2) + r * 32 + (tid & 31);
         m0 = m0 < ni ? m0 : ni - 1;
-        m1 = m1 < ni ? m1 : ni - 1;
-        const float4 p0 = ipts[m0], p1 = ipts[m1];
-        ax[p] = pack2(p0.x, p1.x); ay[p] = pack2(p0.y, p1.y); az[p] = pack2(p0.z, p1.z);
-        if (WGT) al[p] = pack2(p0.w, p1.w);
+        const float4 p = ipts[m0];
+        ax[r] = p.x; ay[r] = p.y; az[r] = p.z; al[r] = p.w;
     }
     float* const mybox = wbox[tid >> 5];
-    if (CULL) warp_bbox<NPAIR2>(ax, ay, az, mybox);
-#pragma unroll
-    for (int r = 0; r < RI2; ++r) { A1[r] = 0.0; AX[r] = 0.0; AY[r] = 0.0; AZ[r] = 0.0; }
+    if (CULL) warp_bbox<RI2>(ax, ay, az, mybox);
+#pragma unroll
+    for (int k = 0; k < 4 * RI2; ++k) acc[k * THREADS] = 0.0;
     for (int it = 0; it < nst; ++it) {
         const int s = it % NSTAGE;
         mbar_wait(&full[s], (uint32_t)((it / NSTAGE) & 1));
-        const ulonglong2* sp = reinterpret_cast<const ulonglong2*>(smraw + s * P2_STAGE_BYTES);
+        const float4* sp = reinterpret_cast<const float4*>(smraw + s * P2_STAGE_BYTES);
         bool skip = false;
         if (CULL) {
             const float4 blo = tbox[2 * (st0 + it)], bhi = tbox[2 * (st0 + it) + 1];
@@ -719,67 +604,43 @@
                 const int sb = (st0 + it) * (P2_STAGE / SUB) + sc;
                 if (box_gap2(mybox, tsub[2 * sb], tsub[2 * sb + 1]) - omax_sub[sb] >= CULL_GAP) continue;
             }
-            const ulonglong2* q = sp + sc * (3 * SUB);
-            u64 s1[NPAIR2], sx[NPAIR2], sy[NPAIR2], sz[NPAIR2];
-#pragma unroll
-            for (int p = 0; p < NPAIR2; ++p) { s1[p] = 0ull; sx[p] = 0ull; sy[p] = 0ull; sz[p] = 0ull; }
-            if (GRP > 0) {
+            const float4* q = sp + sc * (2 * SUB);
+            float s1[RI2], sx[RI2], sy[RI2], sz[RI2];
+#pragma unroll
+            for (int r = 0; r < RI2; ++r) { s1[r] = 0.0f; sx[r] = 0.0f; sy[r] = 0.0f; sz[r] = 0.0f; }
 #pragma unroll 1
-                for (int g0 = 0; g0 < SUB; g0 += (GRP > 0 ? GRP : SUB)) {
-                    u64 g1[NPAIR2], gx[NPAIR2], gy[NPAIR2], gz[NPAIR2];
-#pragma unroll
-                    for (int jj = 0; jj < (GRP > 0 ? GRP : 1); ++jj) {
-                        const ulonglong2 bxy = q[3 * (g0 + jj)];
-                        const ulonglong2 bzo = q[3 * (g0 + jj) + 1];
-                        const u64 rn = q[3 * (g0 + jj) + 2].x;
-#pragma unroll
-                        for (int p = 0; p < NPAIR2; ++p) {
-                            const u64 dx = fsub2(ax[p], bxy.x), dy = fsub2(ay[p], bxy.y), dz = fsub2(az[p], bzo.x);
-                            u64 t = ffma2(dx, dx, bzo.y);
-                            t = ffma2(dy, dy, t);
-                            t = ffma2(dz, dz, t);
-                            if (WGT) t = fadd2(t, al[p]);
-                            const float2 tt = unpack2(t);
-                            const u64 pr = fmul2(pack2(ex2(-tt.x), ex2(-tt.y)), rn);
-                            g1[p] = jj == 0 ? pr : fadd2(g1[p], pr);
-                            gx[p] = jj == 0 ? fmul2(pr, dx) : ffma2(pr, dx, gx[p]);
-                            gy[p] = jj == 0 ? fmul2(pr, dy) : ffma2(pr, dy, gy[p]);
-                            gz[p] = jj == 0 ? fmul2(pr, dz) : ffma2(pr, dz, gz[p]);
-                        }
-                    }
-#pragma unroll
-                    for (int p = 0; p < NPAIR2; ++p) {
-                        s1[p] = fadd2(s1[p], g1[p]); sx[p] = fadd2(sx[p], gx[p]);
-                        sy[p] = fadd2(sy[p], gy[p]); sz[p] = fadd2(sz[p], gz[p]);
+            for (int g0 = 0; g0 < SUB; g0 += GRP) {
+                float g1[RI2], gx[RI2], gy[RI2], gz[RI2];
+#pragma unroll
+                for (int jj = 0; jj < GRP; ++jj) {
+                    const float4 b = q[2 * (g0 + jj)];
+                    const float rn = q[2 * (g0 + jj) + 1].x;
+#pragma unroll
+                    for (int r = 0; r < RI2; ++r) {
+                        const float dx = __fsub_rn(ax[r], b.x), dy = __fsub_rn(ay[r], b.y), dz = __fsub_rn(az[r], b.z);
+                        float t = __fmaf_rn(dx, dx, b.w);
+                        t = __fmaf_rn(dy, dy, t);
+                        t = __fmaf_rn(dz, dz, t);
+                        if (WGT) t = __fadd_rn(t, al[r]);
+                        const float pr = __fmul_rn(ex2(-t), rn);
+                        g1[r] = jj == 0 ? pr : __fadd_rn(g1[r], pr);
+                        gx[r] = jj == 0 ? __fmul_rn(pr, dx) : __fmaf_rn(pr, dx, gx[r]);
+                        gy[r] = jj == 0 ? __fmul_rn(pr, dy) : __fmaf_rn(pr, dy, gy[r]);
+                        gz[r] = jj == 0 ? __fmul_rn(pr, dz) : __fmaf_rn(pr, dz, gz[r]);
                     }
                 }
-            } else {
-#pragma unroll UNROLL2
-                for (int jj = 0; jj < SUB; ++jj) {
-                    const ulonglong2 bxy = q[3 * jj];
-                    const ulonglong2 bzo = q[3 * jj + 1];
-                    const u64 rn = q[3 * jj + 2].x;
-#pragma unroll
-                    for (int p = 0; p < NPAIR2; ++p) {
-                        const u64 dx = fsub2(ax[p], bxy.x), dy = fsub2(ay[p], bxy.y), dz = fsub2(az[p], bzo.x);
-                        u64 t = ffma2(dx, dx, bzo.y);
-                        t = ffma2(dy, dy, t);
-                        t = ffma2(dz, dz, t);
-                        if (WGT) t = fadd2(t, al[p]);
-                        const float2 tt = unpack2(t);
-                        const u64 pr = fmul2(pack2(ex2(-tt.x), ex2(-tt.y)), rn);
-                        s1[p] = fadd2(s1[p], pr);
-                        sx[p] = ffma2(pr, dx, sx[p]);
-                        sy[p] = ffma2(pr, dy, sy[p]);
-                        sz[p] = ffma2(pr, dz, sz[p]);
-                    }
+#pragma unroll
+                for (int r = 0; r < RI2; ++r) {
+                    s1[r] = __fadd_rn(s1[r], g1[r]); sx[r] = __fadd_rn(sx[r], gx[r]);
+                    sy[r] = __fadd_rn(sy[r], gy[r]); sz[r] = __fadd_rn(sz[r], gz[r]);
                 }
             }
 #pragma unroll
-            for (int p = 0; p < NPAIR2; ++p) {
-                const float2 v1 = unpack2(s1[p]), vx = unpack2(sx[p]), vy = unpack2(sy[p]), vz = unpack2(sz[p]);
-                A1[2 * p] += (double)v1.x; AX[2 * p] += (double)vx.x; AY[2 * p] += (double)vy.x; AZ[2 * p] += (double)vz.x;
-                A1[2 * p + 1] += (double)v1.y; AX[2 * p + 1] += (double)vx.y; AY[2 * p + 1] += (double)vy.y; AZ[2 * p + 1] += (double)vz.y;
+            for (int r = 0; r < RI2; ++r) {
+                acc[(0 * RI2 + r) * THREADS] += (double)s1[r];
+                acc[(1 * RI2 + r) * THREADS] += (double)sx[r];
+                acc[(2 * RI2 + r) * THREADS] += (double)sy[r];
+                acc[(3 * RI2 + r) * THREADS] += (double)sz[r];
             }
         }
         __syncthreads();
@@ -793,8 +654,8 @@
         const int m = itile * ITILE2 + (tid >> 5) * (32 * RI2) + r * 32 + (tid & 31);
         if (m < ni) {
             double2* dst = reinterpret_cast<double2*>(part + ((size_t)split * ni + m) * 4);
-            dst[0] = make_double2(A1[r], AX[r]);
-            dst[1] = make_double2(AY[r], AZ[r]);
+            dst[0] = make_double2(acc[(0 * RI2 + r) * THREADS], acc[(1 * RI2 + r) * THREADS]);
+            dst[1] = make_double2(acc[(2 * RI2 + r) * THREADS], acc[(3 * RI2 + r) * THREADS]);
         }
     }
 }
@@ -1604,6 +1465,15 @@
     for (int k = 0; k < 8; ++k) s += a[k];
     if (s == 123.456f) out[0] = s;
 }
+#ifndef CPD_HOST_EMU
+typedef unsigned long long u64;
+__device__ __forceinline__ u64 pack2(float lo, float hi) { u64 r; asm("mov.b64 %0, {%1, %2};" : "=l"(r) : "f"(lo), "f"(hi)); return r; }
+__device__ __forceinline__ float2 unpack2(u64 v) { float2 r; asm("mov.b64 {%0, %1}, %2;" : "=f"(r.x), "=f"(r.y) : "l"(v)); return r; }
+__device__ __forceinline__ u64 ffma2(u64 a, u64 b, u64 c) {
+    const float2 x = unpack2(a), y = unpack2(b), z = unpack2(c);
+    return pack2(__fmaf_rn(x.x, y.x, z.x), __fmaf_rn(x.y, y.y, z.y));
+}
+#endif
 __global__ void __launch_bounds__(256)
 probe_ffma2_kernel(float* out, int iters, float seed) {
     u64 a[8];
```
